# Cecile-hi/Multimodal-Learning-with-Alternating-Unimodal-Adaptation

Hardware: AMD Instinct MI355X
Metric: samples/sec per MLA alternating step, CREMA-D A+V bs=64 (higher is better)
Workload: dtype f32; 1 GPU; CREMA-D MLA step (--gs_flag, --lorb base ResNet18 audio+visual, GS projection as_intended), per-GPU batch 64: spec 1x1024x128 + frames 3x3x224x224, 6 classes; global_batch=64, parallelism=dp1

## Files before the change

### include/mla_hip.h

```cpp
#ifndef MLA_HIP_H
#define MLA_HIP_H

#include <stddef.h>
#include <stdint.h>

#ifdef __cplusplus
extern "C" {
#endif

enum mla_status {
  MLA_OK = 0,
  MLA_ERR_INVALID_ARG = -1,
  MLA_ERR_WORKSPACE = -2,
  MLA_ERR_LAUNCH = -3
};

int mla_abi_version(void);
const char* mla_last_error(void);

int mla_video_to_nhwc(const float* src, float* dst, int B, int C, int T, int H, int W, void* stream);
int mla_nchw_to_nhwc(const float* src, float* dst, int N, int C, int H, int W, void* stream);
int mla_nhwc_to_nchw(const float* src, float* dst, int N, int C, int H, int W, void* stream);

int mla_conv2d_f32_cfg(int cfg);
size_t mla_conv2d_fwd_partial_elems(int N, int H, int W, int Cin, int Cout, int KH, int KW, int stride, int pad);
int mla_conv2d_fwd(const float* x, const float* w_hwio, float* y,
                   int N, int H, int W, int Cin, int Cout, int KH, int KW, int stride, int pad,
                   float* bn_partial, int* bn_tiles, void* stream);

int mla_conv2d_dgrad(const float* dy, const float* w_hwio, float* dx,
                     int N, int H, int W, int Cin, int Cout, int KH, int KW, int stride, int pad,
                     const float* residual, const float* relu_src, float* wt_ws, void* stream);

size_t mla_conv2d_wgrad_ws_bytes(int N, int H, int W, int Cin, int Cout, int KH, int KW, int stride, int pad);
int mla_conv2d_wgrad(const float* x, const float* dy, float* dw_hwio,
                     int N, int H, int W, int Cin, int Cout, int KH, int KW, int stride, int pad,
                     void* ws, size_t ws_bytes, void* stream);

size_t mla_conv2d_wsplit_bytes(int Cin, int Cout, int KH, int KW);
int mla_conv2d_wsplit(const float* w_hwio, void* wsplit, int Cin, int Cout, int KH, int KW, int transposed, void* stream);
int mla_conv2d_wsplit_batch(const float* params, void* wsplit, const int* desc, int n, int total_blocks, void* stream);
int mla_conv2d_fwd_split(const float* x, const void* wsplit_t, float* y,
                         int N, int H, int W, int Cin, int Cout, int KH, int KW, int stride, int pad,
                         float* bn_partial, int* bn_tiles, void* stream);
int mla_conv2d_dgrad_split(const float* dy, const void* wsplit, float* dx,
                           int N, int H, int W, int Cin, int Cout, int KH, int KW, int stride, int pad,
                           const float* residual, const float* relu_src, void* stream);

typedef struct mla_bn_reduce_req {
  const float* x;
  const float* mean;
  const float* invstd;
  float* partial;
} mla_bn_reduce_req;
size_t mla_conv2d_dgrad_bn_partial_elems(int N, int H, int W, int Cin);
int mla_conv2d_dgrad_bn(const float* dy, const float* w_hwio, float* dx, int N, int H, int W, int Cin, int Cout,
                        int KH, int KW, int stride, int pad, const float* residual, const float* relu_src, float* wt_ws,
                        const mla_bn_reduce_req* reqs, int nreq, int* bn_tiles, void* stream);
int mla_conv2d_dgrad_split_bn(const float* dy, const void* wsplit, float* dx, int N, int H, int W, int Cin, int Cout,
                              int KH, int KW, int stride, int pad, const float* residual, const float* relu_src,
                              const mla_bn_reduce_req* reqs, int nreq, int* bn_tiles, void* stream);
int mla_conv2d_dgrad_classes(const float* dy, const float* w_hwio, float* dx, int N, int H, int W, int Cin, int Cout,
                             int KH, int KW, int stride, int pad, const float* residual, const float* relu_src, float* wt_ws,
                             const mla_bn_reduce_req* reqs, int nreq, int* bn_tiles, int class_mask, int residual_mask,
                             void* stream);
int mla_conv2d_dgrad_split_classes(const float* dy, const void* wsplit, float* dx, int N, int H, int W, int Cin, int Cout,
                                   int KH, int KW, int stride, int pad, const float* residual, const float* relu_src,
                                   const mla_bn_reduce_req* reqs, int nreq, int* bn_tiles, int class_mask, int residual_mask,
                                   void* stream);
size_t mla_conv2d_wgrad_split_ws_bytes(int N, int H, int W, int Cin, int Cout, int KH, int KW, int stride, int pad);
int mla_conv2d_wgrad_split(const float* x, const float* dy, float* dw_hwio,
                           int N, int H, int W, int Cin, int Cout, int KH, int KW, int stride, int pad,
                           void* ws, size_t ws_bytes, void* stream);
int mla_conv2d_wgrad_tr(int on);
int mla_conv2d_patch(int on);
int mla_conv2d_bnfold_supported(int N, int H, int W, int Cin, int Cout, int KH, int KW, int stride, int pad);
int mla_conv2d_fwd_split_bnin(const float* x, const void* wsplit_t, float* y, int N, int H, int W, int Cin, int Cout, int KH, int KW,
                              int stride, int pad, const float* in_mean, const float* in_invstd, const float* in_gamma, const float* in_beta,
                              float* bn_partial, int* bn_tiles, void* stream);
int mla_conv2d_wgrad_split_bnin(const float* x, const float* dy, float* dw_hwio, int N, int H, int W, int Cin, int Cout, int KH, int KW,
                                int stride, int pad, const float* in_mean, const float* in_invstd, const float* in_gamma,
                                const float* in_beta, void* ws, size_t ws_bytes, void* stream);
int mla_conv2d_dgrad_split_bnmask(const float* dy, const void* wsplit, float* dx, int N, int H, int W, int Cin, int Cout, int KH, int KW,
                                  int stride, int pad, const mla_bn_reduce_req* reqs, int nreq, int* bn_tiles, const float* mask_gamma,
                                  const float* mask_beta, void* stream);
int mla_conv2d_dgrad_merge(int on);
int mla_conv2d_two_phase(int on);
int mla_conv2d_split_terms(int terms);
int mla_conv2d_stem_supported(int Cin, int Cout, int KH, int KW, int stride, int pad);
int mla_conv2d_stem_waves(int waves);
size_t mla_conv2d_stem_fwd_partial_elems(void);
int mla_conv2d_stem_fwd_split(const float* x, const float* w_hwio, float* y,
                              int N, int H, int W, int Cin, int Cout, int KH, int KW, int stride, int pad,
                              float* bn_partial, int* bn_tiles, void* stream);
size_t mla_conv2d_stem_wgrad_split_ws_bytes(int Cin);
int mla_conv2d_stem_wgrad_split(const float* x, const float* dy, float* dw_hwio,
                                int N, int H, int W, int Cin, int Cout, int KH, int KW, int stride, int pad,
                                void* ws, size_t ws_bytes, void* stream);
int mla_conv2d_split_cfg(int cfg);

size_t mla_conv2d_wimage_bytes_bf16(int Cin, int Cout, int KH, int KW);
int mla_conv2d_wimage_bf16(const float* w_hwio, void* wimage, int Cin, int Cout, int KH, int KW, int transposed, void* stream);
int mla_conv2d_wimage_batch_bf16(const float* params, void* wimage, const int* desc, int n, int total_blocks, void* stream);
int mla_conv2d_tile_bf16(int M, int Cout, int k_total);
int mla_conv2d_fwd_bf16(const float* x, const void* wimage_t, float* y,
                        int N, int H, int W, int Cin, int Cout, int KH, int KW, int stride, int pad,
                        float* bn_partial, int* bn_tiles, void* stream);
int mla_conv2d_dgrad_bf16(const float* dy, const void* wimage, float* dx,
                          int N, int H, int W, int Cin, int Cout, int KH, int KW, int stride, int pad,
                          const float* residual, const float* relu_src, int class_mask, int residual_mask, void* stream);
size_t mla_conv2d_wgrad_ws_bytes_bf16(int N, int H, int W, int Cin, int Cout, int KH, int KW, int stride, int pad);
int mla_conv2d_wgrad_bf16(const float* x, const float* dy, float* dw_hwio,
                          int N, int H, int W, int Cin, int Cout, int KH, int KW, int stride, int pad,
                          void* ws, size_t ws_bytes, void* stream);

size_t mla_bn_partial_scratch_elems(int C);
size_t mla_bn_stats_partial_elems(int M, int C);
int mla_bn_stats_partial(const float* x, int M, int C, float* partial, int* tiles, void* stream);
int mla_bn_finalize(const float* partial, int tiles, int M, int C, float eps, float momentum,
                    float* mean, float* invstd, float* running_mean, float* running_var, void* stream);
int mla_bn_apply(const float* x, const float* mean, const float* invstd, const float* gamma,
                 const float* beta, const float* residual, float* out, int M, int C, int relu, void* stream);
size_t mla_bn_bwd_ws_elems(int M, int C);
int mla_bn_bwd(const float* dout, const float* relu_out, const float* x, const float* mean,
               const float* invstd, const float* gamma, float* dx, float* dgamma, float* dbeta,
               float* g_out, float* ws, int M, int C, void* stream);

int mla_bn_bwd_from_partial(const float* dout, const float* x, const float* mean, const float* invstd, const float* gamma,
                            float* dx, float* dgamma, float* dbeta, float* partial, int tiles, int M, int C, void* stream);
int mla_bn_relu_maxpool_fwd(const float* y, const float* mean, const float* invstd, const float* gamma,
                            const float* beta, float* out, uint8_t* idx, int N, int H, int W, int C, void* stream);
int mla_bn_bwd_pooled(const float* dpool, const uint8_t* idx, const float* y, const float* mean, const float* invstd,
                      const float* gamma, const float* beta, float* dy, float* dgamma, float* dbeta, float* ws,
                      int N, int H, int W, int C, void* stream);

int mla_maxpool3x3s2_fwd(const float* x, float* y, uint8_t* idx, int N, int H, int W, int C, void* stream);
int mla_maxpool3x3s2_bwd(const float* dy, const uint8_t* idx, const float* relu_src, float* dx,
                         int N, int H, int W, int C, void* stream);
int mla_avgpool_fwd(const float* x, float* y, int NB, int P, int C, void* stream);
int mla_avgpool_bwd(const float* dy, const float* relu_src, float* dx, int NB, int P, int C, void* stream);

size_t mla_head_ws_elems(int B, int C);
int mla_head_ce_fwd_bwd(const float* X, const float* W, const float* b, const int64_t* labels,
                        float* logits, float* loss, float* dW, float* db, float* dX, float* ws,
                        int B, int D, int C, float inv_batch, void* stream);

int mla_ce_fwd_bwd(const float* logits, const int64_t* labels, float* loss, float* dlogits, float* ws,
                   int B, int C, float inv_batch, void* stream);
int mla_head_bwd(const float* X, const float* W, const float* dlogits, float* dW, float* db, float* dX,
                 int B, int D, int C, float scale, void* stream);
int mla_scale_by_device_scalar(float* x, const float* scalar, size_t n, void* stream);

size_t mla_concat_head_ws_elems(int B, int C, int M);
int mla_concat_head_ce_fwd_bwd(const float* x0, const float* x1, const float* x2, const float* W, const float* b,
                               const int64_t* labels, float* out, float* out_m, float* loss, float* loss_m, float* dW,
                               float* db, float* dx0, float* dx1, float* dx2, float* ws, int M, int B, int D, int C,
                               float inv_batch, void* stream);
int mla_concat_head_fwd(const float* x0, const float* x1, const float* x2, const float* W, const float* b, float* out,
                        float* out_m, int M, int B, int D, int C, void* stream);
int mla_concat_head_bwd(const float* x0, const float* x1, const float* x2, const float* W, const float* dlogits, float* dW,
                        float* db, float* dx0, float* dx1, float* dx2, int M, int B, int D, int C, float scale, void* stream);

int mla_colsum(const float* X, float* r, int B, int D, float scale, void* stream);
size_t mla_gs_ws_elems(int D, int C);
int mla_gs_project(float* Pl, const float* r, float* G, int D, int C, float alpha, float* ws, void* stream);

int mla_ogm_coeff(const float* out0, const float* out1, const float* out2, const int64_t* labels, int M, int B, int C,
                  float alpha, float* coeff, float* info, void* stream);
int mla_ogm_chunk_elems(void);
size_t mla_ogm_ws_bytes(int total_chunks, int n_seg);
int mla_ogm_modulate(float* grad, const int64_t* seg_desc, const int* first_chunk, int n_seg, int total_chunks,
                     const float* coeff, int ge, uint64_t seed, uint64_t step, void* ws, size_t ws_bytes, void* stream);

int mla_linear_fwd(const float* x, const float* w_kn, const float* bias, const float* residual, float* y,
                   float* y_gelu, int groups, int rows, int x_group_rows, int x_off, int y_group_rows, int y_off,
                   int K, int N, void* stream);
int mla_linear_dgrad(const float* dy, const float* w_kn, float* dx, const float* residual, const float* gelu_src,
                     float* wt_ws, int groups, int rows, int dy_group_rows, int dy_off, int dx_group_rows, int dx_off,
                     int K, int N, void* stream);
size_t mla_linear_wgrad_ws_bytes(int M, int K, int N);
int mla_linear_wgrad(const float* x, const float* dy, float* dw_kn, int groups, int rows, int x_group_rows, int x_off,
                     int K, int N, void* ws, size_t ws_bytes, void* stream);
int mla_linear_fwd_split(const float* x, const void* wsplit_t, const float* bias, const float* residual, float* y,
                         float* y_gelu, int groups, int rows, int x_group_rows, int x_off, int y_group_rows, int y_off,
                         int K, int N, void* stream);
int mla_linear_dgrad_split(const float* dy, const void* wsplit, float* dx, const float* residual, const float* gelu_src,
                           int groups, int rows, int dy_group_rows, int dy_off, int dx_group_rows, int dx_off,
                           int K, int N, void* stream);
size_t mla_linear_wgrad_split_ws_bytes(int M, int K, int N);
int mla_linear_wgrad_split(const float* x, const float* dy, float* dw_kn, int groups, int rows, int x_group_rows, int x_off,
                           int K, int N, void* ws, size_t ws_bytes, void* stream);
int mla_linear_wgrad_split_bias(const float* x, const float* dy, float* dw_kn, float* dbias, int groups, int rows,
                                int x_group_rows, int x_off, int K, int N, void* ws, size_t ws_bytes, void* stream);
int mla_linear_fwd_bf16(const float* x, const void* wimage_t, const float* bias, const float* residual, float* y,
                        float* y_gelu, int groups, int rows, int x_group_rows, int x_off, int y_group_rows, int y_off,
                        int K, int N, void* stream);
int mla_linear_dgrad_bf16(const float* dy, const void* wimage, float* dx, const float* residual, const float* gelu_src,
                          int groups, int rows, int dy_group_rows, int dy_off, int dx_group_rows, int dx_off, int K, int N,
                          void* stream);
size_t mla_linear_wgrad_ws_bytes_bf16(int M, int K, int N);
int mla_linear_wgrad_bf16(const float* x, const float* dy, float* dw_kn, int groups, int rows, int x_group_rows, int x_off,
                          int K, int N, void* ws, size_t ws_bytes, void* stream);
int mla_linear_wgrad_bias_bf16(const float* x, const float* dy, float* dw_kn, float* dbias, int groups, int rows,
                               int x_group_rows, int x_off, int K, int N, void* ws, size_t ws_bytes, void* stream);
size_t mla_colreduce_ws_elems(int M, int C);
int mla_colsum_rows(const float* x, float* out, float* ws, int M, int C, void* stream);
int mla_layernorm_fwd(const float* x, const float* w, const float* b, float* y, float* mean, float* rstd,
                      int M, int D, float eps, void* stream);
int mla_layernorm_bwd(const float* dy, const float* x, const float* w, const float* mean, const float* rstd,
                      const float* add, float* dx, float* dw, float* db, float* ws, int M, int D, void* stream);
int mla_bgemm(const float* A, const float* B, float* C, int batches, int heads, int M, int N, int K,
              const long* a_strides, const long* b_strides, const long* c_strides,
              size_t a_extent, size_t b_extent, size_t c_extent, float alpha, void* stream);
int mla_softmax_fwd(float* S, const float* pad_mask, int B, int H, int n, void* stream);
int mla_softmax_bwd(const float* P, float* dP, int B, int H, int n, void* stream);

int mla_attention_fwd(const float* qkv, const float* pad_mask, float* o, float* lse, int B, int H, int n, int hd, void* stream);
int mla_attention_bwd(const float* d_o, const float* qkv, const float* o, const float* lse, const float* pad_mask,
                      float* dqkv, float* dvec, int B, int H, int n, int hd, void* stream);
int mla_tokens_assemble(float* x0, const float* table, const int64_t* ids, const float* pos, const float* type,
                        const float* cls, int B, int L, int D, int V, void* stream);
size_t mla_tokens_assemble_bwd_ws_bytes(int B, int L, int D);
int mla_tokens_assemble_bwd(const float* dx0, const float* colsum_all, const int64_t* ids, float* dcls, float* dtype,
                            float* dtable, int B, int L, int D, int V, void* ws, size_t ws_bytes, void* stream);
int mla_patchify(const float* img, float* out, int B, int C, int H, int W, int P, int transposed, void* stream);

int mla_frames_check(const int64_t* desc_host, int N, int B, int T, size_t frames_bytes, int out_h, int out_w);
int mla_frames_resample(const uint8_t* frames, size_t frames_bytes, const int64_t* desc, const int64_t* desc_host,
                        const float* lut, float* out, int N, int B, int T, int out_h, int out_w, void* stream);

int mla_head_logits(const float* X, const float* W, const float* b, float* logits, int B, int D, int C, void* stream);
int mla_eval_fuse(const float* out0, const float* out1, const float* out2, const int64_t* labels, int* counts,
                  float* weights_out, int M, int B, int C, int dynamic, float alpha0, float alpha1, float alpha2,
                  void* stream);
int mla_bn_invstd(const float* var, float* invstd, int n, float eps, void* stream);

int mla_sgd_step(float* p, const float* g, float* buf, size_t n, float lr, float momentum, float wd,
                 int first, void* stream);

#ifdef __cplusplus
}
#endif
#endif
```

### multimodal-learning-with-alternating-unimodal-adaptation_amd/csrc/bn.hip

```cpp
#include "common.h"

static size_t bn_red_scratch_floats(int C);
static int bn_tile_rows(int M) {
  long t = M > (1 << 18) ? ((long)M + 2047) / 2048 : ((long)M + 1023) / 1024;
  t = ((t + 15) / 16) * 16;
  if (t < 32) t = 32;
  if (t > 1024) t = 1024;
  return (int)t;
}

extern "C" size_t mla_bn_partial_scratch_elems(int C) { return bn_red_scratch_floats(C); }
extern "C" size_t mla_bn_stats_partial_elems(int M, int C) {
  return (size_t)cdiv(M, bn_tile_rows(M)) * 2 * C * 2 + bn_red_scratch_floats(C);
}
extern "C" size_t mla_bn_bwd_ws_elems(int M, int C) { return (size_t)cdiv(M, bn_tile_rows(M)) * 2 * C + bn_red_scratch_floats(C); }

template <int MODE>
__global__ __launch_bounds__(256) void bn_reduce_kernel(const float* __restrict__ x, const float* __restrict__ dout,
                                                         const float* __restrict__ relu_out,
                                                         const float* __restrict__ mean, const float* __restrict__ invstd,
                                                         float* __restrict__ partial, int M, int C, int tile_rows) {
  __shared__ f32x4 red[2][256];
  const int c4n = C >> 2;
  const int cg = threadIdx.x % c4n, rl = threadIdx.x / c4n, nrl = 256 / c4n;
  const int r0 = blockIdx.x * tile_rows, r1 = min(M, r0 + tile_rows);
  f32x4 s0 = {0.f, 0.f, 0.f, 0.f}, s1 = {0.f, 0.f, 0.f, 0.f};
  f32x4 mu = {0.f, 0.f, 0.f, 0.f}, is = {1.f, 1.f, 1.f, 1.f};
  if (MODE == 1) {
    mu = reinterpret_cast<const f32x4*>(mean)[cg];
    is = reinterpret_cast<const f32x4*>(invstd)[cg];
  }
  if (MODE == 0) {
    double d0[4] = {0.0, 0.0, 0.0, 0.0}, d1[4] = {0.0, 0.0, 0.0, 0.0};
    for (int r = r0 + rl; r < r1; r += nrl) {
      const f32x4 xv = reinterpret_cast<const f32x4*>(x)[(size_t)r * c4n + cg];
#pragma unroll
      for (int e = 0; e < 4; ++e) {
        const double v = (double)xv[e];
        d0[e] += v;
        d1[e] += v * v;
      }
    }
    __shared__ double redd[2][4][256];
#pragma unroll
    for (int e = 0; e < 4; ++e) {
      redd[0][e][threadIdx.x] = d0[e];
      redd[1][e][threadIdx.x] = d1[e];
    }
    __syncthreads();
    if (rl == 0) {
      double* pd = reinterpret_cast<double*>(partial);
#pragma unroll
      for (int e = 0; e < 4; ++e) {
        double a = d0[e], q = d1[e];
        for (int k = 1; k < nrl; ++k) {
          a += redd[0][e][k * c4n + cg];
          q += redd[1][e][k * c4n + cg];
        }
        pd[((size_t)blockIdx.x * 2 + 0) * C + cg * 4 + e] = a;
        pd[((size_t)blockIdx.x * 2 + 1) * C + cg * 4 + e] = q;
      }
    }
    return;
  }
  for (int r = r0 + rl; r < r1; r += nrl) {
    const size_t idx = (size_t)r * c4n + cg;
    const f32x4 xv = reinterpret_cast<const f32x4*>(x)[idx];
    if (MODE == 0) {
      s0 += xv;
      s1 += xv * xv;
    } else {
      f32x4 g = reinterpret_cast<const f32x4*>(dout)[idx];
      if (relu_out) {
        const f32x4 o = reinterpret_cast<const f32x4*>(relu_out)[idx];
#pragma unroll
        for (int e = 0; e < 4; ++e) g[e] = o[e] > 0.f ? g[e] : 0.f;
      }
      s0 += g;
      s1 += g * ((xv - mu) * is);
    }
  }
  red[0][threadIdx.x] = s0;
  red[1][threadIdx.x] = s1;
  __syncthreads();
  if (rl == 0) {
    for (int k = 1; k < nrl; ++k) {
      s0 += red[0][k * c4n + cg];
      s1 += red[1][k * c4n + cg];
    }
    reinterpret_cast<f32x4*>(partial + ((size_t)blockIdx.x * 2 + 0) * C)[cg] = s0;
    reinterpret_cast<f32x4*>(partial + ((size_t)blockIdx.x * 2 + 1) * C)[cg] = s1;
  }
}

#define BN_RED_MAXS 64
static int bn_red_chunks(int tiles) { int s = cdiv(tiles, 64); return s < 1 ? 1 : (s > BN_RED_MAXS ? BN_RED_MAXS : s); }
static size_t bn_red_scratch_floats(int C) { return (size_t)BN_RED_MAXS * 2 * C * 2 + 2; }

template <typename PT>
__global__ __launch_bounds__(256) void bn_tiles_stage1_kernel(const PT* __restrict__ partial, int tiles, int C,
                                                               double* __restrict__ scratch) {
  __shared__ double red[2][4][64];
  const int lane = threadIdx.x & 63, wave = threadIdx.x >> 6;
  const int c = blockIdx.x * 64 + lane;
  const int S = gridDim.y, per = (tiles + S - 1) / S;
  const int t0 = blockIdx.y * per, t1 = min(tiles, t0 + per);
  double s = 0.0, q = 0.0;
  if (c < C)
    for (int t = t0 + wave; t < t1; t += 4) {
      s += (double)partial[((size_t)t * 2 + 0) * C + c];
      q += (double)partial[((size_t)t * 2 + 1) * C + c];
    }
  red[0][wave][lane] = s;
  red[1][wave][lane] = q;
  __syncthreads();
  if (wave == 0 && c < C) {
    for (int w = 1; w < 4; ++w) {
      s += red[0][w][lane];
      q += red[1][w][lane];
    }
    scratch[((size_t)blockIdx.y * 2 + 0) * C + c] = s;
    scratch[((size_t)blockIdx.y * 2 + 1) * C + c] = q;
  }
}

__device__ __forceinline__ void chunk_sums(const double* __restrict__ scratch, int S, int C, double& s, double& q) {
  __shared__ double red2[2][4][64];
  const int lane = threadIdx.x & 63, kl = threadIdx.x >> 6;
  const int c = blockIdx.x * 64 + lane;
  double sv[BN_RED_MAXS / 4], qv[BN_RED_MAXS / 4];
#pragma unroll
  for (int j = 0; j < BN_RED_MAXS / 4; ++j) {
    const int k = kl + 4 * j;
    const bool ok = k < S && c < C;
    sv[j] = ok ? scratch[((size_t)k * 2 + 0) * C + c] : 0.0;
    qv[j] = ok ? scratch[((size_t)k * 2 + 1) * C + c] : 0.0;
  }
  s = 0.0;
  q = 0.0;
#pragma unroll
  for (int j = 0; j < BN_RED_MAXS / 4; ++j) {
    s += sv[j];
    q += qv[j];
  }
  red2[0][kl][lane] = s;
  red2[1][kl][lane] = q;
  __syncthreads();
  if (kl == 0)
    for (int w = 1; w < 4; ++w) {
      s += red2[0][w][lane];
      q += red2[1][w][lane];
    }
}

__global__ __launch_bounds__(256) void bn_finalize_kernel(const double* __restrict__ scratch, int S, int M, int C, float eps,
                                                           float momentum, float* __restrict__ mean, float* __restrict__ invstd,
                                                           float* running_mean, float* running_var) {
  const int c = blockIdx.x * 64 + (threadIdx.x & 63);
  double s, q;
  chunk_sums(scratch, S, C, s, q);
  if ((threadIdx.x >> 6) != 0 || c >= C) return;
  const double m = s / M;
  double var = q / M - m * m;
  if (var < 0.0) var = 0.0;
  mean[c] = (float)m;
  invstd[c] = (float)(1.0 / sqrt(var + (double)eps));
  if (running_mean) {
    const double unb = var * ((double)M / (double)(M > 1 ? M - 1 : 1));
    running_mean[c] = (float)((1.0 - momentum) * (double)running_mean[c] + momentum * m);
    running_var[c] = (float)((1.0 - momentum) * (double)running_var[c] + momentum * unb);
  }
}

__global__ __launch_bounds__(256) void bn_bwd_finalize_kernel(const double* __restrict__ scratch, int S, int C,
                                                               float* __restrict__ dgamma, float* __restrict__ dbeta) {
  const int c = blockIdx.x * 64 + (threadIdx.x & 63);
  double s, q;
  chunk_sums(scratch, S, C, s, q);
  if ((threadIdx.x >> 6) != 0 || c >= C) return;
  dbeta[c] = (float)s;
  dgamma[c] = (float)q;
}

#define BN_ONE_MAXT 1024
template <typename PT, int FWD>
__global__ __launch_bounds__(256) void bn_finalize_tiles_kernel(const PT* __restrict__ partial, int tiles, int M, int C, float eps,
                                                                 float momentum, float* __restrict__ out0, float* __restrict__ out1,
                                                                 float* running_mean, float* running_var) {
  __shared__ double red[2][16][16];
  const int cl = threadIdx.x & 15, kl = threadIdx.x >> 4;
  const int c = blockIdx.x * 16 + cl;
  double s = 0.0, q = 0.0;
  if (c < C) {
    int t = kl;
    for (; t + 48 < tiles; t += 64) {
      const double a0 = (double)partial[((size_t)t * 2 + 0) * C + c], b0 = (double)partial[((size_t)t * 2 + 1) * C + c];
      const double a1 = (double)partial[((size_t)(t + 16) * 2 + 0) * C + c], b1 = (double)partial[((size_t)(t + 16) * 2 + 1) * C + c];
      const double a2 = (double)partial[((size_t)(t + 32) * 2 + 0) * C + c], b2 = (double)partial[((size_t)(t + 32) * 2 + 1) * C + c];
      const double a3 = (double)partial[((size_t)(t + 48) * 2 + 0) * C + c], b3 = (double)partial[((size_t)(t + 48) * 2 + 1) * C + c];
      s += (a0 + a1) + (a2 + a3);
      q += (b0 + b1) + (b2 + b3);
    }
    for (; t < tiles; t += 16) {
      s += (double)partial[((size_t)t * 2 + 0) * C + c];
      q += (double)partial[((size_t)t * 2 + 1) * C + c];
    }
  }
  red[0][kl][cl] = s;
  red[1][kl][cl] = q;
  __syncthreads();
  if (kl != 0 || c >= C) return;
  for (int k = 1; k < 16; ++k) {
    s += red[0][k][cl];
    q += red[1][k][cl];
  }
  if (FWD) {
    const double m = s / M;
    double var = q / M - m * m;
    if (var < 0.0) var = 0.0;
    out0[c] = (float)m;
    out1[c] = (float)(1.0 / sqrt(var + (double)eps));
    if (running_mean) {
      const double unb = var * ((double)M / (double)(M > 1 ? M - 1 : 1));
      running_mean[c] = (float)((1.0 - momentum) * (double)running_mean[c] + momentum * m);
      running_var[c] = (float)((1.0 - momentum) * (double)running_var[c] + momentum * unb);
    }
  } else {
    out1[c] = (float)s;
    out0[c] = (float)q;
  }
}

#define BN_WIDE_MAXT 16384
template <typename PT, int FWD>
__global__ __launch_bounds__(256) void bn_finalize_tiles_wide_kernel(const PT* __restrict__ partial, int tiles, int M, int C, float eps,
                                                                      float momentum, float* __restrict__ out0, float* __restrict__ out1,
                                                                      float* running_mean, float* running_var) {
  __shared__ double red[2][64][4];
  const int cl = threadIdx.x & 3, kl = threadIdx.x >> 2;
  const int c = blockIdx.x * 4 + cl;
  double s = 0.0, q = 0.0;
  if (c < C) {
    int t = kl;
    for (; t + 192 < tiles; t += 256) {
      const double a0 = (double)partial[((size_t)t * 2 + 0) * C + c], b0 = (double)partial[((size_t)t * 2 + 1) * C + c];
      const double a1 = (double)partial[((size_t)(t + 64) * 2 + 0) * C + c], b1 = (double)partial[((size_t)(t + 64) * 2 + 1) * C + c];
      const double a2 = (double)partial[((size_t)(t + 128) * 2 + 0) * C + c], b2 = (double)partial[((size_t)(t + 128) * 2 + 1) * C + c];
      const double a3 = (double)partial[((size_t)(t + 192) * 2 + 0) * C + c], b3 = (double)partial[((size_t)(t + 192) * 2 + 1) * C + c];
      s += (a0 + a1) + (a2 + a3);
      q += (b0 + b1) + (b2 + b3);
    }
    for (; t < tiles; t += 64) {
      s += (double)partial[((size_t)t * 2 + 0) * C + c];
      q += (double)partial[((size_t)t * 2 + 1) * C + c];
    }
  }
  red[0][kl][cl] = s;
  red[1][kl][cl] = q;
  __syncthreads();
  if (kl != 0 || c >= C) return;
  for (int k = 1; k < 64; ++k) {
    s += red[0][k][cl];
    q += red[1][k][cl];
  }
  if (FWD) {
    const double m = s / M;
    double var = q / M - m * m;
    if (var < 0.0) var = 0.0;
    out0[c] = (float)m;
    out1[c] = (float)(1.0 / sqrt(var + (double)eps));
    if (running_mean) {
      const double unb = var * ((double)M / (double)(M > 1 ? M - 1 : 1));
      running_mean[c] = (float)((1.0 - momentum) * (double)running_mean[c] + momentum * m);
      running_var[c] = (float)((1.0 - momentum) * (double)running_var[c] + momentum * unb);
    }
  } else {
    out1[c] = (float)s;
    out0[c] = (float)q;
  }
}

__device__ __forceinline__ f32x4 bn_val(const f32x4 x, const f32x4 mu, const f32x4 is, const f32x4 ga, const f32x4 be) {
  f32x4 r;
#pragma unroll
  for (int e = 0; e < 4; ++e) r[e] = bn_val1(x[e], mu[e], is[e], ga[e], be[e]);
  return r;
}

__global__ __launch_bounds__(256) void bn_apply_kernel(const float* __restrict__ x, const float* __restrict__ mean,
                                                        const float* __restrict__ invstd,
                                                        const float* __restrict__ gamma, const float* __restrict__ beta,
                                                        const float* residual, float* out, size_t n4, int c4n, int relu) {
  for (size_t idx = (size_t)blockIdx.x * blockDim.x + threadIdx.x; idx < n4; idx += (size_t)gridDim.x * blockDim.x) {
    const int cg = (int)(idx % c4n);
    const f32x4 mu = reinterpret_cast<const f32x4*>(mean)[cg], is = reinterpret_cast<const f32x4*>(invstd)[cg];
    const f32x4 ga = reinterpret_cast<const f32x4*>(gamma)[cg], be = reinterpret_cast<const f32x4*>(beta)[cg];
    f32x4 v = bn_val(reinterpret_cast<const f32x4*>(x)[idx], mu, is, ga, be);
    if (residual) v += reinterpret_cast<const f32x4*>(residual)[idx];
    if (relu) {
#pragma unroll
      for (int e = 0; e < 4; ++e) v[e] = fmaxf(v[e], 0.f);
    }
    reinterpret_cast<f32x4*>(out)[idx] = v;
  }
}

__global__ __launch_bounds__(256) void bn_bwd_apply_kernel(const float* dout, const float* __restrict__ relu_out,
                                                            const float* __restrict__ x, const float* __restrict__ mean,
                                                            const float* __restrict__ invstd,
                                                            const float* __restrict__ gamma,
                                                            const float* __restrict__ dgamma,
                                                            const float* __restrict__ dbeta, float* dx, float* g_out,
                                                            size_t n4, int c4n, float invM) {
  for (size_t idx = (size_t)blockIdx.x * blockDim.x + threadIdx.x; idx < n4; idx += (size_t)gridDim.x * blockDim.x) {
    const int cg = (int)(idx % c4n);
    const f32x4 mu = reinterpret_cast<const f32x4*>(mean)[cg], is = reinterpret_cast<const f32x4*>(invstd)[cg];
    const f32x4 ga = reinterpret_cast<const f32x4*>(gamma)[cg];
    const f32x4 dg = reinterpret_cast<const f32x4*>(dgamma)[cg] * invM, db = reinterpret_cast<const f32x4*>(dbeta)[cg] * invM;
    f32x4 g = reinterpret_cast<const f32x4*>(dout)[idx];
    if (relu_out) {
      const f32x4 o = reinterpret_cast<const f32x4*>(relu_out)[idx];
#pragma unroll
      for (int e = 0; e < 4; ++e) g[e] = o[e] > 0.f ? g[e] : 0.f;
    }
    const f32x4 xhat = (reinterpret_cast<const f32x4*>(x)[idx] - mu) * is;
    if (g_out) reinterpret_cast<f32x4*>(g_out)[idx] = g;
    reinterpret_cast<f32x4*>(dx)[idx] = ga * is * (g - db - xhat * dg);
  }
}


__global__ __launch_bounds__(256) void bn_relu_maxpool_fwd_kernel(const float* __restrict__ y, const float* __restrict__ mean,
                                                                   const float* __restrict__ invstd, const float* __restrict__ gamma,
                                                                   const float* __restrict__ beta, float* __restrict__ out,
                                                                   uint8_t* __restrict__ idx, int N, int H, int W, int C, int OH, int OW) {
  const int c4n = C >> 2, QH = (OH + 1) >> 1, QW = (OW + 1) >> 1;
  const size_t total = (size_t)N * QH * QW * c4n;
  for (size_t i = (size_t)blockIdx.x * blockDim.x + threadIdx.x; i < total; i += (size_t)gridDim.x * blockDim.x) {
    const int cg = (int)(i % c4n);
    size_t p = i / c4n;
    const int oxq = (int)(p % QW); p /= QW;
    const int oyq = (int)(p % QH);
    const int n = (int)(p / QH);
    const f32x4 mu = reinterpret_cast<const f32x4*>(mean)[cg], is = reinterpret_cast<const f32x4*>(invstd)[cg];
    const f32x4 ga = reinterpret_cast<const f32x4*>(gamma)[cg], be = reinterpret_cast<const f32x4*>(beta)[cg];
    f32x4 best[2][2];
    int bi[2][2][4];
    bool first[2][2];
#pragma unroll
    for (int qy = 0; qy < 2; ++qy)
#pragma unroll
      for (int qx = 0; qx < 2; ++qx) {
        best[qy][qx] = f32x4{-INFINITY, -INFINITY, -INFINITY, -INFINITY};
        first[qy][qx] = true;
#pragma unroll
        for (int e = 0; e < 4; ++e) bi[qy][qx][e] = 0;
      }
    const int iy0 = oyq * 4 - 1, ix0 = oxq * 4 - 1;
#pragma unroll
    for (int r = 0; r < 5; ++r) {
      const int iy = iy0 + r;
      if ((unsigned)iy >= (unsigned)H) continue;
      f32x4 v[5];
      bool ok[5];
#pragma unroll
      for (int c = 0; c < 5; ++c) {
        const int ix = ix0 + c;
        ok[c] = (unsigned)ix < (unsigned)W;
        v[c] = ok[c] ? reinterpret_cast<const f32x4*>(y)[((size_t)(n * H + iy) * W + ix) * c4n + cg] : f32x4{0.f, 0.f, 0.f, 0.f};
      }
#pragma unroll
      for (int c = 0; c < 5; ++c) {
        v[c] = bn_val(v[c], mu, is, ga, be);
#pragma unroll
        for (int e = 0; e < 4; ++e) v[c][e] = v[c][e] != v[c][e] ? v[c][e] : fmaxf(v[c][e], 0.f);
      }
#pragma unroll
      for (int qy = 0; qy < 2; ++qy) {
        const int kh = r - 2 * qy;
        if (kh < 0 || kh > 2) continue;
#pragma unroll
        for (int qx = 0; qx < 2; ++qx)
#pragma unroll
          for (int kw = 0; kw < 3; ++kw) {
            const int c = 2 * qx + kw;
            if (!ok[c]) continue;
#pragma unroll
            for (int e = 0; e < 4; ++e) {
              const float ve = v[c][e];
              if (first[qy][qx] || ve > best[qy][qx][e] || ve != ve) {
                best[qy][qx][e] = ve;
                bi[qy][qx][e] = kh * 3 + kw;
              }
            }
            first[qy][qx] = false;
          }
      }
    }
#pragma unroll
    for (int qy = 0; qy < 2; ++qy)
#pragma unroll
      for (int qx = 0; qx < 2; ++qx) {
        const int oy = oyq * 2 + qy, ox = oxq * 2 + qx;
        if (oy >= OH || ox >= OW) continue;
        const size_t o = ((size_t)(n * OH + oy) * OW + ox) * c4n + cg;
        reinterpret_cast<f32x4*>(out)[o] = best[qy][qx];
        reinterpret_cast<uchar4*>(idx)[o] = make_uchar4(bi[qy][qx][0], bi[qy][qx][1], bi[qy][qx][2], bi[qy][qx][3]);
      }
  }
}

__global__ __launch_bounds__(256) void bn_bwd_pooled_reduce_kernel(const float* __restrict__ dpool, const uint8_t* __restrict__ idx,
                                                                    const float* __restrict__ y, const float* __restrict__ mean,
                                                                    const float* __restrict__ invstd, const float* __restrict__ gamma,
                                                                    const float* __restrict__ beta, float* __restrict__ out, int N, int H,
                                                                    int W, int C, int OH, int OW, int tile_rows) {
  __shared__ f32x4 red[2][256];
  const int c4n = C >> 2, MP = N * OH * OW;
  const int cg = threadIdx.x % c4n, rl = threadIdx.x / c4n, nrl = 256 / c4n;
  const int r0 = blockIdx.x * tile_rows, r1 = min(MP, r0 + tile_rows);
  const f32x4 mu = reinterpret_cast<const f32x4*>(mean)[cg], is = reinterpret_cast<const f32x4*>(invstd)[cg];
  const f32x4 ga = reinterpret_cast<const f32x4*>(gamma)[cg], be = reinterpret_cast<const f32x4*>(beta)[cg];
  f32x4 s0 = {0.f, 0.f, 0.f, 0.f}, s1 = {0.f, 0.f, 0.f, 0.f};
  for (int r = r0 + rl; r < r1; r += nrl) {
    const int ox = r % OW, t = r / OW, oy = t % OH, n = t / OH;
    const size_t o = (size_t)r * c4n + cg;
    const f32x4 g = reinterpret_cast<const f32x4*>(dpool)[o];
    const uchar4 sel = reinterpret_cast<const uchar4*>(idx)[o];
    const int code[4] = {sel.x, sel.y, sel.z, sel.w};
    f32x4 xv;
#pragma unroll
    for (int e = 0; e < 4; ++e) {
      const int kh = (code[e] * 11) >> 5, kw = code[e] - 3 * kh;
      xv[e] = y[((size_t)(n * H + oy * 2 - 1 + kh) * W + (ox * 2 - 1 + kw)) * C + cg * 4 + e];
    }
    const f32x4 a = bn_val(xv, mu, is, ga, be);
    const f32x4 xhat = (xv - mu) * is;
#pragma unroll
    for (int e = 0; e < 4; ++e) {
      const float ge = a[e] > 0.f ? g[e] : 0.f;
      s0[e] += ge;
      s1[e] += ge * xhat[e];
    }
  }
  red[0][threadIdx.x] = s0;
  red[1][threadIdx.x] = s1;
  __syncthreads();
  if (rl == 0) {
    for (int k = 1; k < nrl; ++k) {
      s0 += red[0][k * c4n + cg];
      s1 += red[1][k * c4n + cg];
    }
    reinterpret_cast<f32x4*>(out + ((size_t)blockIdx.x * 2 + 0) * C)[cg] = s0;
    reinterpret_cast<f32x4*>(out + ((size_t)blockIdx.x * 2 + 1) * C)[cg] = s1;
  }
}

__global__ __launch_bounds__(256) void bn_bwd_pooled_apply_kernel(const float* __restrict__ dpool, const uint8_t* __restrict__ idx,
                                                                   const float* __restrict__ y, const float* __restrict__ mean,
                                                                   const float* __restrict__ invstd, const float* __restrict__ gamma,
                                                                   const float* __restrict__ beta, const float* __restrict__ dgamma,
                                                                   const float* __restrict__ dbeta, float* __restrict__ out, int N, int H,
                                                                   int W, int C, int OH, int OW) {
  const int c4n = C >> 2, QH = (H + 1) >> 1, QW = (W + 1) >> 1;
  const size_t total = (size_t)N * QH * QW * c4n;
  const float invM = 1.0f / ((float)N * (float)H * (float)W);
  for (size_t i = (size_t)blockIdx.x * blockDim.x + threadIdx.x; i < total; i += (size_t)gridDim.x * blockDim.x) {
    const int cg = (int)(i % c4n);
    size_t p = i / c4n;
    const int b = (int)(p % QW); p /= QW;
    const int a = (int)(p % QH);
    const int n = (int)(p / QH);
    const f32x4 mu = reinterpret_cast<const f32x4*>(mean)[cg], is = reinterpret_cast<const f32x4*>(invstd)[cg];
    const f32x4 ga = reinterpret_cast<const f32x4*>(gamma)[cg], be = reinterpret_cast<const f32x4*>(beta)[cg];
    const f32x4 dg = reinterpret_cast<const f32x4*>(dgamma)[cg] * invM, db = reinterpret_cast<const f32x4*>(dbeta)[cg] * invM;
    f32x4 wg[2][2];
    int ws[2][2][4];
#pragma unroll
    for (int wy = 0; wy < 2; ++wy)
#pragma unroll
      for (int wx = 0; wx < 2; ++wx) {
        const int oy = a + wy, ox = b + wx;
        if (oy < OH && ox < OW) {
          const size_t o = ((size_t)(n * OH + oy) * OW + ox) * c4n + cg;
          wg[wy][wx] = reinterpret_cast<const f32x4*>(dpool)[o];
          const uchar4 s = reinterpret_cast<const uchar4*>(idx)[o];
          ws[wy][wx][0] = s.x; ws[wy][wx][1] = s.y; ws[wy][wx][2] = s.z; ws[wy][wx][3] = s.w;
        } else {
          wg[wy][wx] = f32x4{0.f, 0.f, 0.f, 0.f};
          ws[wy][wx][0] = ws[wy][wx][1] = ws[wy][wx][2] = ws[wy][wx][3] = -1;
        }
      }
#pragma unroll
    for (int py = 0; py < 2; ++py)
#pragma unroll
      for (int px = 0; px < 2; ++px) {
        const int iy = 2 * a + py, ix = 2 * b + px;
        if (iy >= H || ix >= W) continue;
        f32x4 g = {0.f, 0.f, 0.f, 0.f};
#pragma unroll
        for (int wy = 0; wy <= py; ++wy)
#pragma unroll
          for (int wx = 0; wx <= px; ++wx) {
            const int code = (py + 1 - 2 * wy) * 3 + (px + 1 - 2 * wx);
#pragma unroll
            for (int e = 0; e < 4; ++e) g[e] += ws[wy][wx][e] == code ? wg[wy][wx][e] : 0.f;
          }
        const size_t o = ((size_t)(n * H + iy) * W + ix) * c4n + cg;
        const f32x4 xv = reinterpret_cast<const f32x4*>(y)[o];
        const f32x4 av = bn_val(xv, mu, is, ga, be);
#pragma unroll
        for (int e = 0; e < 4; ++e) g[e] = av[e] > 0.f ? g[e] : 0.f;
        const f32x4 xhat = (xv - mu) * is;
        reinterpret_cast<f32x4*>(out)[o] = ga * is * (g - db - xhat * dg);
      }
  }
}

static int bn_check(const char* who, int M, int C) {
  MLA_REQUIRE(M > 0 && C > 0, "%s: non-positive dims", who);
  MLA_REQUIRE(C % 4 == 0 && C <= 1024 && 256 % (C / 4) == 0, "%s: C=%d must be 4*2^k, <= 1024", who, C);
  return MLA_OK;
}

static int ew_grid(size_t n4) {
  size_t b = (n4 + 255) / 256;
  return (int)(b < 1 ? 1 : (b > 8192 ? 8192 : b));
}

extern "C" int mla_bn_stats_partial(const float* x, int M, int C, float* partial, int* tiles, void* stream) {
  if (int rc = bn_check("mla_bn_stats_partial", M, C)) return rc;
  MLA_REQUIRE(x && partial, "mla_bn_stats_partial: null pointer");
  const int tr = bn_tile_rows(M), nt = cdiv(M, tr);
  bn_reduce_kernel<0><<<nt, 256, 0, (hipStream_t)stream>>>(x, nullptr, nullptr, nullptr, nullptr, partial, M, C, tr);
  MLA_CHECK_LAUNCH("bn_reduce_kernel<0>");
  if (tiles) *tiles = nt;
  return MLA_OK;
}

extern "C" int mla_bn_finalize(const float* partial, int tiles, int M, int C, float eps, float momentum, float* mean,
                               float* invstd, float* running_mean, float* running_var, void* stream) {
  MLA_REQUIRE(partial && mean && invstd && tiles > 0 && M > 0 && C > 0, "mla_bn_finalize: bad argument");
  MLA_REQUIRE((running_mean == nullptr) == (running_var == nullptr), "mla_bn_finalize: running stats must come in pairs");
  MLA_REQUIRE(((uintptr_t)partial % 8) == 0, "mla_bn_finalize: partial must be 8-byte aligned");
  hipStream_t st = (hipStream_t)stream;
  const double* pd = reinterpret_cast<const double*>(partial);
  if (tiles <= BN_ONE_MAXT) {
    bn_finalize_tiles_kernel<double, 1><<<cdiv(C, 16), 256, 0, st>>>(pd, tiles, M, C, eps, momentum, mean, invstd, running_mean, running_var);
    MLA_CHECK_LAUNCH("bn_finalize_tiles_kernel");
    return MLA_OK;
  }
  if (tiles <= BN_WIDE_MAXT) {
    bn_finalize_tiles_wide_kernel<double, 1><<<cdiv(C, 4), 256, 0, st>>>(pd, tiles, M, C, eps, momentum, mean, invstd, running_mean, running_var);
    MLA_CHECK_LAUNCH("bn_finalize_tiles_wide_kernel");
    return MLA_OK;
  }
  double* scratch = const_cast<double*>(pd) + (size_t)tiles * 2 * C;
  const int S = bn_red_chunks(tiles);
  bn_tiles_stage1_kernel<double><<<dim3(cdiv(C, 64), S), 256, 0, st>>>(pd, tiles, C, scratch);
  MLA_CHECK_LAUNCH("bn_tiles_stage1_kernel");
  bn_finalize_kernel<<<cdiv(C, 64), 256, 0, st>>>(scratch, S, M, C, eps, momentum, mean, invstd, running_mean, running_var);
  MLA_CHECK_LAUNCH("bn_finalize_kernel");
  return MLA_OK;
}

extern "C" int mla_bn_apply(const float* x, const float* mean, const float* invstd, const float* gamma,
                            const float* beta, const float* residual, float* out, int M, int C, int relu, void* stream) {
  if (int rc = bn_check("mla_bn_apply", M, C)) return rc;
  MLA_REQUIRE(x && mean && invstd && gamma && beta && out, "mla_bn_apply: null pointer");
  const size_t n4 = (size_t)M * C / 4;
  bn_apply_kernel<<<ew_grid(n4), 256, 0, (hipStream_t)stream>>>(x, mean, invstd, gamma, beta, residual, out, n4, C / 4, relu);
  MLA_CHECK_LAUNCH("bn_apply_kernel");
  return MLA_OK;
}

extern "C" int mla_bn_bwd(const float* dout, const float* relu_out, const float* x, const float* mean,
                          const float* invstd, const float* gamma, float* dx, float* dgamma, float* dbeta, float* g_out,
                          float* ws, int M, int C, void* stream) {
  if (int rc = bn_check("mla_bn_bwd", M, C)) return rc;
  MLA_REQUIRE(dout && x && mean && invstd && gamma && dx && dgamma && dbeta && ws, "mla_bn_bwd: null pointer");
  hipStream_t st = (hipStream_t)stream;
  const int tr = bn_tile_rows(M), nt = cdiv(M, tr);
  bn_reduce_kernel<1><<<nt, 256, 0, st>>>(x, dout, relu_out, mean, invstd, ws, M, C, tr);
  MLA_CHECK_LAUNCH("bn_reduce_kernel<1>");
  if (nt <= BN_ONE_MAXT) {
    bn_finalize_tiles_kernel<float, 0><<<cdiv(C, 16), 256, 0, st>>>(ws, nt, M, C, 0.f, 0.f, dgamma, dbeta, nullptr, nullptr);
    MLA_CHECK_LAUNCH("bn_finalize_tiles_kernel");
  } else if (nt <= BN_WIDE_MAXT) {
    bn_finalize_tiles_wide_kernel<float, 0><<<cdiv(C, 4), 256, 0, st>>>(ws, nt, M, C, 0.f, 0.f, dgamma, dbeta, nullptr, nullptr);
    MLA_CHECK_LAUNCH("bn_finalize_tiles_wide_kernel");
  } else {
    double* scratch = reinterpret_cast<double*>(ws + (size_t)nt * 2 * C);
    const int S = bn_red_chunks(nt);
    bn_tiles_stage1_kernel<float><<<dim3(cdiv(C, 64), S), 256, 0, st>>>(ws, nt, C, scratch);
    MLA_CHECK_LAUNCH("bn_tiles_stage1_kernel");
    bn_bwd_finalize_kernel<<<cdiv(C, 64), 256, 0, st>>>(scratch, S, C, dgamma, dbeta);
    MLA_CHECK_LAUNCH("bn_bwd_finalize_kernel");
  }
  const size_t n4 = (size_t)M * C / 4;
  bn_bwd_apply_kernel<<<ew_grid(n4), 256, 0, st>>>(dout, relu_out, x, mean, invstd, gamma, dgamma, dbeta, dx, g_out, n4,
                                                   C / 4, 1.0f / (float)M);
  MLA_CHECK_LAUNCH("bn_bwd_apply_kernel");
  return MLA_OK;
}

extern "C" int mla_bn_bwd_from_partial(const float* dout, const float* x, const float* mean, const float* invstd,
                                       const float* gamma, float* dx, float* dgamma, float* dbeta, float* partial, int tiles,
                                       int M, int C, void* stream) {
  if (int rc = bn_check("mla_bn_bwd_from_partial", M, C)) return rc;
  MLA_REQUIRE(dout && x && mean && invstd && gamma && dx && dgamma && dbeta && partial && tiles > 0,
              "mla_bn_bwd_from_partial: null pointer or no tiles");
  hipStream_t st = (hipStream_t)stream;
  if (tiles <= BN_ONE_MAXT) {
    bn_finalize_tiles_kernel<float, 0><<<cdiv(C, 16), 256, 0, st>>>(partial, tiles, M, C, 0.f, 0.f, dgamma, dbeta, nullptr, nullptr);
    MLA_CHECK_LAUNCH("bn_finalize_tiles_kernel");
  } else if (tiles <= BN_WIDE_MAXT) {
    bn_finalize_tiles_wide_kernel<float, 0><<<cdiv(C, 4), 256, 0, st>>>(partial, tiles, M, C, 0.f, 0.f, dgamma, dbeta, nullptr, nullptr);
    MLA_CHECK_LAUNCH("bn_finalize_tiles_wide_kernel");
  } else {
    double* scratch = reinterpret_cast<double*>(partial + (size_t)tiles * 2 * C);
    const int S = bn_red_chunks(tiles);
    bn_tiles_stage1_kernel<float><<<dim3(cdiv(C, 64), S), 256, 0, st>>>(partial, tiles, C, scratch);
    MLA_CHECK_LAUNCH("bn_tiles_stage1_kernel");
    bn_bwd_finalize_kernel<<<cdiv(C, 64), 256, 0, st>>>(scratch, S, C, dgamma, dbeta);
    MLA_CHECK_LAUNCH("bn_bwd_finalize_kernel");
  }
  const size_t n4 = (size_t)M * C / 4;
  bn_bwd_apply_kernel<<<ew_grid(n4), 256, 0, st>>>(dout, nullptr, x, mean, invstd, gamma, dgamma, dbeta, dx, nullptr, n4, C / 4,
                                                   1.0f / (float)M);
  MLA_CHECK_LAUNCH("bn_bwd_apply_kernel");
  return MLA_OK;
}

extern "C" int mla_bn_relu_maxpool_fwd(const float* y, const float* mean, const float* invstd, const float* gamma, const float* beta,
                                       float* out, uint8_t* idx, int N, int H, int W, int C, void* stream) {
  if (int rc = bn_check("mla_bn_relu_maxpool_fwd", N * H * W, C)) return rc;
  MLA_REQUIRE(y && mean && invstd && gamma && beta && out && idx && N > 0 && H > 0 && W > 0, "mla_bn_relu_maxpool_fwd: bad argument");
  const int OH = (H + 2 - 3) / 2 + 1, OW = (W + 2 - 3) / 2 + 1;
  const size_t n4 = (size_t)N * ((OH + 1) / 2) * ((OW + 1) / 2) * (C / 4);
  bn_relu_maxpool_fwd_kernel<<<ew_grid(n4), 256, 0, (hipStream_t)stream>>>(y, mean, invstd, gamma, beta, out, idx, N, H, W, C, OH, OW);
  MLA_CHECK_LAUNCH("bn_relu_maxpool_fwd_kernel");
  return MLA_OK;
}

extern "C" int mla_bn_bwd_pooled(const float* dpool, const uint8_t* idx, const float* y, const float* mean, const float* invstd,
                                 const float* gamma, const float* beta, float* dy, float* dgamma, float* dbeta, float* ws, int N,
                                 int H, int W, int C, void* stream) {
  const long Ml = (long)N * H * W;
  MLA_REQUIRE(Ml > 0 && Ml < (1L << 31), "mla_bn_bwd_pooled: bad dims");
  const int M = (int)Ml;
  if (int rc = bn_check("mla_bn_bwd_pooled", M, C)) return rc;
  MLA_REQUIRE(dpool && idx && y && mean && invstd && gamma && beta && dy && dgamma && dbeta && ws, "mla_bn_bwd_pooled: null pointer");
  hipStream_t st = (hipStream_t)stream;
  const int OH = (H + 2 - 3) / 2 + 1, OW = (W + 2 - 3) / 2 + 1;
  const int MP = N * OH * OW;
  const int trp = bn_tile_rows(MP), nt = cdiv(MP, trp);
  bn_bwd_pooled_reduce_kernel<<<nt, 256, 0, st>>>(dpool, idx, y, mean, invstd, gamma, beta, ws, N, H, W, C, OH, OW, trp);
  MLA_CHECK_LAUNCH("bn_bwd_pooled_reduce_kernel");
  if (nt <= BN_ONE_MAXT) {
    bn_finalize_tiles_kernel<float, 0><<<cdiv(C, 16), 256, 0, st>>>(ws, nt, M, C, 0.f, 0.f, dgamma, dbeta, nullptr, nullptr);
    MLA_CHECK_LAUNCH("bn_finalize_tiles_kernel");
  } else if (nt <= BN_WIDE_MAXT) {
    bn_finalize_tiles_wide_kernel<float, 0><<<cdiv(C, 4), 256, 0, st>>>(ws, nt, M, C, 0.f, 0.f, dgamma, dbeta, nullptr, nullptr);
    MLA_CHECK_LAUNCH("bn_finalize_tiles_wide_kernel");
  } else {
    double* scratch = reinterpret_cast<double*>(ws + (size_t)nt * 2 * C);
    const int S = bn_red_chunks(nt);
    bn_tiles_stage1_kernel<float><<<dim3(cdiv(C, 64), S), 256, 0, st>>>(ws, nt, C, scratch);
    MLA_CHECK_LAUNCH("bn_tiles_stage1_kernel");
    bn_bwd_finalize_kernel<<<cdiv(C, 64), 256, 0, st>>>(scratch, S, C, dgamma, dbeta);
    MLA_CHECK_LAUNCH("bn_bwd_finalize_kernel");
  }
  const size_t nq = (size_t)N * ((H + 1) / 2) * ((W + 1) / 2) * (C / 4);
  bn_bwd_pooled_apply_kernel<<<ew_grid(nq), 256, 0, st>>>(dpool, idx, y, mean, invstd, gamma, beta, dgamma, dbeta, dy, N, H, W, C, OH, OW);
  MLA_CHECK_LAUNCH("bn_bwd_pooled_apply_kernel");
  return MLA_OK;
}
```

### multimodal-learning-with-alternating-unimodal-adaptation_amd/csrc/common.h

```cpp
#pragma once
#include <hip/hip_runtime.h>
#include <limits.h>
#include <stdint.h>
#include <stdio.h>
#include <stdlib.h>
#include "../../include/mla_hip.h"

#define MLA_WAVE 64

typedef float f32x4 __attribute__((ext_vector_type(4)));
typedef float f32x16 __attribute__((ext_vector_type(16)));

void mla_set_error(const char* fmt, ...);

#define MLA_REQUIRE(cond, ...)              \
  do {                                      \
    if (!(cond)) {                          \
      mla_set_error(__VA_ARGS__);           \
      return MLA_ERR_INVALID_ARG;           \
    }                                       \
  } while (0)

#define MLA_CHECK_LAUNCH(name)                                             \
  do {                                                                     \
    hipError_t e__ = hipGetLastError();                                    \
    if (e__ != hipSuccess) {                                               \
      mla_set_error("%s: launch failed: %s", name, hipGetErrorString(e__)); \
      return MLA_ERR_LAUNCH;                                               \
    }                                                                      \
  } while (0)

static inline int cdiv(long a, long b) { return (int)((a + b - 1) / b); }

inline int mla_cu_count() {
  static const int cus = [] {
    int dev = 0, n = 0;
    if (hipGetDevice(&dev) != hipSuccess || hipDeviceGetAttribute(&n, hipDeviceAttributeMultiprocessorCount, dev) != hipSuccess || n <= 0) n = 256;
    return n;
  }();
  return cus;
}

struct EnvInt {
  const char* name;
  int lo, hi, dflt;
  bool numeric = false;
  int v = INT_MIN;
  int get() {
    if (v == INT_MIN) {
      const char* e = getenv(name);
      v = dflt;
      if (e && numeric) { const int x = atoi(e); v = x < lo ? lo : (x > hi ? hi : x); }
      else if (e && e[0] >= '0' + lo && e[0] <= '0' + hi) v = e[0] - '0';
    }
    return v;
  }
  int hook(int x) {
    if (x >= lo && x <= hi) v = x;
    return get();
  }
};

__device__ __forceinline__ float wave_sum(float v) {
#pragma unroll
  for (int o = 32; o > 0; o >>= 1) v += __shfl_xor(v, o, 64);
  return v;
}
__device__ __forceinline__ double wave_sum_d(double v) {
#pragma unroll
  for (int o = 32; o > 0; o >>= 1) v += __shfl_xor(v, o, 64);
  return v;
}
__device__ __forceinline__ float wave_max(float v) {
#pragma unroll
  for (int o = 32; o > 0; o >>= 1) v = fmaxf(v, __shfl_xor(v, o, 64));
  return v;
}

__device__ __forceinline__ float bn_val1(float x, float mu, float is, float ga, float be) { return fmaf((x - mu) * is, ga, be); }

__device__ __forceinline__ void tile_coords(int wg, int gridM, int gridN, int& tm, int& tn) {
  if (gridN <= 8) {
    tm = wg / gridN;
    tn = wg - tm * gridN;
    return;
  }
  const int per_panel = gridM * 8;
  int panel = wg / per_panel;
  const int full = gridN >> 3;
  if (panel > full) panel = full;
  const int rem = wg - panel * per_panel;
  const int pw = panel < full ? 8 : gridN - full * 8;
  tm = rem / pw;
  tn = panel * 8 + (rem - tm * pw);
}

__device__ __forceinline__ int xcd_remap(int bid, int nwg) {
  const int q = nwg >> 3, r = nwg & 7, x = bid & 7, l = bid >> 3;
  return (x < r ? x * (q + 1) : r * (q + 1) + (x - r) * q) + l;
}
```

### multimodal-learning-with-alternating-unimodal-adaptation_amd/csrc/stem_split.hip

```cpp
#include "split_common.h"
#ifndef WG_VALU
#define WG_VALU 6
#endif

namespace {

template <int CIN>
struct StemCfg {
  static_assert(CIN == 1 || CIN == 3, "stem: 1 (audio) or 3 (visual) input channels");
  static constexpr int ROWE = 7 * CIN;
  static constexpr int G = (ROWE + 7) / 8;
  static constexpr int NG = 7 * G;
  static constexpr int NCH = (NG + 1) / 2;
  static constexpr int KPAD = NCH * 16;
  static constexpr int KROW = KPAD + ((KPAD / 8) % 2 == 0 ? 8 : 0);
  static constexpr int SR = 37;
  static constexpr int SE = 37 * CIN;
  static constexpr int NPQ = (SE + 1) / 2;
  static constexpr int PD = CIN == 1 ? 24 : 56;
  static constexpr int SBUF = SR * PD + 8;
  static constexpr int NLD = (SR * NPQ + 255) / 256;
  static constexpr int WPC = CIN == 1 ? 2 : 1;
};

struct StemGeom {
  int N, H, W, OH, OW, tilesY, tilesX, ntiles;
  unsigned x_bytes, y_bytes;
};

__device__ __forceinline__ unsigned off_or_oob(int ok, unsigned off) { return off | ((unsigned)ok - 1u); }
__device__ __forceinline__ int in_range(int v, int n) { return (int)((unsigned)v < (unsigned)n); }

__device__ __forceinline__ void buf_store1(rsrc_t r, float v, unsigned voff) {
  __builtin_amdgcn_raw_buffer_store_b32(__builtin_bit_cast(unsigned, v), r, (int)voff, 0, 0);
}

template <int CIN, bool STATS, bool RAGGED, int WAVES>
__global__ __launch_bounds__(64 * WAVES, (CIN == 3 && WAVES == 4) ? 1 : 2) void stem_fwd_split_kernel(
    const float* __restrict__ X, const float* __restrict__ Wf, float* __restrict__ Y, double* __restrict__ part, const StemGeom g) {
  using C = StemCfg<CIN>;
  constexpr int G = C::G, NG = C::NG, NCH = C::NCH, KROW = C::KROW, PD = C::PD, SBUF = C::SBUF, NPQ = C::NPQ;
  constexpr int NT = 64 * WAVES, MI = 8 / WAVES;
  constexpr int NLD = (C::SR * NPQ + NT - 1) / NT;
  static_assert(WAVES == 4 || WAVES == 8, "4 or 8 waves");
  __shared__ __attribute__((aligned(16))) unsigned short Wl[3 * 64 * KROW];
  __shared__ __attribute__((aligned(16))) unsigned S[2 * 3 * SBUF];

  const int tid = threadIdx.x, lane = tid & 63, wave = tid >> 6;
  const int i = lane & 31, h = lane >> 5;

  for (int idx = tid; idx < C::KPAD * 64; idx += NT) {
    const int co = idx & 63, k = idx >> 6;
    const int gq = k >> 3, e = k & 7;
    const int kh = gq / G, pt = gq - kh * G, re = pt * 8 + e;
    const float v = (gq < NG && re < C::ROWE) ? Wf[(kh * C::ROWE + re) * 64 + co] : 0.f;
    unsigned hi, mid, lo;
    split_pair(v, 0.f, hi, mid, lo);
    Wl[co * KROW + k] = (unsigned short)hi;
    Wl[64 * KROW + co * KROW + k] = (unsigned short)mid;
    Wl[2 * 64 * KROW + co * KROW + k] = (unsigned short)lo;
  }
  for (int idx = tid; idx < 2 * 3 * SBUF; idx += NT) S[idx] = 0u;

  const rsrc_t xr = make_rsrc(X, g.x_bytes), yr = make_rsrc(Y, g.y_bytes);
  auto slot_row = [&](int u) { const int s = tid + NT * u; return s < C::SR * NPQ ? s / NPQ : -1; };
  auto slot_pair = [&](int u) { const int s = tid + NT * u; return s - (s / NPQ) * NPQ; };
  float pre0[NLD], pre1[NLD];
  auto decode = [&](int t, int& n, int& oy0, int& ox0) {
    const int per = g.tilesY * g.tilesX;
    n = t / per;
    const int rem = t - n * per;
    const int ty = rem / g.tilesX;
    oy0 = ty * 16;
    ox0 = (rem - ty * g.tilesX) * 16;
  };
  auto stage_load = [&](int t) {
    int n, oy0, ox0;
    decode(t, n, oy0, ox0);
    const int iy0 = 2 * oy0 - 3, ex0 = (2 * ox0 - 3) * CIN, rowE = g.W * CIN;
#pragma unroll
    for (int u = 0; u < NLD; ++u) {
      const int sr = slot_row(u), sp = slot_pair(u);
      const int iy = iy0 + sr, e0 = ex0 + 2 * sp;
      const int rok = (int)(sr >= 0) & in_range(iy, g.H);
      const unsigned base = ((unsigned)(n * g.H + iy) * (unsigned)rowE + (unsigned)e0) * 4u;
      const int ok0 = rok & in_range(e0, rowE) & (int)(2 * sp < C::SE);
      const int ok1 = rok & in_range(e0 + 1, rowE) & (int)(2 * sp + 1 < C::SE);
      pre0[u] = buf_load1(xr, off_or_oob(ok0, base), 0);
      pre1[u] = buf_load1(xr, off_or_oob(ok1, base + 4u), 0);
    }
  };
  constexpr int NPART = NLD < 3 ? NLD : 3, PER = (NLD + NPART - 1) / NPART;
  auto stage_store = [&](int buf, int part_) {
    unsigned* Sb = S + buf * 3 * SBUF;
#pragma unroll
    for (int u = 0; u < NLD; ++u) {
      if (part_ >= 0 && u / PER != part_) continue;
      unsigned hi, mid, lo;
      split_pair<true>(pre0[u], pre1[u], hi, mid, lo);
      const int sr = slot_row(u);
      const int d = sr >= 0 ? sr * PD + slot_pair(u) : C::SR * PD + 4;
      Sb[d] = hi;
      Sb[SBUF + d] = mid;
      Sb[2 * SBUF + d] = lo;
    }
  };

  int a_base[MI];
#pragma unroll
  for (int mi = 0; mi < MI; ++mi) {
    const int oyl = 2 * (MI * wave + mi) + (i >> 4), oxl = i & 15;
    a_base[mi] = 2 * oyl * PD + oxl * CIN;
  }
  const int b_base = i * KROW + 8 * h;

  double csum[2] = {0.0, 0.0}, csq[2] = {0.0, 0.0};
  float s1[2] = {0.f, 0.f}, s2[2] = {0.f, 0.f}, v0[2] = {0.f, 0.f}, cnt[2] = {0.f, 0.f};
  constexpr unsigned OOB_ST = 0xFFFFFF00u;
  auto epi_piece = [&](int piece, const f32x16 (&pa)[MI][2], int pn, int poy0, int pox0) {
    const int mi = piece >> 2, eq = piece & 3;
#pragma unroll
    for (int e4 = 0; e4 < 4; ++e4) {
      const int e = 4 * eq + e4;
      const int row = e4 + 8 * eq + 4 * h;
      const int oy = poy0 + 2 * (MI * wave + mi) + (row >> 4), ox = pox0 + (row & 15);
      int ok;
      if constexpr (RAGGED) ok = (int)(oy < g.OH) & (int)(ox < g.OW);
      else ok = (int)(poy0 < (1 << 27));
      const unsigned off = (((unsigned)((pn * g.OH + oy) * g.OW + ox) * 64u + (unsigned)i) * 4u) | (((unsigned)ok - 1u) & OOB_ST);
#pragma unroll
      for (int ni = 0; ni < 2; ++ni) {
        const float v = pa[mi][ni][e];
        buf_store1(yr, v, off + ni * 128u);
        if constexpr (STATS) {
          if (piece == 0 && e4 == 0) {
            v0[ni] = RAGGED ? (ok ? v : 0.f) : v;
            if constexpr (RAGGED) cnt[ni] = 0.f;
          }
          const float d = v - v0[ni];
          if constexpr (RAGGED) {
            const float dz = ok ? d : 0.f;
            s1[ni] += dz;
            s2[ni] = fmaf(dz, dz, s2[ni]);
            cnt[ni] += ok ? 1.f : 0.f;
          } else {
            s1[ni] += d;
            s2[ni] = fmaf(d, d, s2[ni]);
          }
        }
      }
    }
  };
  auto fold_stats = [&](bool valid) {
    if constexpr (STATS) {
#pragma unroll
      for (int ni = 0; ni < 2; ++ni) {
        const double n_ = RAGGED ? (double)cnt[ni] : (valid ? 16.0 * MI : 0.0);
        const double a = (double)v0[ni], b = (double)s1[ni], c = (double)s2[ni];
        csum[ni] += n_ * a + b;
        csq[ni] += n_ * a * a + 2.0 * a * b + c;
        s1[ni] = 0.f;
        s2[ni] = 0.f;
      }
    }
  };

  int cur = 0;
  int t = blockIdx.x;
  if (t < g.ntiles) {
    stage_load(t);
    __syncthreads();
    stage_store(0, -1);
  }
  __syncthreads();
  f32x16 prev[MI][2];
  zero_acc(prev);
  int pn = 0, poy0 = 1 << 28, pox0 = 0;
  constexpr int NPC = 4 * MI;
  constexpr int NEB = NCH >= NPC + NPART ? NCH - NPART : (NCH < NPC ? NCH : NPC);
  constexpr int EPB = (NPC + NEB - 1) / NEB;
  for (; t < g.ntiles; t += gridDim.x) {
    const int tn = t + gridDim.x;
    const bool has_next = tn < g.ntiles;
    if (has_next) stage_load(tn);
    f32x16 acc[MI][2];
    const unsigned* Sc = S + cur * 3 * SBUF;
    struct Frags { u32x4 a[3][MI]; bf16x8_t b[3][2]; };
    auto load_frags = [&](int kk, Frags& f) {
      const int g0 = 2 * kk, g1 = 2 * kk + 1;
      const int off0 = g0 < NG ? (g0 / G) * PD + (g0 % G) * 4 : 0, off1 = g1 < NG ? (g1 / G) * PD + (g1 % G) * 4 : 0;
      const int loff = h ? off1 : off0;
#pragma unroll
      for (int pl = 0; pl < 3; ++pl) {
#pragma unroll
        for (int mi = 0; mi < MI; ++mi) {
          const unsigned* p = Sc + pl * SBUF + a_base[mi] + loff;
          f.a[pl][mi] = u32x4{p[0], p[1], p[2], p[3]};
        }
#pragma unroll
        for (int ni = 0; ni < 2; ++ni)
          f.b[pl][ni] = __builtin_bit_cast(bf16x8_t, *reinterpret_cast<const u32x4*>(Wl + pl * 64 * KROW + ni * 32 * KROW + b_base + kk * 16));
      }
    };
    auto mask_frags = [&](int kk, Frags& f) {
#pragma unroll
      for (int d = 0; d < 4; ++d) {
        unsigned m[2];
#pragma unroll
        for (int hh = 0; hh < 2; ++hh) {
          const int gq = 2 * kk + hh;
          const int pt = gq % G;
          const int nreal = gq < NG ? (C::ROWE - pt * 8 < 8 ? C::ROWE - pt * 8 : 8) : 0;
          m[hh] = nreal >= 2 * d + 2 ? 0xFFFFFFFFu : (nreal == 2 * d + 1 ? 0x0000FFFFu : 0u);
        }
        if (m[0] == 0xFFFFFFFFu && m[1] == 0xFFFFFFFFu) continue;
        const unsigned lm = h ? m[1] : m[0];
#pragma unroll
        for (int pl = 0; pl < 3; ++pl)
#pragma unroll
          for (int mi = 0; mi < MI; ++mi) f.a[pl][mi][d] &= lm;
      }
    };
    auto mma_frags = [&](const Frags& f, bool first) {
#pragma unroll
      for (int term = 0; term < 6; ++term)
#pragma unroll
        for (int mi = 0; mi < MI; ++mi)
#pragma unroll
          for (int ni = 0; ni < 2; ++ni) {
            f32x16 c = acc[mi][ni];
            if (first && term == 0) {
#pragma unroll
              for (int e = 0; e < 16; ++e) c[e] = 0.f;
            }
            acc[mi][ni] = __builtin_amdgcn_mfma_f32_32x32x16_bf16(__builtin_bit_cast(bf16x8_t, f.a[TERM_A[term]][mi]), f.b[TERM_B[term]][ni], c, 0, 0, 0);
          }
    };
    constexpr bool DBUF = !(CIN == 1 && WAVES == 4);
    Frags fr0, fr1;
    if constexpr (DBUF) load_frags(0, fr0);
#pragma unroll
    for (int kk = 0; kk < NCH; ++kk) {
      Frags& fc = (DBUF && (kk & 1)) ? fr1 : fr0;
      Frags& fn = (kk & 1) ? fr0 : fr1;
      if constexpr (DBUF) {
        if (kk + 1 < NCH) load_frags(kk + 1, fn);
      } else {
        load_frags(kk, fr0);
      }
      mask_frags(kk, fc);
      mma_frags(fc, kk == 0);
      if (kk < NEB) {
#pragma unroll
        for (int q = 0; q < EPB; ++q)
          if (kk * EPB + q < NPC) epi_piece(kk * EPB + q, prev, pn, poy0, pox0);
      }
      if (kk >= NCH - NPART) stage_store(cur ^ 1, kk - (NCH - NPART));
      __builtin_amdgcn_sched_group_barrier(0x100, 32, 0);
      __builtin_amdgcn_sched_group_barrier(0x002, 12 * MI, 0);
#pragma unroll
      for (int m = 0; m < 12 * MI; ++m) {
        __builtin_amdgcn_sched_group_barrier(0x008, 1, 0);
        __builtin_amdgcn_sched_group_barrier(0x002, 6, 0);
        __builtin_amdgcn_sched_group_barrier(0x040, 1, 0);
      }
      __builtin_amdgcn_sched_barrier(0);
    }
    fold_stats(poy0 < (1 << 27));
#pragma unroll
    for (int mi = 0; mi < MI; ++mi)
#pragma unroll
      for (int ni = 0; ni < 2; ++ni) prev[mi][ni] = acc[mi][ni];
    decode(t, pn, poy0, pox0);
    __syncthreads();
    cur ^= 1;
  }
#pragma unroll
  for (int piece = 0; piece < NPC; ++piece) epi_piece(piece, prev, pn, poy0, pox0);
  fold_stats(poy0 < (1 << 27));
  if constexpr (STATS) {
    double* red = reinterpret_cast<double*>(S);
    __syncthreads();
#pragma unroll
    for (int ni = 0; ni < 2; ++ni) {
      csum[ni] += __shfl_xor(csum[ni], 32, 64);
      csq[ni] += __shfl_xor(csq[ni], 32, 64);
      if (h == 0) {
        red[(wave * 2 + 0) * 64 + ni * 32 + i] = csum[ni];
        red[(wave * 2 + 1) * 64 + ni * 32 + i] = csq[ni];
      }
    }
    __syncthreads();
    if (tid < 64) {
      double s = 0.0, q = 0.0;
#pragma unroll
      for (int w = 0; w < WAVES; ++w) {
        s += red[(w * 2 + 0) * 64 + tid];
        q += red[(w * 2 + 1) * 64 + tid];
      }
      part[((size_t)blockIdx.x * 2 + 0) * 64 + tid] = s;
      part[((size_t)blockIdx.x * 2 + 1) * 64 + tid] = q;
    }
  }
}

template <int CIN>
struct StemWCfg {
  static constexpr int K = 49 * CIN;
  static constexpr int KB = (K + 31) / 32;
  static constexpr int SR = 37;
  static constexpr int XQ = 10;
  static constexpr int XPD = CIN == 1 ? 13 : 10;
  static constexpr int ARR = SR * XPD;
  static constexpr int HALF = CIN * ARR + (CIN == 1 ? 9 : 0);
  static constexpr int ZROW = 2 * HALF;
  static constexpr int PLANE = ZROW + 16;
  static constexpr int COPY = 3 * PLANE + (CIN == 1 ? 20 : 0);
  static constexpr int SBUF = 2 * COPY;
  static constexpr int NSL = 2 * CIN * SR * XQ;
  static constexpr int RACC = KB * 32 * 64;
  static constexpr int LDSF = 2 * SBUF > RACC ? 2 * SBUF : RACC;
};

template <int CIN>
__global__ __launch_bounds__(512, 2) void stem_wgrad_split_kernel(const float* __restrict__ X, const float* __restrict__ dY,
                                                                   float* __restrict__ slabs, const StemGeom g, unsigned dy_bytes) {
  using C = StemWCfg<CIN>;
  constexpr int KB = C::KB, XPD = C::XPD, ARR = C::ARR, HALF = C::HALF, PLANE = C::PLANE, COPY = C::COPY, SBUF = C::SBUF;
  constexpr int NT = 512, NLD = (C::NSL + NT - 1) / NT;
  __shared__ __attribute__((aligned(16))) unsigned S[C::LDSF];

  const int tid = threadIdx.x, lane = tid & 63, wave = tid >> 6;
  const int i = lane & 31, h = lane >> 5;
  const int ni = wave >> 2, wq = wave & 3;
  for (int idx = tid; idx < C::LDSF; idx += NT) S[idx] = 0u;

  const rsrc_t xr = make_rsrc(X, g.x_bytes), yr = make_rsrc(dY, dy_bytes);
  float pre0[NLD], pre1[NLD], pre2[NLD];
  auto decode = [&](int t, int& n, int& oy0, int& ox0) {
    const int per = g.tilesY * g.tilesX;
    n = t / per;
    const int rem = t - n * per;
    const int ty = rem / g.tilesX;
    oy0 = ty * 16;
    ox0 = (rem - ty * g.tilesX) * 16;
  };
  auto stage_load = [&](int t) {
    int n, oy0, ox0;
    decode(t, n, oy0, ox0);
    const int iy0 = 2 * oy0 - 3, ix0 = 2 * ox0 - 3;
#pragma unroll
    for (int u = 0; u < NLD; ++u) {
      const int sl = tid + NT * u;
      const int a = sl / (C::SR * C::XQ), rq = sl - a * (C::SR * C::XQ);
      const int r = rq / C::XQ, q = rq - r * C::XQ;
      const int par = a / CIN, ci = a - par * CIN;
      const int iy = iy0 + r;
      const int rok = (int)(sl < C::NSL) & in_range(iy, g.H);
      auto ld = [&](int j) {
        const int sc = 2 * (2 * q + j) + par;
        const int ix = ix0 + sc;
        const int ok = rok & (int)(sc <= 36) & in_range(ix, g.W);
        return buf_load1(xr, off_or_oob(ok, (((unsigned)(n * g.H + iy) * (unsigned)g.W + (unsigned)ix) * CIN + ci) * 4u), 0);
      };
      pre0[u] = ld(0);
      pre1[u] = ld(1);
      pre2[u] = ld(2);
    }
  };
  auto stage_store = [&](int buf, int u) {
    unsigned* Sb = S + buf * SBUF;
    const int sl = tid + NT * u;
    const int a = sl / (C::SR * C::XQ), rq = sl - a * (C::SR * C::XQ);
    const int r = rq / C::XQ, q = rq - r * C::XQ;
    const int par = a / CIN, ci = a - par * CIN;
    const int d = sl < C::NSL ? par * HALF + ci * ARR + r * XPD + q : C::ZROW + 8;
    unsigned h0, m0, l0, h1, m1, l1;
    split_pair<true>(pre0[u], pre1[u], h0, m0, l0);
    split_pair<true>(pre1[u], pre2[u], h1, m1, l1);
    Sb[d] = h0; Sb[PLANE + d] = m0; Sb[2 * PLANE + d] = l0;
    Sb[COPY + d] = h1; Sb[COPY + PLANE + d] = m1; Sb[COPY + 2 * PLANE + d] = l1;
  };

  int a_base[KB], a_rstep[KB];
#pragma unroll
  for (int kb = 0; kb < KB; ++kb) {
    const int k = kb * 32 + i;
    if (k < C::K) {
      const int kh = k / (7 * CIN), rem = k - kh * 7 * CIN;
      const int kw = rem / CIN, ci = rem - kw * CIN;
      const int sft = kw >> 1;
      a_base[kb] = (sft & 1) * COPY + (kw & 1) * HALF + ci * ARR + (kh + 8 * wq) * XPD + 4 * h + (sft >> 1);
      a_rstep[kb] = 2 * XPD;
    } else {
      a_base[kb] = C::ZROW + 4 * h;
      a_rstep[kb] = 0;
    }
  }

  f32x16 acc[KB];
  zero_acc(acc);

  constexpr int U = 4 * KB;
  float dyv[2][8];
  auto load_dy = [&](int t, int s, float (&dst)[8]) {
    int n, oy0, ox0;
    decode(t, n, oy0, ox0);
    const int oy = oy0 + 4 * wq + s;
#pragma unroll
    for (int e = 0; e < 8; ++e) {
      const int ox = ox0 + 8 * h + e;
      const int ok = (int)(t < g.ntiles) & (int)(oy < g.OH) & (int)(ox < g.OW);
      dst[e] = buf_load1(yr, off_or_oob(ok, ((unsigned)((n * g.OH + oy) * g.OW + ox) * 64u + (unsigned)(ni * 32 + i)) * 4u), 0);
    }
  };
  auto load_dy_step = [&](int t, int tn, int s, float (&dst)[8]) {
    if (s < 4) load_dy(t, s, dst);
    else load_dy(tn, s - 4, dst);
  };
  struct BFr { u32x4 p[3]; };
  auto split_dy_half = [&](int j, const float (&src)[8], BFr& b) {
#pragma unroll
    for (int qq = 0; qq < 2; ++qq) {
      const int q = 2 * j + qq;
      unsigned hi, mid, lo;
      split_pair<true>(src[2 * q], src[2 * q + 1], hi, mid, lo);
      b.p[0][q] = hi; b.p[1][q] = mid; b.p[2][q] = lo;
    }
  };
  struct AFr { u32x4 p[3]; };
  auto read_a = [&](const unsigned* Sc, int u, AFr& a) {
    const int s_ = u / KB, kb = u - s_ * KB;
    const unsigned* ap = Sc + a_base[kb] + s_ * a_rstep[kb];
#pragma unroll
    for (int pl = 0; pl < 3; ++pl) a.p[pl] = u32x4{ap[pl * PLANE], ap[pl * PLANE + 1], ap[pl * PLANE + 2], ap[pl * PLANE + 3]};
  };

  int cur = 0;
  int t = blockIdx.x;
  BFr bf0, bf1;
  if (t < g.ntiles) stage_load(t);
  __syncthreads();
  if (t < g.ntiles) {
#pragma unroll
    for (int u = 0; u < NLD; ++u) stage_store(0, u);
    load_dy(t, 0, dyv[0]);
    split_dy_half(0, dyv[0], bf0);
    split_dy_half(1, dyv[0], bf0);
    load_dy(t, 1, dyv[1]);
    load_dy(t, 2, dyv[0]);
  }
  __syncthreads();
  constexpr int ST0 = U - NLD < 0 ? 0 : U - NLD;
  for (; t < g.ntiles; t += gridDim.x) {
    const int tn = t + gridDim.x;
    const bool has_next = tn < g.ntiles;
    if (has_next) stage_load(tn);
    const unsigned* Sc = S + cur * SBUF;
    AFr a0, a1;
    read_a(Sc, 0, a0);
    __builtin_amdgcn_sched_barrier(0);
#pragma unroll
    for (int u = 0; u < U; ++u) {
      const int s_ = u / KB, kb = u - s_ * KB;
      AFr& acur = (u & 1) ? a1 : a0;
      AFr& anext = (u & 1) ? a0 : a1;
      BFr& bcur = (s_ & 1) ? bf1 : bf0;
      BFr& bnext = (s_ & 1) ? bf0 : bf1;
      if (u + 1 < U) read_a(Sc, u + 1, anext);
      if (kb < 2) split_dy_half(kb, dyv[(s_ + 1) & 1], bnext);
      if (u >= ST0) stage_store(cur ^ 1, u - ST0);
      split_mma<6>(acur.p, bcur.p, acc[kb]);
      if (kb == 1) load_dy_step(t, tn, s_ + 3, dyv[(s_ + 1) & 1]);
      __builtin_amdgcn_sched_group_barrier(0x100, 16, 0);
#pragma unroll
      for (int m = 0; m < 6; ++m) {
        __builtin_amdgcn_sched_group_barrier(0x008, 1, 0);
        __builtin_amdgcn_sched_group_barrier(0x002, WG_VALU, 0);
      }
      __builtin_amdgcn_sched_barrier(0);
    }
    __syncthreads();
    cur ^= 1;
  }
  float* R = reinterpret_cast<float*>(S);
  for (int w = 0; w < 4; ++w) {
    if (wq == w) {
#pragma unroll
      for (int kb = 0; kb < KB; ++kb) {
#pragma unroll
        for (int e = 0; e < 16; ++e) {
          const int row = kb * 32 + acc_row(e) + 4 * h;
          const int o = row * 64 + ni * 32 + i;
          const float v = w == 0 ? acc[kb][e] : R[o] + acc[kb][e];
          if (w == 3) {
            if (row < C::K) slabs[(size_t)blockIdx.x * C::K * 64 + o] = v;
          } else {
            R[o] = v;
          }
        }
      }
    }
    __syncthreads();
  }
}

int stem_check(const char* who, int N, int H, int W, int Cin, int Cout, int KH, int KW, int stride, int pad) {
  MLA_REQUIRE(KH == 7 && KW == 7 && stride == 2 && pad == 3 && Cout == 64 && (Cin == 1 || Cin == 3),
              "%s: the stem kernels are 7x7 / stride 2 / pad 3, 1 or 3 -> 64 channels (got %dx%d s%d p%d, %d -> %d)", who, KH, KW, stride, pad, Cin, Cout);
  MLA_REQUIRE(N > 0 && H > 0 && W > 0 && H < 32768 && W < 32768, "%s: bad dims", who);
  const long oh = (H + 6 - 7) / 2 + 1, ow = (W + 6 - 7) / 2 + 1;
  MLA_REQUIRE(oh > 0 && ow > 0 && (long)N * H * W * Cin * 4 < 0xFFFFFFF0L && (long)N * oh * ow * 64 * 4 < 0xFFFFFFF0L,
              "%s: input and output tensors must each be < 4 GiB (32-bit buffer offsets)", who);
  return MLA_OK;
}

}

static int g_stem_waves = 0;
extern "C" int mla_conv2d_stem_waves(int waves) {
  if (waves == 4 || waves == 8 || waves == 0) g_stem_waves = waves;
  return g_stem_waves;
}

extern "C" int mla_conv2d_stem_supported(int Cin, int Cout, int KH, int KW, int stride, int pad) {
  return KH == 7 && KW == 7 && stride == 2 && pad == 3 && Cout == 64 && (Cin == 1 || Cin == 3);
}

extern "C" size_t mla_conv2d_stem_fwd_partial_elems(void) { return (size_t)mla_cu_count() * 2 * 2 * 64 * 2; }

extern "C" int mla_conv2d_stem_fwd_split(const float* x, const float* w, float* y, int N, int H, int W, int Cin, int Cout, int KH,
                                         int KW, int stride, int pad, float* bn_partial, int* bn_tiles, void* stream) {
  if (int rc = stem_check("mla_conv2d_stem_fwd_split", N, H, W, Cin, Cout, KH, KW, stride, pad)) return rc;
  MLA_REQUIRE(x && w && y, "mla_conv2d_stem_fwd_split: null pointer");
  MLA_REQUIRE(!bn_partial || ((uintptr_t)bn_partial % 8) == 0, "mla_conv2d_stem_fwd_split: bn_partial must be 8-byte aligned");
  StemGeom g;
  g.N = N; g.H = H; g.W = W;
  g.OH = conv_out(H, 7, 2, 3); g.OW = conv_out(W, 7, 2, 3);
  g.tilesY = cdiv(g.OH, 16); g.tilesX = cdiv(g.OW, 16);
  g.ntiles = N * g.tilesY * g.tilesX;
  g.x_bytes = (unsigned)((size_t)N * H * W * Cin * 4);
  g.y_bytes = (unsigned)((size_t)N * g.OH * g.OW * 64 * 4);
  hipStream_t st = (hipStream_t)stream;
  const int waves = g_stem_waves ? g_stem_waves : (Cin == 1 ? 4 : 8);
  const int slots = mla_cu_count() * ((Cin == 1 && waves == 4) ? 2 : 1);
  const int grid = g.ntiles < slots ? g.ntiles : slots;
  double* pd = reinterpret_cast<double*>(bn_partial);
  const bool ragged = (g.OH % 16) != 0 || (g.OW % 16) != 0;
#define STEM_LAUNCH(CIN_, ST_, RG_, WV_) stem_fwd_split_kernel<CIN_, ST_, RG_, WV_><<<grid, 64 * WV_, 0, st>>>(x, w, y, pd, g)
#define STEM_PICK(CIN_, WV_)                                                            \
  do {                                                                                  \
    if (pd && ragged) STEM_LAUNCH(CIN_, true, true, WV_);                               \
    else if (pd) STEM_LAUNCH(CIN_, true, false, WV_);                                   \
    else if (ragged) STEM_LAUNCH(CIN_, false, true, WV_);                               \
    else STEM_LAUNCH(CIN_, false, false, WV_);                                          \
  } while (0)
  if (Cin == 1 && waves == 8) STEM_PICK(1, 8);
  else if (Cin == 1) STEM_PICK(1, 4);
  else if (waves == 8) STEM_PICK(3, 8);
  else STEM_PICK(3, 4);
#undef STEM_PICK
#undef STEM_LAUNCH
  MLA_CHECK_LAUNCH("stem_fwd_split_kernel");
  if (bn_tiles) *bn_tiles = grid;
  return MLA_OK;
}

int mla_wgrad_reduce(const float* part, float* dw, size_t n4, int splits, hipStream_t st);

extern "C" size_t mla_conv2d_stem_wgrad_split_ws_bytes(int Cin) { return (size_t)mla_cu_count() * 49 * Cin * 64 * sizeof(float); }

extern "C" int mla_conv2d_stem_wgrad_split(const float* x, const float* dy, float* dw, int N, int H, int W, int Cin, int Cout,
                                           int KH, int KW, int stride, int pad, void* ws, size_t ws_bytes, void* stream) {
  if (int rc = stem_check("mla_conv2d_stem_wgrad_split", N, H, W, Cin, Cout, KH, KW, stride, pad)) return rc;
  MLA_REQUIRE(x && dy && dw && ws, "mla_conv2d_stem_wgrad_split: null pointer");
  StemGeom g;
  g.N = N; g.H = H; g.W = W;
  g.OH = conv_out(H, 7, 2, 3); g.OW = conv_out(W, 7, 2, 3);
  g.tilesY = cdiv(g.OH, 16); g.tilesX = cdiv(g.OW, 16);
  g.ntiles = N * g.tilesY * g.tilesX;
  g.x_bytes = (unsigned)((size_t)N * H * W * Cin * 4);
  const size_t dyb = (size_t)N * g.OH * g.OW * 64 * 4;
  MLA_REQUIRE(dyb < 0xFFFFFFF0UL, "mla_conv2d_stem_wgrad_split: dy must be < 4 GiB (32-bit buffer offsets)");
  const int grid = g.ntiles < mla_cu_count() ? g.ntiles : mla_cu_count();
  const size_t need = (size_t)grid * 49 * Cin * 64 * sizeof(float);
  if (ws_bytes < need) {
    mla_set_error("mla_conv2d_stem_wgrad_split: workspace %zu < %zu bytes", ws_bytes, need);
    return MLA_ERR_WORKSPACE;
  }
  hipStream_t st = (hipStream_t)stream;
  if (Cin == 1) stem_wgrad_split_kernel<1><<<grid, 512, 0, st>>>(x, dy, (float*)ws, g, (unsigned)dyb);
  else stem_wgrad_split_kernel<3><<<grid, 512, 0, st>>>(x, dy, (float*)ws, g, (unsigned)dyb);
  MLA_CHECK_LAUNCH("stem_wgrad_split_kernel");
  return mla_wgrad_reduce((const float*)ws, dw, (size_t)49 * Cin * 64 / 4, grid, st);
}
```

### multimodal-learning-with-alternating-unimodal-adaptation_amd/mla_hip/_lib.py

```python
from __future__ import annotations

import ctypes
import os
from ctypes import c_char_p, c_float, c_int, c_size_t, c_void_p

_HERE = os.path.dirname(os.path.abspath(__file__))
LIB_PATH = os.path.join(_HERE, "libmla_hip.so")
LIB_PATH = os.environ.get("MLA_HIP_LIB", LIB_PATH)


class MLAHipError(RuntimeError):
    pass


_P, _I, _F, _Z = c_void_p, c_int, c_float, c_size_t

PROTOTYPES = {
    "mla_abi_version": (_I, []),
    "mla_last_error": (c_char_p, []),
    "mla_video_to_nhwc": (_I, [_P, _P, _I, _I, _I, _I, _I, _P]),
    "mla_nchw_to_nhwc": (_I, [_P, _P, _I, _I, _I, _I, _P]),
    "mla_nhwc_to_nchw": (_I, [_P, _P, _I, _I, _I, _I, _P]),
    "mla_conv2d_f32_cfg": (_I, [_I]),
    "mla_conv2d_fwd_partial_elems": (_Z, [_I] * 9),
    "mla_conv2d_fwd": (_I, [_P, _P, _P] + [_I] * 9 + [_P, _P, _P]),
    "mla_conv2d_dgrad": (_I, [_P, _P, _P] + [_I] * 9 + [_P, _P, _P, _P]),
    "mla_conv2d_wgrad_ws_bytes": (_Z, [_I] * 9),
    "mla_conv2d_wgrad": (_I, [_P, _P, _P] + [_I] * 9 + [_P, _Z, _P]),
    "mla_conv2d_wsplit_bytes": (_Z, [_I] * 4),
    "mla_conv2d_wsplit": (_I, [_P, _P, _I, _I, _I, _I, _I, _P]),
    "mla_conv2d_wsplit_batch": (_I, [_P, _P, _P, _I, _I, _P]),
    "mla_conv2d_fwd_split": (_I, [_P, _P, _P] + [_I] * 9 + [_P, _P, _P]),
    "mla_conv2d_dgrad_split": (_I, [_P, _P, _P] + [_I] * 9 + [_P, _P, _P]),
    "mla_conv2d_dgrad_bn_partial_elems": (_Z, [_I, _I, _I, _I]),
    "mla_conv2d_dgrad_bn": (_I, [_P, _P, _P] + [_I] * 9 + [_P, _P, _P, _P, _I, _P, _P]),
    "mla_conv2d_dgrad_split_bn": (_I, [_P, _P, _P] + [_I] * 9 + [_P, _P, _P, _I, _P, _P]),
    "mla_conv2d_dgrad_classes": (_I, [_P, _P, _P] + [_I] * 9 + [_P, _P, _P, _P, _I, _P, _I, _I, _P]),
    "mla_conv2d_dgrad_split_classes": (_I, [_P, _P, _P] + [_I] * 9 + [_P, _P, _P, _I, _P, _I, _I, _P]),
    "mla_conv2d_wgrad_split_ws_bytes": (_Z, [_I] * 9),
    "mla_conv2d_wgrad_split": (_I, [_P, _P, _P] + [_I] * 9 + [_P, _Z, _P]),
    "mla_conv2d_wgrad_tr": (_I, [_I]),
    "mla_conv2d_patch": (_I, [_I]),
    "mla_conv2d_dgrad_merge": (_I, [_I]),
    "mla_conv2d_two_phase": (_I, [_I]),
    "mla_conv2d_bnfold_supported": (_I, [_I] * 9),
    "mla_conv2d_fwd_split_bnin": (_I, [_P, _P, _P] + [_I] * 9 + [_P, _P, _P, _P, _P, _P, _P]),
    "mla_conv2d_wgrad_split_bnin": (_I, [_P, _P, _P] + [_I] * 9 + [_P, _P, _P, _P, _P, _Z, _P]),
    "mla_conv2d_dgrad_split_bnmask": (_I, [_P, _P, _P] + [_I] * 9 + [_P, _I, _P, _P, _P, _P]),
    "mla_conv2d_split_terms": (_I, [_I]),
    "mla_conv2d_stem_supported": (_I, [_I] * 6),
    "mla_conv2d_stem_waves": (_I, [_I]),
    "mla_conv2d_stem_fwd_partial_elems": (_Z, []),
    "mla_conv2d_stem_fwd_split": (_I, [_P, _P, _P] + [_I] * 9 + [_P, _P, _P]),
    "mla_conv2d_stem_wgrad_split_ws_bytes": (_Z, [_I]),
    "mla_conv2d_stem_wgrad_split": (_I, [_P, _P, _P] + [_I] * 9 + [_P, _Z, _P]),
    "mla_conv2d_split_cfg": (_I, [_I]),
    "mla_conv2d_wimage_bytes_bf16": (_Z, [_I] * 4),
    "mla_conv2d_wimage_bf16": (_I, [_P, _P, _I, _I, _I, _I, _I, _P]),
    "mla_conv2d_wimage_batch_bf16": (_I, [_P, _P, _P, _I, _I, _P]),
    "mla_conv2d_tile_bf16": (_I, [_I, _I, _I]),
    "mla_conv2d_fwd_bf16": (_I, [_P, _P, _P] + [_I] * 9 + [_P, _P, _P]),
    "mla_conv2d_dgrad_bf16": (_I, [_P, _P, _P] + [_I] * 9 + [_P, _P, _I, _I, _P]),
    "mla_conv2d_wgrad_ws_bytes_bf16": (_Z, [_I] * 9),
    "mla_conv2d_wgrad_bf16": (_I, [_P, _P, _P] + [_I] * 9 + [_P, _Z, _P]),
    "mla_bn_partial_scratch_elems": (_Z, [_I]),
    "mla_bn_stats_partial_elems": (_Z, [_I, _I]),
    "mla_bn_stats_partial": (_I, [_P, _I, _I, _P, _P, _P]),
    "mla_bn_finalize": (_I, [_P, _I, _I, _I, _F, _F, _P, _P, _P, _P, _P]),
    "mla_bn_apply": (_I, [_P, _P, _P, _P, _P, _P, _P, _I, _I, _I, _P]),
    "mla_bn_bwd_ws_elems": (_Z, [_I, _I]),
    "mla_bn_bwd": (_I, [_P] * 11 + [_I, _I, _P]),
    "mla_bn_bwd_from_partial": (_I, [_P] * 9 + [_I, _I, _I, _P]),
    "mla_bn_relu_maxpool_fwd": (_I, [_P] * 7 + [_I, _I, _I, _I, _P]),
    "mla_bn_bwd_pooled": (_I, [_P] * 11 + [_I, _I, _I, _I, _P]),
    "mla_maxpool3x3s2_fwd": (_I, [_P, _P, _P, _I, _I, _I, _I, _P]),
    "mla_maxpool3x3s2_bwd": (_I, [_P, _P, _P, _P, _I, _I, _I, _I, _P]),
    "mla_avgpool_fwd": (_I, [_P, _P, _I, _I, _I, _P]),
    "mla_avgpool_bwd": (_I, [_P, _P, _P, _I, _I, _I, _P]),
    "mla_head_ws_elems": (_Z, [_I, _I]),
    "mla_head_ce_fwd_bwd": (_I, [_P] * 10 + [_I, _I, _I, _F, _P]),
    "mla_ce_fwd_bwd": (_I, [_P, _P, _P, _P, _P, _I, _I, _F, _P]),
    "mla_head_bwd": (_I, [_P] * 6 + [_I, _I, _I, _F, _P]),
    "mla_scale_by_device_scalar": (_I, [_P, _P, _Z, _P]),
    "mla_concat_head_ws_elems": (_Z, [_I, _I, _I]),
    "mla_concat_head_ce_fwd_bwd": (_I, [_P] * 16 + [_I, _I, _I, _I, _F, _P]),
    "mla_concat_head_fwd": (_I, [_P] * 7 + [_I, _I, _I, _I, _P]),
    "mla_concat_head_bwd": (_I, [_P] * 10 + [_I, _I, _I, _I, _F, _P]),
    "mla_ogm_coeff": (_I, [_P, _P, _P, _P, _I, _I, _I, _F, _P, _P, _P]),
    "mla_ogm_chunk_elems": (_I, []),
    "mla_ogm_ws_bytes": (_Z, [_I, _I]),
    "mla_ogm_modulate": (_I, [_P, _P, _P, _I, _I, _P, _I, ctypes.c_uint64, ctypes.c_uint64, _P, _Z, _P]),
    "mla_colsum": (_I, [_P, _P, _I, _I, _F, _P]),
    "mla_gs_ws_elems": (_Z, [_I, _I]),
    "mla_gs_project": (_I, [_P, _P, _P, _I, _I, _F, _P, _P]),
    "mla_sgd_step": (_I, [_P, _P, _P, _Z, _F, _F, _F, _I, _P]),
    "mla_head_logits": (_I, [_P, _P, _P, _P, _I, _I, _I, _P]),
    "mla_eval_fuse": (_I, [_P, _P, _P, _P, _P, _P, _I, _I, _I, _I, _F, _F, _F, _P]),
    "mla_bn_invstd": (_I, [_P, _P, _I, _F, _P]),
    "mla_linear_fwd": (_I, [_P] * 6 + [_I] * 8 + [_P]),
    "mla_linear_dgrad": (_I, [_P] * 6 + [_I] * 8 + [_P]),
    "mla_linear_wgrad_ws_bytes": (_Z, [_I, _I, _I]),
    "mla_linear_wgrad": (_I, [_P, _P, _P] + [_I] * 6 + [_P, _Z, _P]),
    "mla_linear_fwd_split": (_I, [_P] * 6 + [_I] * 8 + [_P]),
    "mla_linear_dgrad_split": (_I, [_P] * 5 + [_I] * 8 + [_P]),
    "mla_linear_wgrad_split_ws_bytes": (_Z, [_I, _I, _I]),
    "mla_linear_wgrad_split": (_I, [_P, _P, _P] + [_I] * 6 + [_P, _Z, _P]),
    "mla_linear_wgrad_split_bias": (_I, [_P, _P, _P, _P, _I, _I, _I, _I, _I, _I, _P, _Z, _P]),
    "mla_linear_fwd_bf16": (_I, [_P] * 6 + [_I] * 8 + [_P]),
    "mla_linear_dgrad_bf16": (_I, [_P] * 5 + [_I] * 8 + [_P]),
    "mla_linear_wgrad_ws_bytes_bf16": (_Z, [_I, _I, _I]),
    "mla_linear_wgrad_bf16": (_I, [_P, _P, _P] + [_I] * 6 + [_P, _Z, _P]),
    "mla_linear_wgrad_bias_bf16": (_I, [_P, _P, _P, _P, _I, _I, _I, _I, _I, _I, _P, _Z, _P]),
    "mla_colreduce_ws_elems": (_Z, [_I, _I]),
    "mla_colsum_rows": (_I, [_P, _P, _P, _I, _I, _P]),
    "mla_layernorm_fwd": (_I, [_P] * 6 + [_I, _I, _F, _P]),
    "mla_layernorm_bwd": (_I, [_P] * 10 + [_I, _I, _P]),
    "mla_bgemm": (_I, [_P, _P, _P, _I, _I, _I, _I, _I, _P, _P, _P, _Z, _Z, _Z, _F, _P]),
    "mla_softmax_fwd": (_I, [_P, _P, _I, _I, _I, _P]),
    "mla_softmax_bwd": (_I, [_P, _P, _I, _I, _I, _P]),
    "mla_attention_fwd": (_I, [_P, _P, _P, _P, _I, _I, _I, _I, _P]),
    "mla_attention_bwd": (_I, [_P] * 7 + [_I, _I, _I, _I, _P]),
    "mla_tokens_assemble": (_I, [_P] * 6 + [_I, _I, _I, _I, _P]),
    "mla_tokens_assemble_bwd_ws_bytes": (_Z, [_I, _I, _I]),
    "mla_tokens_assemble_bwd": (_I, [_P] * 6 + [_I, _I, _I, _I, _P, _Z, _P]),
    "mla_patchify": (_I, [_P, _P, _I, _I, _I, _I, _I, _I, _P]),
    "mla_frames_check": (_I, [_P, _I, _I, _I, _Z, _I, _I]),
    "mla_frames_resample": (_I, [_P, _Z, _P, _P, _P, _P, _I, _I, _I, _I, _I, _P]),
}

_lib = None


def load() -> ctypes.CDLL:
    global _lib
    if _lib is not None:
        return _lib
    if not os.path.exists(LIB_PATH):
        raise MLAHipError(
            f"{LIB_PATH} not found: build it with `python -c 'import __graft_entry__ as g; g.build()'` "
            "(or `make -C multimodal-learning-with-alternating-unimodal-adaptation_amd/csrc`). "
            "mla_hip has no CPU/eager fallback.")
    lib = ctypes.CDLL(LIB_PATH)
    for name, (res, args) in PROTOTYPES.items():
        try:
            fn = getattr(lib, name)
        except AttributeError as e:
            raise MLAHipError(f"libmla_hip.so does not export {name}") from e
        fn.restype = res
        fn.argtypes = args
    _lib = lib
    return lib


def check(rc: int, who: str) -> None:
    if rc != 0:
        msg = load().mla_last_error()
        raise MLAHipError(f"{who} failed (status {rc}): {msg.decode() if msg else '?'}")
```

### multimodal-learning-with-alternating-unimodal-adaptation_amd/mla_hip/encoder.py

```python
from __future__ import annotations

import math
import os
from typing import Dict, List, Optional, Tuple

import torch

from . import ops
from ._lib import MLAHipError
from .module import BatchNorm2dHolder, Conv2dHolder, FlatEncoder

FUSE_BN_REDUCE = os.environ.get("MLA_FUSE_BN_REDUCE", "1") != "0"
DS_DGRAD_FOLD = os.environ.get("MLA_DS_DGRAD_FOLD", "1") != "0"
BN_FOLD = os.environ.get("MLA_BN_FOLD", "1") != "0"


def conv_specs(modality: str) -> List[Tuple[str, int, int, int, int, int]]:
    if modality not in ("audio", "visual"):
        raise NotImplementedError("Incorrect modality, should be audio or visual but got {}".format(modality))
    specs = [("conv1", 1 if modality == "audio" else 3, 64, 7, 2, 3)]
    inpl = 64
    for li, planes in enumerate([64, 128, 256, 512], start=1):
        for bi in range(2):
            stride = 2 if (li > 1 and bi == 0) else 1
            specs.append((f"layer{li}.{bi}.conv1", inpl, planes, 3, stride, 1))
            specs.append((f"layer{li}.{bi}.conv2", planes, planes, 3, 1, 1))
            if bi == 0 and (stride != 1 or inpl != planes):
                specs.append((f"layer{li}.{bi}.downsample.0", inpl, planes, 1, stride, 0))
            inpl = planes
    return specs


def bn_name_for_conv(conv_name: str) -> str:
    if conv_name == "conv1":
        return "bn1"
    if conv_name.endswith("downsample.0"):
        return conv_name[:-1] + "1"
    return conv_name.replace("conv", "bn")


class ResNet18Encoder(FlatEncoder):

    side_wgrad = True

    def __init__(self, modality: str, device="cuda", seed: Optional[int] = None, conv_math: Optional[str] = None):
        super().__init__(device, conv_math)
        self.modality = modality
        self.specs = conv_specs(modality)
        self.stem_split = (self.conv_math in ("split", "bf16") and os.environ.get("MLA_STEM_SPLIT", "1") != "0"
                           and ops.conv2d_stem_supported(self.specs[0][1], self.specs[0][2], self.specs[0][3], self.specs[0][3], self.specs[0][4], self.specs[0][5]))
        self._alloc_flat([(name + ".weight", (k, k, cin, cout)) for name, cin, cout, k, _s, _p in self.specs] +
                         [(bn_name_for_conv(name) + leaf, (cout,)) for name, _cin, cout, _k, _s, _p in self.specs
                          for leaf in (".weight", ".bias")])
        self.bn_names = [bn_name_for_conv(n) for n, *_ in self.specs]
        self.bn_ch = {bn_name_for_conv(n): cout for n, _ci, cout, *_ in self.specs}
        tot = sum(self.bn_ch.values())
        self.running = torch.zeros(2 * tot, device=self.device, dtype=torch.float32)
        self.rm, self.rv = {}, {}
        o = 0
        for bn in self.bn_names:
            c = self.bn_ch[bn]
            self.rm[bn] = self.running[o:o + c]
            self.rv[bn] = self.running[tot + o:tot + o + c]
            o += c
        self.running[tot:].fill_(1.0)
        self.num_batches_tracked = {bn: 0 for bn in self.bn_names}
        self._rinv_flat = torch.zeros(tot, device=self.device, dtype=torch.float32)
        self._tot_bn = tot
        self.rinv = {}
        o = 0
        for bn in self.bn_names:
            c = self.bn_ch[bn]
            self.rinv[bn] = self._rinv_flat[o:o + c]
            o += c
        self.grad_ready = False
        self._fwd_training = False
        self._plan_key = None
        self._ws: dict = {}
        self.fuse_bn_reduce = FUSE_BN_REDUCE and not self.bf16
        self._build_wsplit([(name, name + ".weight", k * k, cin, cout) for name, cin, cout, k, _s, _p in self.specs if cin % 64 == 0])
        self.wgrad_stream: Optional[torch.cuda.Stream] = None
        for name, _cin, _cout, _k, s_, p_ in self.specs:
            w = self._param_view(self.p[name + ".weight"], self.g[name + ".weight"], lambda t: t.permute(3, 2, 0, 1), name + ".weight")
            parent, leaf = self._descend(self, name)
            parent.add_module(leaf, Conv2dHolder(w, s_, p_))
            bn = bn_name_for_conv(name)
            bw = self._param_view(self.p[bn + ".weight"], self.g[bn + ".weight"], lambda t: t, bn + ".weight")
            bb = self._param_view(self.p[bn + ".bias"], self.g[bn + ".bias"], lambda t: t, bn + ".bias")
            parent, leaf = self._descend(self, bn)
            parent.add_module(leaf, BatchNorm2dHolder(bw, bb, self.rm[bn], self.rv[bn]))
        self.register_state_dict_pre_hook(ResNet18Encoder._before_state_dict)
        self.register_load_state_dict_post_hook(ResNet18Encoder._after_load_state_dict)
        self.reset_parameters(seed)

    @torch.no_grad()
    def reset_parameters(self, seed: Optional[int] = None) -> None:
        gen = torch.Generator(device="cpu")
        if seed is not None:
            gen.manual_seed(seed)
        else:
            gen.seed()
        for name, cin, cout, k, _s, _p in self.specs:
            std = math.sqrt(2.0 / (cout * k * k))
            w = torch.randn((k, k, cin, cout), generator=gen) * std
            self.p[name + ".weight"].copy_(w)
            bn = bn_name_for_conv(name)
            self.p[bn + ".weight"].fill_(1.0)
            self.p[bn + ".bias"].zero_()

    def _bn_module(self, bn: str):
        m = self
        for part in bn.split("."):
            m = m._modules[part]
        return m

    @staticmethod
    def _before_state_dict(self, prefix, keep_vars) -> None:
        for bn in self.bn_names:
            self._bn_module(bn).num_batches_tracked.fill_(self.num_batches_tracked[bn])

    @staticmethod
    def _after_load_state_dict(self, incompatible_keys) -> None:
        for bn in self.bn_names:
            self.num_batches_tracked[bn] = int(self._bn_module(bn).num_batches_tracked)

    def grads_as_reference(self) -> Dict[str, torch.Tensor]:
        self._await_tail()
        out = {}
        for k in self.layout:
            t = self.g[k]
            out[k] = t.permute(3, 2, 0, 1).contiguous() if t.dim() == 4 else t.clone()
        return out

    def _plan(self, N: int, H: int, W: int) -> dict:
        key = (N, H, W)
        if self._plan_key == key:
            return self._ws
        dev = self.device
        ws: dict = {"shapes": {}}
        f32 = dict(device=dev, dtype=torch.float32)
        cin0 = self.specs[0][1]
        h1, w1 = ops.conv_out(H, 7, 2, 3), ops.conv_out(W, 7, 2, 3)
        hp, wp = ops.conv_out(h1, 3, 2, 1), ops.conv_out(w1, 3, 2, 1)
        ws["x0_shape"] = (N, H, W, cin0)
        ws["y_stem"] = torch.empty((N, h1, w1, 64), **f32)
        ws["p0"] = torch.empty((N, hp, wp, 64), **f32)
        ws["pool_idx"] = torch.empty((N, hp, wp, 64), device=dev, dtype=torch.uint8)
        max_act = N * hp * wp * 64
        max_partial = max(ops.conv2d_fwd_partial_elems(N, H, W, cin0, 64, 7, 7, 2, 3), ops.conv2d_stem_fwd_partial_elems())
        max_wgrad = max(ops.conv2d_wgrad_ws_bytes(N, H, W, cin0, 64, 7, 7, 2, 3), ops.conv2d_stem_wgrad_split_ws_bytes(cin0))
        max_bnws = ops.bn_bwd_ws_elems(N * h1 * w1, 64)
        max_w = 0
        ch, cw, inpl = hp, wp, 64
        blocks = []
        for li, planes in enumerate([64, 128, 256, 512], start=1):
            for bi in range(2):
                pre = f"layer{li}.{bi}"
                stride = 2 if (li > 1 and bi == 0) else 1
                oh, ow = ops.conv_out(ch, 3, stride, 1), ops.conv_out(cw, 3, stride, 1)
                has_ds = bi == 0 and (stride != 1 or inpl != planes)
                blk = {"pre": pre, "stride": stride, "cin": inpl, "cout": planes, "in_hw": (ch, cw), "out_hw": (oh, ow),
                       "ds": has_ds, "fold": False}
                for nm in ("y1", "y2", "out"):
                    blk[nm] = torch.empty((N, oh, ow, planes), **f32)
                if has_ds:
                    blk["yd"] = torch.empty((N, oh, ow, planes), **f32)
                blocks.append(blk)
                max_act = max(max_act, N * oh * ow * planes, N * ch * cw * inpl)
                for (ci, co, k, s, p, hh, ww) in ((inpl, planes, 3, stride, 1, ch, cw), (planes, planes, 3, 1, 1, oh, ow)) + \
                        (((inpl, planes, 1, stride, 0, ch, cw),) if has_ds else ()):
                    max_partial = max(max_partial, ops.conv2d_fwd_partial_elems(N, hh, ww, ci, co, k, k, s, p))
                    max_wgrad = max(max_wgrad, ops.conv2d_wgrad_ws_bytes(N, hh, ww, ci, co, k, k, s, p))
                    if self.conv_math == "split":
                        max_wgrad = max(max_wgrad, ops.conv2d_wgrad_split_ws_bytes(N, hh, ww, ci, co, k, k, s, p))
                    elif self.bf16:
                        max_wgrad = max(max_wgrad, ops.conv2d_wgrad_ws_bytes_bf16(N, hh, ww, ci, co, k, k, s, p))
                    max_w = max(max_w, ci * co * k * k)
                max_bnws = max(max_bnws, ops.bn_bwd_ws_elems(N * oh * ow, planes))
                ch, cw, inpl = oh, ow, planes
        ws["blocks"] = blocks
        ws["feat_hw"] = (ch, cw)
        ws["idn"] = torch.empty(max_act, **f32)
        ws["partial"] = torch.empty(max(max_partial, 1), **f32)
        ws["stats"] = {bn: (torch.empty(self.bn_ch[bn], **f32), torch.empty(self.bn_ch[bn], **f32)) for bn in self.bn_names}
        ws["bwd_sizes"] = (max_act, max_wgrad, max_w, max_bnws)
        self._ws, self._plan_key = ws, key
        return ws

    def _bwd_ws(self, ws: dict) -> None:
        if "G" in ws:
            return
        max_act, max_wgrad, max_w, max_bnws = ws["bwd_sizes"]
        f32 = dict(device=self.device, dtype=torch.float32)
        ws["G"] = [torch.empty(max_act, **f32) for _ in range(4)]
        ws["DY"] = {"conv1": torch.empty_like(ws["y_stem"])}
        for blk in ws["blocks"]:
            ws["DY"][blk["pre"] + ".conv1"] = torch.empty_like(blk["y1"])
            ws["DY"][blk["pre"] + ".conv2"] = torch.empty_like(blk["y2"])
            if blk["ds"]:
                ws["DY"][blk["pre"] + ".downsample.0"] = torch.empty_like(blk["yd"])
        ws["wgrad_ws"] = torch.empty((max_wgrad + 3) // 4, **f32)
        ws["wt_ws"] = torch.empty(max_w, **f32)
        ws["bn_ws"] = torch.empty(max_bnws, **f32)
        n_bnp = max(ops.conv2d_dgrad_bn_partial_elems(b["out"].shape[0], b["out"].shape[1], b["out"].shape[2], b["cout"])
                    for b in ws["blocks"])
        ws["bnp"] = [torch.empty(n_bnp, **f32) for _ in range(3)]

    def train(self, mode: bool = True):
        super().train(mode)
        self._await_tail()
        if not self.training:
            ops.bn_invstd(self.running[self._tot_bn:], self._rinv_flat)
        return self

    def _bn_in(self, ws, bn):
        mean, invstd = ws["stats"][bn]
        return (mean, invstd, self.p[bn + ".weight"], self.p[bn + ".bias"])

    def _conv_fwd(self, ws, st, x, name, stride, pad, y, partial=None, bn_in=None) -> int:
        w = self.p[name + ".weight"]
        wsp = self.wsp.get(name)
        if name == "conv1" and self.stem_split:
            return ops.conv2d_stem_fwd_split(x, w, y=y, bn_partial=partial, stream=st)[1]
        if bn_in is not None:
            return ops.conv2d_fwd_split_bnin(x, wsp[0], w.shape, stride, pad, bn_in, y=y, bn_partial=partial, stream=st)[1]
        if wsp is not None:
            fwd = ops.conv2d_fwd_bf16 if self.bf16 else ops.conv2d_fwd_split
            return fwd(x, wsp[0], w.shape, stride, pad, y=y, bn_partial=partial, stream=st)[1]
        return ops.conv2d_fwd(x, w, stride, pad, y=y, bn_partial=partial, stream=st)[1]

    def _conv_bn(self, ws, st, x, conv_name, stride, pad, y, out, relu, residual=None, bn_in=None):
        bn = bn_name_for_conv(conv_name)
        C = y.shape[3]
        M = y.numel() // C
        if not self.training:
            self._conv_fwd(ws, st, x, conv_name, stride, pad, y)
            ops.bn_apply(y, self.rm[bn], self.rinv[bn], self.p[bn + ".weight"], self.p[bn + ".bias"], out, M, C, relu, residual=residual, stream=st)
            return
        tiles = self._conv_fwd(ws, st, x, conv_name, stride, pad, y, ws["partial"], bn_in)
        mean, invstd = ws["stats"][bn]
        ops.bn_finalize(ws["partial"], tiles, M, C, mean, invstd, self.rm[bn], self.rv[bn], stream=st)
        self.num_batches_tracked[bn] += 1
        if out is None:
            return
        ops.bn_apply(y, mean, invstd, self.p[bn + ".weight"], self.p[bn + ".bias"], out, M, C, relu, residual=residual, stream=st)

    def _stem(self, ws, st) -> None:
        x, y = ws["x0"], ws["y_stem"]
        ga, be = self.p["bn1.weight"], self.p["bn1.bias"]
        if not self.training:
            self._conv_fwd(ws, st, x, "conv1", 2, 3, y)
            ops.bn_relu_maxpool_fwd(y, self.rm["bn1"], self.rinv["bn1"], ga, be, ws["p0"], ws["pool_idx"], stream=st)
            return
        tiles = self._conv_fwd(ws, st, x, "conv1", 2, 3, y, ws["partial"])
        mean, invstd = ws["stats"]["bn1"]
        ops.bn_finalize(ws["partial"], tiles, y.numel() // 64, 64, mean, invstd, self.rm["bn1"], self.rv["bn1"], stream=st)
        self.num_batches_tracked["bn1"] += 1
        ops.bn_relu_maxpool_fwd(y, mean, invstd, ga, be, ws["p0"], ws["pool_idx"], stream=st)

    def stem_relu(self, gamma: Optional[torch.Tensor] = None, beta: Optional[torch.Tensor] = None) -> torch.Tensor:
        ws = self._ws
        y = ws["y_stem"]
        mean, invstd = ws["stats"]["bn1"] if self._fwd_training else (self.rm["bn1"], self.rinv["bn1"])
        ga = self.p["bn1.weight"] if gamma is None else gamma.to(y.device, torch.float32).contiguous()
        be = self.p["bn1.bias"] if beta is None else beta.to(y.device, torch.float32).contiguous()
        out = torch.empty_like(y)
        ops.bn_apply(y, mean, invstd, ga, be, out, y.numel() // 64, 64, True)
        return out

    def block_a1(self, blk: dict, gamma: Optional[torch.Tensor] = None, beta: Optional[torch.Tensor] = None) -> torch.Tensor:
        if not blk["fold"]:
            return blk["a1"]
        bn = blk["pre"] + ".bn1"
        y = blk["y1"]
        C = y.shape[3]
        mean, invstd = self._ws["stats"][bn]
        ga = self.p[bn + ".weight"] if gamma is None else gamma.to(y.device, torch.float32).contiguous()
        be = self.p[bn + ".bias"] if beta is None else beta.to(y.device, torch.float32).contiguous()
        out = torch.empty_like(y)
        ops.bn_apply(y, mean, invstd, ga, be, out, y.numel() // C, C, True)
        return out

    def forward(self, x: torch.Tensor) -> torch.Tensor:
        self._await_tail()
        st = ops.cur_stream()
        if self.modality == "visual":
            if x.dim() != 5:
                raise MLAHipError("visual encoder expects (B,C,T,H,W)")
            B, C, T, H, W = x.shape
            N = B * T
        else:
            if x.dim() != 4 or x.shape[1] != 1:
                raise MLAHipError("audio encoder expects (B,1,H,W)")
            N, C, H, W = x.shape
        if C != self.specs[0][1]:
            raise MLAHipError(f"{self.modality} encoder expects {self.specs[0][1]} input channels, got {C}")
        ws = self._plan(N, H, W)
        if self.wsp and (self.training or self._wsplit_dirty):
            self._refresh_wsplit(st)
        x = x.contiguous()
        if self.modality == "visual":
            if "x0" not in ws:
                ws["x0"] = torch.empty((N, H, W, C), device=self.device, dtype=torch.float32)
            ops.video_to_nhwc(x, ws["x0"], stream=st)
        else:
            if "x0" not in ws:
                ws["x0"] = torch.empty((N, H, W, 1), device=self.device, dtype=torch.float32)
            ws["x0"].copy_(x.view(N, H, W, 1))
        self._fwd_training = False
        self._stem(ws, st)
        cur = ws["p0"]
        for blk in ws["blocks"]:
            pre = blk["pre"]
            fold = blk["fold"] = bool(BN_FOLD and self.training and self.fuse_bn_reduce and self.conv_math == "split"
                                      and ops.conv2d_bnfold_supported(*blk["y1"].shape, blk["cout"], 3, 3, 1, 1))
            if not fold and "a1" not in blk:
                blk["a1"] = torch.empty_like(blk["y1"])
            self._conv_bn(ws, st, cur, pre + ".conv1", blk["stride"], 1, blk["y1"], None if fold else blk["a1"], relu=True)
            if blk["ds"]:
                idn = ws["idn"][:blk["yd"].numel()].view(blk["yd"].shape)
                self._conv_bn(ws, st, cur, pre + ".downsample.0", blk["stride"], 0, blk["yd"], idn, relu=False)
            else:
                idn = cur
            self._conv_bn(ws, st, blk["y1"] if fold else blk["a1"], pre + ".conv2", 1, 1, blk["y2"], blk["out"], relu=True, residual=idn,
                          bn_in=self._bn_in(ws, pre + ".bn1") if fold else None)
            blk["xin"] = cur
            cur = blk["out"]
        self._fwd_training, self.grad_ready = self.training, False
        return cur

    def _bn_bwd(self, ws, st, bn, dout, x, dx, reduced=None):
        C = self.bn_ch[bn]
        M = x.numel() // C
        mean, invstd = ws["stats"][bn]
        if reduced is not None:
            ops.bn_bwd_from_partial(dout, x, mean, invstd, self.p[bn + ".weight"], dx, self.g[bn + ".weight"],
                                    self.g[bn + ".bias"], reduced[0], reduced[1], M, C, stream=st)
            return
        ops.bn_bwd(dout, x, mean, invstd, self.p[bn + ".weight"], dx, self.g[bn + ".weight"], self.g[bn + ".bias"],
                   ws["bn_ws"], M, C, stream=st)

    def backward_from_pooled(self, dfeat: torch.Tensor, P: int) -> None:
        if not self._fwd_training:
            raise MLAHipError(f"{self.modality} encoder: backward_from_pooled needs a training-mode forward, but the most recent forward "
                              "ran in eval mode (or none has run)")
        ws = self._ws
        st = ops.cur_stream()
        self._bwd_ws(ws)
        G = ws["G"]
        last = ws["blocks"][-1]
        out = last["out"]
        NB = dfeat.shape[0]
        d = G[0][:out.numel()].view(out.shape)
        ops.avgpool_bwd(dfeat.contiguous(), d, NB, P, out.shape[3], relu_src=out, stream=st)
        self._backward_trunk(ws, st)

    def _wgrad(self, ws, x, dy, name, stride, pad, bn_in=None) -> None:
        if bn_in is not None:
            wgrad = ops.conv2d_wgrad_split_bnin
        elif name == "conv1" and self.stem_split:
            wgrad = ops.conv2d_stem_wgrad_split
        elif self.bf16 and name in self.wsp:
            wgrad = ops.conv2d_wgrad_bf16
        else:
            wgrad = ops.conv2d_wgrad_split if name in self.wsp else ops.conv2d_wgrad
        args = (x, dy, self.g[name + ".weight"], stride, pad, ws["wgrad_ws"]) + (() if bn_in is None else (bn_in,))
        side = self.wgrad_stream
        if side is None:
            wgrad(*args)
            return
        ev = torch.cuda.Event()
        ev.record()
        side.wait_event(ev)
        with torch.cuda.stream(side):
            wgrad(*args)

    def _dgrad(self, ws, st, dy, name, x_shape, stride, pad, dx, residual=None, relu_src=None, bn_next=(), class_mask=0xF,
               residual_mask=0xF, mask_gb=None):
        wsp = self.wsp.get(name)
        w = self.p[name + ".weight"]
        if not self.fuse_bn_reduce:
            bn_next = ()
        reqs = [(y,) + tuple(ws["stats"][bn]) + (part,) for bn, y, part in bn_next]
        if mask_gb is not None:
            r = ops.conv2d_dgrad_split_bnmask(dy, wsp[1], w.shape, x_shape, stride, pad, dx, reqs[0], mask_gb[0], mask_gb[1], stream=st)
        elif wsp is not None and self.bf16:
            r = ops.conv2d_dgrad_bf16(dy, wsp[1], w.shape, x_shape, stride, pad, dx=dx, residual=residual, relu_src=relu_src, stream=st,
                                      class_mask=class_mask, residual_mask=residual_mask)
        elif wsp is not None:
            r = ops.conv2d_dgrad_split(dy, wsp[1], w.shape, x_shape, stride, pad, dx=dx, residual=residual, relu_src=relu_src,
                                       stream=st, bn_reqs=reqs, class_mask=class_mask, residual_mask=residual_mask)
        else:
            r = ops.conv2d_dgrad(dy, w, x_shape, stride, pad, ws["wt_ws"], dx=dx, residual=residual, relu_src=relu_src, stream=st,
                                 bn_reqs=reqs, class_mask=class_mask, residual_mask=residual_mask)
        return {bn: (part, r[1]) for bn, _, part in bn_next} if bn_next else {}

    def _backward_trunk(self, ws, st) -> None:
        G, DY = ws["G"], ws["DY"]
        if self.wgrad_stream is not None:
            self.wgrad_stream.wait_stream(torch.cuda.current_stream())
        blocks = ws["blocks"]
        bnp = ws["bnp"]
        have: dict = {}
        for bi_, blk in reversed(list(enumerate(blocks))):
            pre = blk["pre"]
            oshape = blk["out"].shape
            n_out = blk["out"].numel()
            xin = blk["xin"]
            d = G[0][:n_out].view(oshape)
            dy2 = DY[pre + ".conv2"]
            self._bn_bwd(ws, st, pre + ".bn2", d, blk["y2"], dy2, have.pop(pre + ".bn2", None))
            da1 = G[2][:n_out].view(oshape)
            bn_in = self._bn_in(ws, pre + ".bn1") if blk["fold"] else None
            a1 = blk["y1"] if blk["fold"] else blk["a1"]
            self._wgrad(ws, a1, dy2, pre + ".conv2", 1, 1, bn_in=bn_in)
            got = self._dgrad(ws, st, dy2, pre + ".conv2", oshape, 1, 1, da1, relu_src=a1 if bn_in is None else None,
                              bn_next=[(pre + ".bn1", blk["y1"], bnp[2])], mask_gb=None if bn_in is None else bn_in[2:])
            dy1 = DY[pre + ".conv1"]
            self._bn_bwd(ws, st, pre + ".bn1", da1, blk["y1"], dy1, got.get(pre + ".bn1"))
            self._wgrad(ws, xin, dy1, pre + ".conv1", blk["stride"], 1)
            dx = G[3][:xin.numel()].view(xin.shape)
            mask = xin if bi_ > 0 else None
            nxt = []
            if bi_ > 0:
                prev = blocks[bi_ - 1]
                nxt.append((prev["pre"] + ".bn2", prev["y2"], bnp[0]))
                if prev["ds"]:
                    nxt.append((prev["pre"] + ".downsample.1", prev["yd"], bnp[1]))
            if blk["ds"]:
                dyd = DY[pre + ".downsample.0"]
                self._bn_bwd(ws, st, pre + ".downsample.1", d, blk["yd"], dyd, have.pop(pre + ".downsample.1", None))
                self._wgrad(ws, xin, dyd, pre + ".downsample.0", blk["stride"], 0)
                if blk["stride"] == 2 and DS_DGRAD_FOLD:
                    self._dgrad(ws, st, dyd, pre + ".downsample.0", xin.shape, 2, 0, dx, class_mask=0x1)
                    have = self._dgrad(ws, st, dy1, pre + ".conv1", xin.shape, 2, 1, dx, residual=dx, relu_src=mask, bn_next=nxt,
                                       residual_mask=0x1)
                else:
                    self._dgrad(ws, st, dy1, pre + ".conv1", xin.shape, blk["stride"], 1, dx)
                    have = self._dgrad(ws, st, dyd, pre + ".downsample.0", xin.shape, blk["stride"], 0, dx, residual=dx, relu_src=mask,
                                       bn_next=nxt)
            else:
                have = self._dgrad(ws, st, dy1, pre + ".conv1", xin.shape, blk["stride"], 1, dx, residual=d, relu_src=mask,
                                   bn_next=nxt)
            G[0], G[3] = G[3], G[0]
        dpool = G[0][:ws["p0"].numel()].view(ws["p0"].shape)
        mean, invstd = ws["stats"]["bn1"]
        ops.bn_bwd_pooled(dpool, ws["pool_idx"], ws["y_stem"], mean, invstd, self.p["bn1.weight"], self.p["bn1.bias"],
                          DY["conv1"], self.g["bn1.weight"], self.g["bn1.bias"], ws["bn_ws"], stream=st)
        self._wgrad(ws, ws["x0"], DY["conv1"], "conv1", 2, 3)
        if self.wgrad_stream is not None:
            torch.cuda.current_stream().wait_stream(self.wgrad_stream)
        self.grad_ready = True
```

### multimodal-learning-with-alternating-unimodal-adaptation_amd/mla_hip/ops.py

```python
from __future__ import annotations

import ctypes
from typing import Optional, Tuple

import torch

from . import _lib
from ._lib import MLAHipError, check

BN_EPS = 1e-5
BN_MOMENTUM = 0.1


class KernelTimer:

    def __init__(self):
        self.records = []

    def begin(self):
        e = torch.cuda.Event(enable_timing=True)
        e.record()
        return e

    def end(self, kind: str, work: float, start, moved: float = 0.0) -> None:
        e = torch.cuda.Event(enable_timing=True)
        e.record()
        self.records.append((kind, work, start, e, moved))

    def summary(self) -> dict:
        groups: dict = {}
        for kind, work, s, e, moved in self.records:
            groups.setdefault((kind, work), []).append(s.elapsed_time(e))
        med = {k: sorted(v)[len(v) // 2] for k, v in groups.items()}
        out: dict = {}
        for kind, work, s, e, moved in self.records:
            d = out.setdefault(kind, {"launches": 0, "ms": 0.0, "ms_raw": 0.0, "work": 0.0, "moved": 0.0, "stalls": 0})
            t, m = s.elapsed_time(e), med[(kind, work)]
            d["ms_raw"] += t
            if len(groups[(kind, work)]) >= 3 and t > 4.0 * m and t > m + 1.0:
                t = m
                d["stalls"] += 1
            d["launches"] += 1
            d["ms"] += t
            d["work"] += work
            d["moved"] += moved
        return out


TIMER: Optional[KernelTimer] = None


def cur_stream() -> int:
    return torch.cuda.current_stream().cuda_stream


def _p(t: Optional[torch.Tensor], dtype=torch.float32) -> Optional[int]:
    if t is None:
        return None
    if not (t.is_cuda and t.dtype == dtype and t.is_contiguous()):
        raise MLAHipError(f"expected a contiguous {dtype} device tensor, got {t.dtype} {t.device} "
                          f"contiguous={t.is_contiguous()}")
    return t.data_ptr()


def _call(name: str, *args) -> None:
    check(getattr(_lib.load(), name)(*args), name)


def _begin():
    return None if TIMER is None else TIMER.begin()


def _end(t0, kind: str, work: float, moved: float = 0.0) -> None:
    if t0 is not None:
        TIMER.end(kind, work, t0, moved)


def conv_out(n: int, k: int, s: int, p: int) -> int:
    return (n + 2 * p - k) // s + 1


def video_to_nhwc(src: torch.Tensor, dst: Optional[torch.Tensor] = None, stream: Optional[int] = None) -> torch.Tensor:
    B, C, T, H, W = src.shape
    if dst is None:
        dst = torch.empty((B * T, H, W, C), device=src.device, dtype=torch.float32)
    _call("mla_video_to_nhwc", _p(src), _p(dst), B, C, T, H, W, stream or cur_stream())
    return dst


def nchw_to_nhwc(src: torch.Tensor, stream: Optional[int] = None) -> torch.Tensor:
    N, C, H, W = src.shape
    dst = torch.empty((N, H, W, C), device=src.device, dtype=torch.float32)
    _call("mla_nchw_to_nhwc", _p(src), _p(dst), N, C, H, W, stream or cur_stream())
    return dst


def nhwc_to_nchw(src: torch.Tensor, stream: Optional[int] = None) -> torch.Tensor:
    N, H, W, C = src.shape
    dst = torch.empty((N, C, H, W), device=src.device, dtype=torch.float32)
    _call("mla_nhwc_to_nchw", _p(src), _p(dst), N, C, H, W, stream or cur_stream())
    return dst


def conv2d_f32_cfg(cfg: int = -1) -> int:
    return int(_lib.load().mla_conv2d_f32_cfg(int(cfg)))


def conv2d_fwd_partial_elems(N, H, W, Cin, Cout, KH, KW, stride, pad) -> int:
    return int(_lib.load().mla_conv2d_fwd_partial_elems(N, H, W, Cin, Cout, KH, KW, stride, pad))


def _conv_fwd(who: str, entry: str, kind: str, x, w, w_dtype, w_shape, stride: int, pad: int, y, bn_partial, stream, bn_in=(),
              min_partial: int = 0) -> Tuple[torch.Tensor, int]:
    N, H, W, Cin = x.shape
    KH, KW, Cin2, Cout = w_shape
    if Cin2 != Cin:
        raise MLAHipError(f"{who}: x has {Cin} channels, weight expects {Cin2}")
    if y is None:
        y = torch.empty((N, conv_out(H, KH, stride, pad), conv_out(W, KW, stride, pad), Cout), device=x.device, dtype=torch.float32)
    if bn_partial is not None and bn_partial.numel() < min_partial:
        raise MLAHipError(f"{who}: bn_partial too small")
    tiles = ctypes.c_int(0)
    t0 = _begin()
    _call(entry, _p(x), _p(w, w_dtype), _p(y), N, H, W, Cin, Cout, KH, KW, stride, pad, *[_p(t) for t in bn_in[:4]], _p(bn_partial),
          ctypes.addressof(tiles), stream or cur_stream())
    _end(t0, kind, 2.0 * y.numel() * KH * KW * Cin)
    return y, tiles.value


def conv2d_fwd(x: torch.Tensor, w_hwio: torch.Tensor, stride: int, pad: int, y: Optional[torch.Tensor] = None,
               bn_partial: Optional[torch.Tensor] = None, stream: Optional[int] = None) -> Tuple[torch.Tensor, int]:
    return _conv_fwd("conv2d_fwd", "mla_conv2d_fwd", "conv_fwd", x, w_hwio, torch.float32, w_hwio.shape, stride, pad, y, bn_partial, stream)


class _BnReduceReq(ctypes.Structure):
    _fields_ = [("x", ctypes.c_void_p), ("mean", ctypes.c_void_p), ("invstd", ctypes.c_void_p), ("partial", ctypes.c_void_p)]


def conv2d_dgrad_bn_partial_elems(N: int, H: int, W: int, Cin: int) -> int:
    return int(_lib.load().mla_conv2d_dgrad_bn_partial_elems(N, H, W, Cin))


def _bn_reqs(bn_reqs, x_shape):
    if not bn_reqs:
        return None, 0
    if len(bn_reqs) > 2:
        raise MLAHipError("conv2d_dgrad: at most two BatchNorm reduction requests")
    N, H, W, Cin = x_shape
    need = conv2d_dgrad_bn_partial_elems(N, H, W, Cin)
    arr = (_BnReduceReq * len(bn_reqs))()
    for q, (x, mean, invstd, partial) in enumerate(bn_reqs):
        if tuple(x.shape) != tuple(x_shape) or mean.numel() != Cin or invstd.numel() != Cin or partial.numel() < need:
            raise MLAHipError(f"conv2d_dgrad: BatchNorm request {q} does not match dx {tuple(x_shape)} (partial >= {need} floats)")
        arr[q].x, arr[q].mean, arr[q].invstd, arr[q].partial = _p(x), _p(mean), _p(invstd), _p(partial)
    return arr, len(bn_reqs)


def _conv_dgrad(entry: str, dy, w, w_dtype, w_shape, x_shape, stride: int, pad: int, dx, bn_reqs, stream, before=(), after=()):
    N, H, W, Cin = x_shape
    KH, KW, _, Cout = w_shape
    if dx is None:
        dx = torch.empty((N, H, W, Cin), device=dy.device, dtype=torch.float32)
    arr, nreq = _bn_reqs(bn_reqs, x_shape)
    tiles = ctypes.c_int(0)
    t0 = _begin()
    _call(entry, _p(dy), _p(w, w_dtype), _p(dx), N, H, W, Cin, Cout, KH, KW, stride, pad, *[_p(t) for t in before],
          ctypes.addressof(arr) if nreq else None, nreq, ctypes.addressof(tiles), *[a if isinstance(a, int) else _p(a) for a in after],
          stream or cur_stream())
    _end(t0, "conv_dgrad", 2.0 * dy.numel() * KH * KW * Cin)
    return (dx, tiles.value) if nreq else dx


def conv2d_dgrad(dy: torch.Tensor, w_hwio: torch.Tensor, x_shape, stride: int, pad: int, wt_ws: torch.Tensor,
                 dx: Optional[torch.Tensor] = None, residual: Optional[torch.Tensor] = None,
                 relu_src: Optional[torch.Tensor] = None, stream: Optional[int] = None, bn_reqs=None,
                 class_mask: int = 0xF, residual_mask: int = 0xF):
    if wt_ws.numel() < w_hwio.numel():
        raise MLAHipError("conv2d_dgrad: wt_ws too small")
    return _conv_dgrad("mla_conv2d_dgrad_classes", dy, w_hwio, torch.float32, w_hwio.shape, x_shape, stride, pad, dx, bn_reqs, stream,
                       before=(residual, relu_src, wt_ws), after=(class_mask, residual_mask))


def conv2d_wsplit(w_hwio: torch.Tensor, transposed: bool, out: Optional[torch.Tensor] = None,
                  stream: Optional[int] = None) -> torch.Tensor:
    KH, KW, Cin, Cout = w_hwio.shape
    n = int(_lib.load().mla_conv2d_wsplit_bytes(Cin, Cout, KH, KW)) // 2
    if out is None:
        out = torch.empty(n, device=w_hwio.device, dtype=torch.int16)
    if out.numel() < n or out.dtype != torch.int16:
        raise MLAHipError("conv2d_wsplit: out must hold 3*KH*KW*Cin*Cout int16")
    _call("mla_conv2d_wsplit", _p(w_hwio), _p(out, torch.int16), Cin, Cout, KH, KW, int(transposed), stream or cur_stream())
    return out


def conv2d_wsplit_batch(params: torch.Tensor, wsplit: torch.Tensor, desc: torch.Tensor, total_blocks: int,
                        stream: Optional[int] = None) -> None:
    _call("mla_conv2d_wsplit_batch", _p(params), _p(wsplit, torch.int16), _p(desc, torch.int32), desc.shape[0], int(total_blocks),
          stream or cur_stream())


def conv2d_fwd_split(x: torch.Tensor, wsplit_t: torch.Tensor, w_shape, stride: int, pad: int,
                     y: Optional[torch.Tensor] = None, bn_partial: Optional[torch.Tensor] = None,
                     stream: Optional[int] = None) -> Tuple[torch.Tensor, int]:
    return _conv_fwd("conv2d_fwd_split", "mla_conv2d_fwd_split", "conv_fwd", x, wsplit_t, torch.int16, w_shape, stride, pad, y, bn_partial,
                     stream)


def conv2d_dgrad_split(dy: torch.Tensor, wsplit: torch.Tensor, w_shape, x_shape, stride: int, pad: int,
                       dx: Optional[torch.Tensor] = None, residual: Optional[torch.Tensor] = None,
                       relu_src: Optional[torch.Tensor] = None, stream: Optional[int] = None, bn_reqs=None,
                       class_mask: int = 0xF, residual_mask: int = 0xF):
    return _conv_dgrad("mla_conv2d_dgrad_split_classes", dy, wsplit, torch.int16, w_shape, x_shape, stride, pad, dx, bn_reqs, stream,
                       before=(residual, relu_src), after=(class_mask, residual_mask))


def conv2d_wimage_bf16(w_hwio: torch.Tensor, transposed: bool, out: Optional[torch.Tensor] = None,
                       stream: Optional[int] = None) -> torch.Tensor:
    KH, KW, Cin, Cout = w_hwio.shape
    n = int(_lib.load().mla_conv2d_wimage_bytes_bf16(Cin, Cout, KH, KW)) // 2
    if out is None:
        out = torch.empty(n, device=w_hwio.device, dtype=torch.int16)
    if out.numel() < n or out.dtype != torch.int16:
        raise MLAHipError("conv2d_wimage_bf16: out must hold KH*KW*Cin*Cout int16")
    _call("mla_conv2d_wimage_bf16", _p(w_hwio), _p(out, torch.int16), Cin, Cout, KH, KW, int(transposed), stream or cur_stream())
    return out


def conv2d_wimage_batch_bf16(params: torch.Tensor, wimage: torch.Tensor, desc: torch.Tensor, total_blocks: int,
                             stream: Optional[int] = None) -> None:
    _call("mla_conv2d_wimage_batch_bf16", _p(params), _p(wimage, torch.int16), _p(desc, torch.int32), desc.shape[0], int(total_blocks),
          stream or cur_stream())


def conv2d_tile_bf16(M: int, Cout: int, k_total: int) -> int:
    return int(_lib.load().mla_conv2d_tile_bf16(int(M), int(Cout), int(k_total)))


def conv2d_fwd_bf16(x: torch.Tensor, wimage_t: torch.Tensor, w_shape, stride: int, pad: int, y: Optional[torch.Tensor] = None,
                    bn_partial: Optional[torch.Tensor] = None, stream: Optional[int] = None) -> Tuple[torch.Tensor, int]:
    return _conv_fwd("conv2d_fwd_bf16", "mla_conv2d_fwd_bf16", "conv_fwd", x, wimage_t, torch.int16, w_shape, stride, pad, y, bn_partial,
                     stream)


def conv2d_dgrad_bf16(dy: torch.Tensor, wimage: torch.Tensor, w_shape, x_shape, stride: int, pad: int,
                      dx: Optional[torch.Tensor] = None, residual: Optional[torch.Tensor] = None,
                      relu_src: Optional[torch.Tensor] = None, stream: Optional[int] = None, class_mask: int = 0xF,
                      residual_mask: int = 0xF) -> torch.Tensor:
    N, H, W, Cin = x_shape
    KH, KW, _, Cout = w_shape
    if dx is None:
        dx = torch.empty((N, H, W, Cin), device=dy.device, dtype=torch.float32)
    t0 = _begin()
    _call("mla_conv2d_dgrad_bf16", _p(dy), _p(wimage, torch.int16), _p(dx), N, H, W, Cin, Cout, KH, KW, stride, pad, _p(residual), _p(relu_src),
          class_mask, residual_mask, stream or cur_stream())
    _end(t0, "conv_dgrad", 2.0 * dy.numel() * KH * KW * Cin)
    return dx


def conv2d_wgrad_ws_bytes_bf16(N, H, W, Cin, Cout, KH, KW, stride, pad) -> int:
    return int(_lib.load().mla_conv2d_wgrad_ws_bytes_bf16(N, H, W, Cin, Cout, KH, KW, stride, pad))


def conv2d_wgrad_bf16(x: torch.Tensor, dy: torch.Tensor, dw_hwio: torch.Tensor, stride: int, pad: int, ws: torch.Tensor,
                      stream: Optional[int] = None) -> torch.Tensor:
    return _conv_wgrad("mla_conv2d_wgrad_bf16", "conv_wgrad", x, dy, dw_hwio, stride, pad, ws, stream)


def conv2d_bnfold_supported(N: int, H: int, W: int, Cin: int, Cout: int, KH: int, KW: int, stride: int, pad: int) -> bool:
    return bool(_lib.load().mla_conv2d_bnfold_supported(N, H, W, Cin, Cout, KH, KW, stride, pad))


def conv2d_fwd_split_bnin(x: torch.Tensor, wsplit_t: torch.Tensor, w_shape, stride: int, pad: int, bn_in, y: Optional[torch.Tensor] = None,
                          bn_partial: Optional[torch.Tensor] = None, stream: Optional[int] = None) -> Tuple[torch.Tensor, int]:
    return _conv_fwd("conv2d_fwd_split_bnin", "mla_conv2d_fwd_split_bnin", "conv_fwd", x, wsplit_t, torch.int16, w_shape, stride, pad, y,
                     bn_partial, stream, bn_in=bn_in)


def conv2d_wgrad_split_bnin(x: torch.Tensor, dy: torch.Tensor, dw_hwio: torch.Tensor, stride: int, pad: int, ws: torch.Tensor, bn_in,
                            stream: Optional[int] = None) -> torch.Tensor:
    return _conv_wgrad("mla_conv2d_wgrad_split_bnin", "conv_wgrad", x, dy, dw_hwio, stride, pad, ws, stream, bn_in=bn_in)


def conv2d_dgrad_split_bnmask(dy: torch.Tensor, wsplit: torch.Tensor, w_shape, x_shape, stride: int, pad: int, dx: torch.Tensor, bn_req,
                              mask_gamma: torch.Tensor, mask_beta: torch.Tensor, stream: Optional[int] = None):
    return _conv_dgrad("mla_conv2d_dgrad_split_bnmask", dy, wsplit, torch.int16, w_shape, x_shape, stride, pad, dx, [bn_req], stream,
                       after=(mask_gamma, mask_beta))


def conv2d_stem_supported(Cin: int, Cout: int, KH: int, KW: int, stride: int, pad: int) -> bool:
    return bool(_lib.load().mla_conv2d_stem_supported(Cin, Cout, KH, KW, stride, pad))


def conv2d_stem_waves(waves: int = -1) -> int:
    return int(_lib.load().mla_conv2d_stem_waves(int(waves)))


def conv2d_stem_fwd_partial_elems() -> int:
    return int(_lib.load().mla_conv2d_stem_fwd_partial_elems())


def conv2d_stem_fwd_split(x: torch.Tensor, w_hwio: torch.Tensor, y: Optional[torch.Tensor] = None,
                          bn_partial: Optional[torch.Tensor] = None, stream: Optional[int] = None) -> Tuple[torch.Tensor, int]:
    return _conv_fwd("conv2d_stem_fwd_split", "mla_conv2d_stem_fwd_split", "stem_fwd", x, w_hwio, torch.float32, w_hwio.shape, 2, 3, y,
                     bn_partial, stream, min_partial=conv2d_stem_fwd_partial_elems() if bn_partial is not None else 0)


def conv2d_stem_wgrad_split_ws_bytes(Cin: int) -> int:
    return int(_lib.load().mla_conv2d_stem_wgrad_split_ws_bytes(Cin))


def _conv_wgrad(entry: str, kind: str, x, dy, dw_hwio, stride: int, pad: int, ws, stream, bn_in=()) -> torch.Tensor:
    N, H, W, Cin = x.shape
    KH, KW, _, Cout = dw_hwio.shape
    t0 = _begin()
    _call(entry, _p(x), _p(dy), _p(dw_hwio), N, H, W, Cin, Cout, KH, KW, stride, pad, *[_p(t) for t in bn_in[:4]], _p(ws),
          ws.numel() * ws.element_size(), stream or cur_stream())
    _end(t0, kind, 2.0 * dy.numel() * KH * KW * Cin)
    return dw_hwio


def conv2d_stem_wgrad_split(x: torch.Tensor, dy: torch.Tensor, dw_hwio: torch.Tensor, stride: int, pad: int, ws: torch.Tensor,
                            stream: Optional[int] = None) -> torch.Tensor:
    return _conv_wgrad("mla_conv2d_stem_wgrad_split", "stem_wgrad", x, dy, dw_hwio, stride, pad, ws, stream)


def conv2d_wgrad_tr(on: int = -1) -> int:
    return int(_lib.load().mla_conv2d_wgrad_tr(int(on)))


def conv2d_patch(on: int = -1) -> int:
    return int(_lib.load().mla_conv2d_patch(int(on)))


def conv2d_dgrad_merge(on: int = -1) -> int:
    return int(_lib.load().mla_conv2d_dgrad_merge(int(on)))


def conv2d_two_phase(on: int = -1) -> int:
    return int(_lib.load().mla_conv2d_two_phase(int(on)))


def conv2d_split_terms(terms: int = 0) -> int:
    return int(_lib.load().mla_conv2d_split_terms(int(terms)))


def conv2d_split_cfg(cfg: int = -1) -> int:
    return int(_lib.load().mla_conv2d_split_cfg(int(cfg)))


def conv2d_wgrad_ws_bytes(N, H, W, Cin, Cout, KH, KW, stride, pad) -> int:
    return int(_lib.load().mla_conv2d_wgrad_ws_bytes(N, H, W, Cin, Cout, KH, KW, stride, pad))


def conv2d_wgrad(x: torch.Tensor, dy: torch.Tensor, dw_hwio: torch.Tensor, stride: int, pad: int, ws: torch.Tensor,
                 stream: Optional[int] = None) -> torch.Tensor:
    return _conv_wgrad("mla_conv2d_wgrad", "conv_wgrad", x, dy, dw_hwio, stride, pad, ws, stream)


def conv2d_wgrad_split_ws_bytes(N, H, W, Cin, Cout, KH, KW, stride, pad) -> int:
    return int(_lib.load().mla_conv2d_wgrad_split_ws_bytes(N, H, W, Cin, Cout, KH, KW, stride, pad))


def conv2d_wgrad_split(x: torch.Tensor, dy: torch.Tensor, dw_hwio: torch.Tensor, stride: int, pad: int, ws: torch.Tensor,
                       stream: Optional[int] = None) -> torch.Tensor:
    return _conv_wgrad("mla_conv2d_wgrad_split", "conv_wgrad", x, dy, dw_hwio, stride, pad, ws, stream)


def bn_stats_partial_elems(M: int, C: int) -> int:
    return int(_lib.load().mla_bn_stats_partial_elems(M, C))


def bn_stats_partial(x2d: torch.Tensor, M: int, C: int, partial: torch.Tensor, stream: Optional[int] = None) -> int:
    tiles = ctypes.c_int(0)
    _call("mla_bn_stats_partial", _p(x2d), M, C, _p(partial), ctypes.addressof(tiles), stream or cur_stream())
    return tiles.value


def bn_finalize(partial: torch.Tensor, tiles: int, M: int, C: int, mean: torch.Tensor, invstd: torch.Tensor,
                running_mean: Optional[torch.Tensor], running_var: Optional[torch.Tensor],
                eps: float = BN_EPS, momentum: float = BN_MOMENTUM, stream: Optional[int] = None) -> None:
    t0 = _begin()
    _call("mla_bn_finalize", _p(partial), tiles, M, C, eps, momentum, _p(mean), _p(invstd), _p(running_mean), _p(running_var), stream or cur_stream())
    _end(t0, "bn_fwd", 0.0)


def bn_apply(x: torch.Tensor, mean, invstd, gamma, beta, out: torch.Tensor, M: int, C: int, relu: bool,
             residual: Optional[torch.Tensor] = None, stream: Optional[int] = None) -> torch.Tensor:
    t0 = _begin()
    _call("mla_bn_apply", _p(x), _p(mean), _p(invstd), _p(gamma), _p(beta), _p(residual), _p(out), M, C, int(relu), stream or cur_stream())
    _end(t0, "bn_fwd", 12.0 * M * C, (12.0 if residual is not None else 8.0) * M * C)
    return out


def bn_bwd_ws_elems(M: int, C: int) -> int:
    return int(_lib.load().mla_bn_bwd_ws_elems(M, C))


def bn_bwd(dout, x, mean, invstd, gamma, dx, dgamma, dbeta, ws, M: int, C: int, relu_out=None, g_out=None,
           stream: Optional[int] = None) -> None:
    t0 = _begin()
    _call("mla_bn_bwd", _p(dout), _p(relu_out), _p(x), _p(mean), _p(invstd), _p(gamma), _p(dx), _p(dgamma), _p(dbeta), _p(g_out), _p(ws), M, C,
          stream or cur_stream())
    _end(t0, "bn_bwd", 20.0 * M * C, 20.0 * M * C)


def bn_relu_maxpool_fwd(y, mean, invstd, gamma, beta, out, idx, stream: Optional[int] = None) -> None:
    N, H, W, C = y.shape
    t0 = _begin()
    _call("mla_bn_relu_maxpool_fwd", _p(y), _p(mean), _p(invstd), _p(gamma), _p(beta), _p(out), _p(idx, torch.uint8), N, H, W, C,
          stream or cur_stream())
    by = 4.0 * N * H * W * C + 5.0 * out.numel()
    _end(t0, "bn_fwd", by, by)


def bn_bwd_pooled(dpool, idx, y, mean, invstd, gamma, beta, dy, dgamma, dbeta, ws, stream: Optional[int] = None) -> None:
    N, H, W, C = y.shape
    t0 = _begin()
    _call("mla_bn_bwd_pooled", _p(dpool), _p(idx, torch.uint8), _p(y), _p(mean), _p(invstd), _p(gamma), _p(beta), _p(dy), _p(dgamma), _p(dbeta),
          _p(ws), N, H, W, C, stream or cur_stream())
    by = 12.0 * N * H * W * C + 10.0 * dpool.numel()
    _end(t0, "bn_bwd", by, by)


def bn_bwd_from_partial(dout, x, mean, invstd, gamma, dx, dgamma, dbeta, partial, tiles: int, M: int, C: int,
                        stream: Optional[int] = None) -> None:
    t0 = _begin()
    _call("mla_bn_bwd_from_partial", _p(dout), _p(x), _p(mean), _p(invstd), _p(gamma), _p(dx), _p(dgamma), _p(dbeta), _p(partial), tiles, M, C,
          stream or cur_stream())
    _end(t0, "bn_bwd", 12.0 * M * C, 12.0 * M * C)


def maxpool_fwd(x: torch.Tensor, y: torch.Tensor, idx: torch.Tensor, stream: Optional[int] = None) -> None:
    N, H, W, C = x.shape
    _call("mla_maxpool3x3s2_fwd", _p(x), _p(y), _p(idx, torch.uint8), N, H, W, C, stream or cur_stream())


def maxpool_bwd(dy, idx, dx, x_shape, relu_src=None, stream: Optional[int] = None) -> None:
    N, H, W, C = x_shape
    _call("mla_maxpool3x3s2_bwd", _p(dy), _p(idx, torch.uint8), _p(relu_src), _p(dx), N, H, W, C, stream or cur_stream())


def avgpool_fwd(x, y, NB: int, P: int, C: int, stream: Optional[int] = None) -> None:
    _call("mla_avgpool_fwd", _p(x), _p(y), NB, P, C, stream or cur_stream())


def avgpool_bwd(dy, dx, NB: int, P: int, C: int, relu_src=None, stream: Optional[int] = None) -> None:
    _call("mla_avgpool_bwd", _p(dy), _p(relu_src), _p(dx), NB, P, C, stream or cur_stream())


def head_ws_elems(B: int, C: int) -> int:
    return int(_lib.load().mla_head_ws_elems(B, C))


def head_ce_fwd_bwd(X, W, b, labels, logits, loss, dW, db, dX, ws, inv_batch: float, stream: Optional[int] = None) -> None:
    B, D = X.shape
    C = W.shape[0]
    _call("mla_head_ce_fwd_bwd", _p(X), _p(W), _p(b), _p(labels, torch.int64), _p(logits), _p(loss), _p(dW), _p(db), _p(dX), _p(ws), B, D, C,
          inv_batch, stream or cur_stream())


def ce_fwd_bwd(logits, labels, loss, dlogits, ws, inv_batch: float, stream: Optional[int] = None) -> None:
    B, C = logits.shape
    _call("mla_ce_fwd_bwd", _p(logits), _p(labels, torch.int64), _p(loss), _p(dlogits), _p(ws), B, C, inv_batch, stream or cur_stream())


def head_bwd(X, W, dlogits, dW, db, dX, scale: float = 1.0, stream: Optional[int] = None) -> None:
    B, D = X.shape
    C = W.shape[0]
    if tuple(dlogits.shape) != (B, C):
        raise MLAHipError(f"head_bwd: dlogits {tuple(dlogits.shape)} does not match ({B}, {C})")
    _call("mla_head_bwd", _p(X), _p(W), _p(dlogits), _p(dW), _p(db), _p(dX), B, D, C, scale, stream or cur_stream())


def _concat_ptrs(xs, who: str):
    M = len(xs)
    if M not in (2, 3):
        raise MLAHipError(f"{who}: needs 2 or 3 feature tensors, got {M}")
    B, D = xs[0].shape
    for x in xs[1:]:
        if tuple(x.shape) != (B, D):
            raise MLAHipError(f"{who}: every modality must have the same (B, D); got {[tuple(t.shape) for t in xs]}")
    return [_p(x) for x in xs] + [None] * (3 - M), M, B, D


def concat_head_ws_elems(B: int, C: int, M: int) -> int:
    return int(_lib.load().mla_concat_head_ws_elems(B, C, M))


def concat_head_ce_fwd_bwd(xs, W, b, labels, out, out_m, loss, loss_m, dW, db, dxs, ws, inv_batch: float,
                           stream: Optional[int] = None) -> None:
    x, M, B, D = _concat_ptrs(xs, "concat_head_ce_fwd_bwd")
    C = W.shape[0]
    if tuple(W.shape) != (C, M * D) or len(dxs) != M:
        raise MLAHipError(f"concat_head_ce_fwd_bwd: W {tuple(W.shape)} does not match {M} x (B, {D})")
    dx = [_p(t) for t in dxs] + [None] * (3 - M)
    _call("mla_concat_head_ce_fwd_bwd", x[0], x[1], x[2], _p(W), _p(b), _p(labels, torch.int64), _p(out), _p(out_m), _p(loss), _p(loss_m), _p(dW),
          _p(db), dx[0], dx[1], dx[2], _p(ws), M, B, D, C, inv_batch, stream or cur_stream())


def concat_head_fwd(xs, W, b, out, out_m, stream: Optional[int] = None) -> None:
    x, M, B, D = _concat_ptrs(xs, "concat_head_fwd")
    C = W.shape[0]
    if tuple(W.shape) != (C, M * D):
        raise MLAHipError(f"concat_head_fwd: W {tuple(W.shape)} does not match {M} x (B, {D})")
    _call("mla_concat_head_fwd", x[0], x[1], x[2], _p(W), _p(b), _p(out), _p(out_m), M, B, D, C, stream or cur_stream())


def concat_head_bwd(xs, W, dlogits, dW, db, dxs, scale: float = 1.0, stream: Optional[int] = None) -> None:
    x, M, B, D = _concat_ptrs(xs, "concat_head_bwd")
    C = W.shape[0]
    if tuple(W.shape) != (C, M * D) or tuple(dlogits.shape) != (B, C) or len(dxs) != M:
        raise MLAHipError(f"concat_head_bwd: W {tuple(W.shape)} / dlogits {tuple(dlogits.shape)} do not match {M} x ({B}, {D})")
    dx = [_p(t) for t in dxs] + [None] * (3 - M)
    _call("mla_concat_head_bwd", x[0], x[1], x[2], _p(W), _p(dlogits), _p(dW), _p(db), dx[0], dx[1], dx[2], M, B, D, C, scale, stream or cur_stream())


def scale_by_device_scalar(x, scalar, stream: Optional[int] = None) -> None:
    _call("mla_scale_by_device_scalar", _p(x), _p(scalar), x.numel(), stream or cur_stream())


def colsum(X, r, scale: float, stream: Optional[int] = None) -> None:
    B, D = X.shape
    _call("mla_colsum", _p(X), _p(r), B, D, scale, stream or cur_stream())


def gs_ws_elems(D: int, C: int) -> int:
    return int(_lib.load().mla_gs_ws_elems(D, C))


def gs_project(Pl, r, G, alpha: float, ws, stream: Optional[int] = None) -> None:
    D = Pl.shape[0]
    C = G.shape[0]
    _call("mla_gs_project", _p(Pl), _p(r), _p(G), D, C, alpha, _p(ws), stream or cur_stream())


def sgd_step(p, g, buf, lr: float, momentum: float, wd: float, first: bool, stream: Optional[int] = None) -> None:
    _call("mla_sgd_step", _p(p), _p(g), _p(buf), p.numel(), lr, momentum, wd, int(first), stream or cur_stream())


LN_EPS = 1e-5


def linear_fwd(x, w_kn, bias, y, groups: int, rows: int, K: int, N: int, x_group_rows: Optional[int] = None, x_off: int = 0,
               y_group_rows: Optional[int] = None, y_off: int = 0, residual=None, y_gelu=None, stream: Optional[int] = None,
               wsplit=None, bf16: bool = False):
    if bf16 and wsplit is None:
        raise MLAHipError("linear_fwd: bf16 needs the weight image (conv2d_wimage_bf16)")
    if wsplit is not None:
        _call("mla_linear_fwd_bf16" if bf16 else "mla_linear_fwd_split", _p(x), _p(wsplit, torch.int16), _p(bias), _p(residual), _p(y), _p(y_gelu), groups, rows, x_group_rows or rows,
              x_off, y_group_rows or rows, y_off, K, N, stream or cur_stream())
        return
    _call("mla_linear_fwd", _p(x), _p(w_kn), _p(bias), _p(residual), _p(y), _p(y_gelu), groups, rows, x_group_rows or rows, x_off,
          y_group_rows or rows, y_off, K, N, stream or cur_stream())


def linear_dgrad(dy, w_kn, dx, wt_ws, groups: int, rows: int, K: int, N: int, residual=None, gelu_src=None,
                 stream: Optional[int] = None, wsplit=None, bf16: bool = False):
    if bf16 and wsplit is None:
        raise MLAHipError("linear_dgrad: bf16 needs the weight image (conv2d_wimage_bf16)")
    if wsplit is not None:
        _call("mla_linear_dgrad_bf16" if bf16 else "mla_linear_dgrad_split", _p(dy), _p(wsplit, torch.int16), _p(dx), _p(residual), _p(gelu_src), groups, rows, rows, 0, rows, 0, K, N,
              stream or cur_stream())
        return
    _call("mla_linear_dgrad", _p(dy), _p(w_kn), _p(dx), _p(residual), _p(gelu_src), _p(wt_ws), groups, rows, rows, 0, rows, 0, K, N,
          stream or cur_stream())


def linear_wgrad_ws_bytes(M: int, K: int, N: int, split: bool = False, bf16: bool = False) -> int:
    if bf16:
        return int(_lib.load().mla_linear_wgrad_ws_bytes_bf16(M, K, N))
    if split:
        return int(_lib.load().mla_linear_wgrad_split_ws_bytes(M, K, N))
    return int(_lib.load().mla_linear_wgrad_ws_bytes(M, K, N))


def linear_wgrad(x, dy, dw_kn, ws, groups: int, rows: int, K: int, N: int, x_group_rows: Optional[int] = None, x_off: int = 0,
                 stream: Optional[int] = None, split: bool = False, dbias: Optional[torch.Tensor] = None, bf16: bool = False):
    if split or bf16:
        _call("mla_linear_wgrad_bias_bf16" if bf16 else "mla_linear_wgrad_split_bias", _p(x), _p(dy), _p(dw_kn), _p(dbias), groups, rows, x_group_rows or rows, x_off, K, N, _p(ws),
              ws.numel() * ws.element_size(), stream or cur_stream())
        return
    if dbias is not None:
        raise MLAHipError("linear_wgrad: the fused bias gradient exists on the split arithmetic only (use colsum_rows)")
    _call("mla_linear_wgrad", _p(x), _p(dy), _p(dw_kn), groups, rows, x_group_rows or rows, x_off, K, N, _p(ws), ws.numel() * ws.element_size(),
          stream or cur_stream())


def colreduce_ws_elems(M: int, C: int) -> int:
    return int(_lib.load().mla_colreduce_ws_elems(M, C))


def colsum_rows(x, out, ws, M: int, C: int, stream: Optional[int] = None):
    _call("mla_colsum_rows", _p(x), _p(out), _p(ws), M, C, stream or cur_stream())


def layernorm_fwd(x, w, b, y, mean, rstd, M: int, D: int, eps: float = LN_EPS, stream: Optional[int] = None):
    _call("mla_layernorm_fwd", _p(x), _p(w), _p(b), _p(y), _p(mean), _p(rstd), M, D, eps, stream or cur_stream())


def layernorm_bwd(dy, x, w, mean, rstd, dx, dw, db, ws, M: int, D: int, add=None, stream: Optional[int] = None):
    _call("mla_layernorm_bwd", _p(dy), _p(x), _p(w), _p(mean), _p(rstd), _p(add), _p(dx), _p(dw), _p(db), _p(ws), M, D, stream or cur_stream())


def bgemm(A, B, C, batches: int, heads: int, M: int, N: int, K: int, a_strides, b_strides, c_strides, alpha: float = 1.0,
          a_off: int = 0, b_off: int = 0, c_off: int = 0, stream: Optional[int] = None):
    L4 = ctypes.c_long * 4
    sa, sb, sc = L4(*a_strides), L4(*b_strides), L4(*c_strides)
    pa, pb, pc = _p(A) + 4 * a_off, _p(B) + 4 * b_off, _p(C) + 4 * c_off
    if min(a_off, b_off, c_off) < 0 or a_off >= A.numel() or b_off >= B.numel() or c_off >= C.numel():
        raise MLAHipError("bgemm: element offset outside its buffer")
    _call("mla_bgemm", pa, pb, pc, batches, heads, M, N, K, ctypes.addressof(sa), ctypes.addressof(sb), ctypes.addressof(sc), A.numel() - a_off,
          B.numel() - b_off, C.numel() - c_off, alpha, stream or cur_stream())


def softmax_fwd(S, pad_mask, B: int, H: int, n: int, stream: Optional[int] = None):
    _call("mla_softmax_fwd", _p(S), _p(pad_mask), B, H, n, stream or cur_stream())


def softmax_bwd(P, dP, B: int, H: int, n: int, stream: Optional[int] = None):
    _call("mla_softmax_bwd", _p(P), _p(dP), B, H, n, stream or cur_stream())


def attention_fwd(qkv, pad_mask, o, lse, B: int, H: int, n: int, hd: int, stream: Optional[int] = None):
    _call("mla_attention_fwd", _p(qkv), _p(pad_mask), _p(o), _p(lse), B, H, n, hd, stream or cur_stream())


def attention_bwd(do, qkv, o, lse, pad_mask, dqkv, dvec, B: int, H: int, n: int, hd: int, stream: Optional[int] = None):
    _call("mla_attention_bwd", _p(do), _p(qkv), _p(o), _p(lse), _p(pad_mask), _p(dqkv), _p(dvec), B, H, n, hd, stream or cur_stream())


def tokens_assemble(x0, table, ids, pos, type_emb, cls, B: int, L: int, D: int, stream: Optional[int] = None):
    V = table.shape[0] if table is not None else 0
    _call("mla_tokens_assemble", _p(x0), _p(table), _p(ids, torch.int64), _p(pos), _p(type_emb), _p(cls), B, L, D, V, stream or cur_stream())


def tokens_assemble_bwd_ws_bytes(B: int, L: int, D: int) -> int:
    return int(_lib.load().mla_tokens_assemble_bwd_ws_bytes(B, L, D))


def tokens_assemble_bwd(dx0, colsum_all, ids, dcls, dtype, dtable, B: int, L: int, D: int, stream: Optional[int] = None,
                        ws: Optional[torch.Tensor] = None):
    V = dtable.shape[0] if dtable is not None else 0
    if dtable is not None and ws is None:
        ws = torch.empty(tokens_assemble_bwd_ws_bytes(B, L, D), device=dx0.device, dtype=torch.uint8)
    _call("mla_tokens_assemble_bwd", _p(dx0), _p(colsum_all), _p(ids, torch.int64), _p(dcls), _p(dtype), _p(dtable), B, L, D, V,
          _p(ws, torch.uint8) if ws is not None else None, ws.numel() if ws is not None else 0, stream or cur_stream())


def patchify(img, out, P: int = 16, transposed_hw: Optional[tuple] = None, stream: Optional[int] = None):
    if transposed_hw is None:
        B, C, H, W = img.shape
        tr = 0
    else:
        B, C = img.shape[0], 1
        H, W = transposed_hw
        tr = 1
    _call("mla_patchify", _p(img), _p(out), B, C, H, W, P, tr, stream or cur_stream())


def head_logits(X, W, b, logits, stream: Optional[int] = None):
    B, D = X.shape
    _call("mla_head_logits", _p(X), _p(W), _p(b), _p(logits), B, D, W.shape[0], stream or cur_stream())


def eval_fuse(outs, labels, counts, weights_out, dynamic: bool, alphas, stream: Optional[int] = None):
    M = len(outs)
    B, C = outs[0].shape
    o = [_p(t) for t in outs] + [None] * (3 - M)
    al = list(alphas) + [0.0] * (3 - len(alphas))
    _call("mla_eval_fuse", o[0], o[1], o[2], _p(labels, torch.int64), _p(counts, torch.int32), _p(weights_out), M, B, C, int(dynamic), al[0], al[1],
          al[2], stream or cur_stream())


def bn_invstd(var, invstd, eps: float = BN_EPS, stream: Optional[int] = None):
    _call("mla_bn_invstd", _p(var), _p(invstd), var.numel(), eps, stream or cur_stream())


def ogm_coeff(outs, labels, alpha: float, coeff, info=None, stream: Optional[int] = None):
    M = len(outs)
    B, C = outs[0].shape
    ptrs = [_p(t) for t in outs] + [None] * (3 - M)
    _call("mla_ogm_coeff", ptrs[0], ptrs[1], ptrs[2], _p(labels, torch.int64), M, B, C, alpha, _p(coeff), _p(info), stream or cur_stream())


def ogm_chunk_elems() -> int:
    return int(_lib.load().mla_ogm_chunk_elems())


def ogm_ws_bytes(total_chunks: int, n_seg: int) -> int:
    return int(_lib.load().mla_ogm_ws_bytes(total_chunks, n_seg))


def ogm_modulate(grad, seg_desc, first_chunk, n_seg: int, total_chunks: int, coeff, ge: bool, seed: int, step: int, ws,
                 stream: Optional[int] = None):
    _call("mla_ogm_modulate", _p(grad), _p(seg_desc, torch.int64), _p(first_chunk, torch.int32), n_seg, total_chunks, _p(coeff), int(ge), seed, step,
          _p(ws, torch.uint8) if ws is not None else None, ws.numel() if ws is not None else 0, stream or cur_stream())


def _desc_host(desc_host: torch.Tensor) -> torch.Tensor:
    if desc_host.is_cuda or desc_host.dtype != torch.int64 or desc_host.dim() != 2 or desc_host.shape[1] != 8 \
            or not desc_host.is_contiguous():
        raise MLAHipError(f"frame descriptors: expected a contiguous host int64 (N, 8) tensor, got {desc_host.dtype} "
                          f"{tuple(desc_host.shape)} on {desc_host.device}")
    return desc_host


def frames_check(desc_host: torch.Tensor, B: int, T: int, frames_bytes: int, out_h: int = 224, out_w: int = 224) -> None:
    d = _desc_host(desc_host)
    _call("mla_frames_check", d.data_ptr(), d.shape[0], B, T, frames_bytes, out_h, out_w)


def frames_resample(frames: torch.Tensor, desc: torch.Tensor, desc_host: torch.Tensor, lut: torch.Tensor, out: torch.Tensor,
                    T: int, stream: Optional[int] = None) -> torch.Tensor:
    d = _desc_host(desc_host)
    if tuple(desc.shape) != tuple(d.shape):
        raise MLAHipError(f"frame descriptors: device table {tuple(desc.shape)} and host table {tuple(d.shape)} differ")
    if tuple(lut.shape) != (3, 256) or out.dim() != 5 or out.shape[1] != 3 or out.shape[2] != T:
        raise MLAHipError(f"frames_resample: lut {tuple(lut.shape)} / out {tuple(out.shape)} do not match (3, 256) / (B, 3, {T}, H, W)")
    B, _, _, OH, OW = out.shape
    _call("mla_frames_resample", _p(frames, torch.uint8), frames.numel(), _p(desc, torch.int64), d.data_ptr(), _p(lut), _p(out), d.shape[0], B, T, OH,
          OW, stream or cur_stream())
    return out
```

Baseline: 2795 samples/s.

## Fuse stem BN+maxpool backward into stem weight-gradient kernel, skip dy materialization

The stem backward no longer writes the full-resolution conv1 dy tensor. The BN-pooled backward now only computes dgamma/dbeta. The stem wgrad kernel recomputes dy on the fly from the pooled gradient, pool indices, the pre-BN output and the BN stats while it loads its operands, with ragged-edge variants. This removes a large write plus re-read of the stem activation gradient, at the cost of more VALU work and extra loads inside the wgrad MMA loop. The fused kernel also runs on the side wgrad stream.

```diff
diff --git a/include/mla_hip.h b/include/mla_hip.h
--- a/include/mla_hip.h
+++ b/include/mla_hip.h
@@ -97,6 +97,11 @@
 int mla_conv2d_stem_wgrad_split(const float* x, const float* dy, float* dw_hwio,
                                 int N, int H, int W, int Cin, int Cout, int KH, int KW, int stride, int pad,
                                 void* ws, size_t ws_bytes, void* stream);
+int mla_conv2d_stem_wgrad_split_bnpool(const float* x, const float* dpool, const uint8_t* idx, const float* y,
+                                       const float* mean, const float* invstd, const float* gamma, const float* beta,
+                                       const float* dgamma, const float* dbeta, float* dw_hwio,
+                                       int N, int H, int W, int Cin, int Cout, int KH, int KW, int stride, int pad,
+                                       void* ws, size_t ws_bytes, void* stream);
 int mla_conv2d_split_cfg(int cfg);
 
 size_t mla_conv2d_wimage_bytes_bf16(int Cin, int Cout, int KH, int KW);
diff --git a/multimodal-learning-with-alternating-unimodal-adaptation_amd/csrc/bn.hip b/multimodal-learning-with-alternating-unimodal-adaptation_amd/csrc/bn.hip
--- a/multimodal-learning-with-alternating-unimodal-adaptation_amd/csrc/bn.hip
+++ b/multimodal-learning-with-alternating-unimodal-adaptation_amd/csrc/bn.hip
@@ -464,7 +464,7 @@
                                                                    int W, int C, int OH, int OW) {
   const int c4n = C >> 2, QH = (H + 1) >> 1, QW = (W + 1) >> 1;
   const size_t total = (size_t)N * QH * QW * c4n;
-  const float invM = 1.0f / ((float)N * (float)H * (float)W);
+  const float invM = bn_inv_count(N, H, W);
   for (size_t i = (size_t)blockIdx.x * blockDim.x + threadIdx.x; i < total; i += (size_t)gridDim.x * blockDim.x) {
     const int cg = (int)(i % c4n);
     size_t p = i / c4n;
@@ -473,7 +473,10 @@
     const int n = (int)(p / QH);
     const f32x4 mu = reinterpret_cast<const f32x4*>(mean)[cg], is = reinterpret_cast<const f32x4*>(invstd)[cg];
     const f32x4 ga = reinterpret_cast<const f32x4*>(gamma)[cg], be = reinterpret_cast<const f32x4*>(beta)[cg];
-    const f32x4 dg = reinterpret_cast<const f32x4*>(dgamma)[cg] * invM, db = reinterpret_cast<const f32x4*>(dbeta)[cg] * invM;
+    const f32x4 dgs = reinterpret_cast<const f32x4*>(dgamma)[cg], dbs = reinterpret_cast<const f32x4*>(dbeta)[cg];
+    f32x4 dg, db;
+#pragma unroll
+    for (int e = 0; e < 4; ++e) { dg[e] = bn_bwd_scale(dgs[e], invM); db[e] = bn_bwd_scale(dbs[e], invM); }
     f32x4 wg[2][2];
     int ws[2][2][4];
 #pragma unroll
@@ -504,15 +507,14 @@
           for (int wx = 0; wx <= px; ++wx) {
             const int code = (py + 1 - 2 * wy) * 3 + (px + 1 - 2 * wx);
 #pragma unroll
-            for (int e = 0; e < 4; ++e) g[e] += ws[wy][wx][e] == code ? wg[wy][wx][e] : 0.f;
+            for (int e = 0; e < 4; ++e) g[e] = pool_pick(g[e], ws[wy][wx][e], code, wg[wy][wx][e]);
           }
         const size_t o = ((size_t)(n * H + iy) * W + ix) * c4n + cg;
         const f32x4 xv = reinterpret_cast<const f32x4*>(y)[o];
-        const f32x4 av = bn_val(xv, mu, is, ga, be);
-#pragma unroll
-        for (int e = 0; e < 4; ++e) g[e] = av[e] > 0.f ? g[e] : 0.f;
-        const f32x4 xhat = (xv - mu) * is;
-        reinterpret_cast<f32x4*>(out)[o] = ga * is * (g - db - xhat * dg);
+        f32x4 r;
+#pragma unroll
+        for (int e = 0; e < 4; ++e) r[e] = bn_bwd_pooled_dy1(xv[e], g[e], mu[e], is[e], ga[e], be[e], dg[e], db[e]);
+        reinterpret_cast<f32x4*>(out)[o] = r;
       }
   }
 }
@@ -650,7 +652,7 @@
   MLA_REQUIRE(Ml > 0 && Ml < (1L << 31), "mla_bn_bwd_pooled: bad dims");
   const int M = (int)Ml;
   if (int rc = bn_check("mla_bn_bwd_pooled", M, C)) return rc;
-  MLA_REQUIRE(dpool && idx && y && mean && invstd && gamma && beta && dy && dgamma && dbeta && ws, "mla_bn_bwd_pooled: null pointer");
+  MLA_REQUIRE(dpool && idx && y && mean && invstd && gamma && beta && dgamma && dbeta && ws, "mla_bn_bwd_pooled: null pointer");
   hipStream_t st = (hipStream_t)stream;
   const int OH = (H + 2 - 3) / 2 + 1, OW = (W + 2 - 3) / 2 + 1;
   const int MP = N * OH * OW;
@@ -671,6 +673,7 @@
     bn_bwd_finalize_kernel<<<cdiv(C, 64), 256, 0, st>>>(scratch, S, C, dgamma, dbeta);
     MLA_CHECK_LAUNCH("bn_bwd_finalize_kernel");
   }
+  if (!dy) return MLA_OK;
   const size_t nq = (size_t)N * ((H + 1) / 2) * ((W + 1) / 2) * (C / 4);
   bn_bwd_pooled_apply_kernel<<<ew_grid(nq), 256, 0, st>>>(dpool, idx, y, mean, invstd, gamma, beta, dgamma, dbeta, dy, N, H, W, C, OH, OW);
   MLA_CHECK_LAUNCH("bn_bwd_pooled_apply_kernel");
diff --git a/multimodal-learning-with-alternating-unimodal-adaptation_amd/csrc/common.h b/multimodal-learning-with-alternating-unimodal-adaptation_amd/csrc/common.h
--- a/multimodal-learning-with-alternating-unimodal-adaptation_amd/csrc/common.h
+++ b/multimodal-learning-with-alternating-unimodal-adaptation_amd/csrc/common.h
@@ -79,6 +79,15 @@
 
 __device__ __forceinline__ float bn_val1(float x, float mu, float is, float ga, float be) { return fmaf((x - mu) * is, ga, be); }
 
+__device__ __forceinline__ float pool_pick(float g, int sel, int code, float w) { return g + (sel == code ? w : 0.f); }
+__device__ __forceinline__ float bn_bwd_pooled_dy1(float y, float g, float mu, float is, float ga, float be, float dg, float db) {
+  const float gm = bn_val1(y, mu, is, ga, be) > 0.f ? g : 0.f;
+  const float xhat = (y - mu) * is;
+  return (ga * is) * fmaf(-xhat, dg, gm - db);
+}
+__device__ __forceinline__ float bn_inv_count(int N, int H, int W) { return 1.0f / ((float)N * (float)H * (float)W); }
+__device__ __forceinline__ float bn_bwd_scale(float sum, float invM) { return __fmul_rn(sum, invM); }
+
 __device__ __forceinline__ void tile_coords(int wg, int gridM, int gridN, int& tm, int& tn) {
   if (gridN <= 8) {
     tm = wg / gridN;
diff --git a/multimodal-learning-with-alternating-unimodal-adaptation_amd/csrc/stem_split.hip b/multimodal-learning-with-alternating-unimodal-adaptation_amd/csrc/stem_split.hip
--- a/multimodal-learning-with-alternating-unimodal-adaptation_amd/csrc/stem_split.hip
+++ b/multimodal-learning-with-alternating-unimodal-adaptation_amd/csrc/stem_split.hip
@@ -1,6 +1,9 @@
 #include "split_common.h"
 #ifndef WG_VALU
 #define WG_VALU 6
+#endif
+#ifndef WG_VALU_FUSED
+#define WG_VALU_FUSED 16
 #endif
 
 namespace {
@@ -28,8 +31,18 @@
   unsigned x_bytes, y_bytes;
 };
 
+struct StemBnPool {
+  const float* dpool;
+  const uint8_t* idx;
+  const float *mean, *invstd, *gamma, *beta, *dgamma, *dbeta;
+  int PH, PW;
+  unsigned dp_bytes;
+};
+
 __device__ __forceinline__ unsigned off_or_oob(int ok, unsigned off) { return off | ((unsigned)ok - 1u); }
 __device__ __forceinline__ int in_range(int v, int n) { return (int)((unsigned)v < (unsigned)n); }
+
+__device__ __forceinline__ int buf_load_u8(rsrc_t r, unsigned voff) { return (int)__builtin_amdgcn_raw_buffer_load_b8(r, (int)voff, 0, 0); }
 
 __device__ __forceinline__ void buf_store1(rsrc_t r, float v, unsigned voff) {
   __builtin_amdgcn_raw_buffer_store_b32(__builtin_bit_cast(unsigned, v), r, (int)voff, 0, 0);
@@ -322,9 +335,11 @@
   static constexpr int LDSF = 2 * SBUF > RACC ? 2 * SBUF : RACC;
 };
 
-template <int CIN>
+template <int CIN, bool FUSED, bool RAGGED>
 __global__ __launch_bounds__(512, 2) void stem_wgrad_split_kernel(const float* __restrict__ X, const float* __restrict__ dY,
-                                                                   float* __restrict__ slabs, const StemGeom g, unsigned dy_bytes) {
+                                                                   float* __restrict__ slabs, const StemGeom g, unsigned dy_bytes,
+                                                                   const StemBnPool bp) {
+  static_assert(FUSED || !RAGGED, "the plain kernel needs no ragged form: its out-of-range dy loads are zeros");
   using C = StemWCfg<CIN>;
   constexpr int KB = C::KB, XPD = C::XPD, ARR = C::ARR, HALF = C::HALF, PLANE = C::PLANE, COPY = C::COPY, SBUF = C::SBUF;
   constexpr int NT = 512, NLD = (C::NSL + NT - 1) / NT;
@@ -402,29 +417,94 @@
   zero_acc(acc);
 
   constexpr int U = 4 * KB;
+  constexpr bool WDEEP = CIN == 1;
+  constexpr int NWS = WDEEP ? 2 : 1;
   float dyv[2][8];
-  auto load_dy = [&](int t, int s, float (&dst)[8]) {
+  float wp[NWS][2][5];
+  int wc[NWS][2][5], nv[2], nw[NWS];
+  float mu = 0.f, is = 0.f, ga = 0.f, be = 0.f, dg = 0.f, db = 0.f;
+  rsrc_t dpr = yr, ixr = yr;
+  if constexpr (FUSED) {
+    const int ch = ni * 32 + i;
+    const float invM = bn_inv_count(g.N, g.OH, g.OW);
+    mu = bp.mean[ch]; is = bp.invstd[ch]; ga = bp.gamma[ch]; be = bp.beta[ch];
+    dg = bn_bwd_scale(bp.dgamma[ch], invM); db = bn_bwd_scale(bp.dbeta[ch], invM);
+    dpr = make_rsrc(bp.dpool, bp.dp_bytes);
+    ixr = make_rsrc(bp.idx, bp.dp_bytes >> 2);
+  }
+  constexpr unsigned OOB_ROW = 0xFFFFF000u;
+  auto load_dy = [&](int t, int s, int slot) {
     int n, oy0, ox0;
     decode(t, n, oy0, ox0);
     const int oy = oy0 + 4 * wq + s;
-#pragma unroll
-    for (int e = 0; e < 8; ++e) {
-      const int ox = ox0 + 8 * h + e;
-      const int ok = (int)(t < g.ntiles) & (int)(oy < g.OH) & (int)(ox < g.OW);
-      dst[e] = buf_load1(yr, off_or_oob(ok, ((unsigned)((n * g.OH + oy) * g.OW + ox) * 64u + (unsigned)(ni * 32 + i)) * 4u), 0);
-    }
-  };
-  auto load_dy_step = [&](int t, int tn, int s, float (&dst)[8]) {
-    if (s < 4) load_dy(t, s, dst);
-    else load_dy(tn, s - 4, dst);
+    const int tok = (int)(t < g.ntiles);
+    if constexpr (!FUSED) {
+#pragma unroll
+      for (int e = 0; e < 8; ++e) {
+        const int ox = ox0 + 8 * h + e;
+        const int ok = tok & (int)(oy < g.OH) & (int)(ox < g.OW);
+        dyv[slot][e] = buf_load1(yr, off_or_oob(ok, ((unsigned)((n * g.OH + oy) * g.OW + ox) * 64u + (unsigned)(ni * 32 + i)) * 4u), 0);
+      }
+    } else {
+      const int ox = ox0 + 8 * h;
+      const int rok = tok & (int)(oy < g.OH) & (int)(ox < g.OW);
+      const unsigned yo = rok ? ((unsigned)((n * g.OH + oy) * g.OW + ox) * 64u + (unsigned)(ni * 32 + i)) * 4u : OOB_ROW;
+#pragma unroll
+      for (int e = 0; e < 8; ++e) dyv[slot][e] = buf_load1(yr, yo + 256u * e, 0);
+      if constexpr (RAGGED) nv[slot] = rok ? g.OW - ox : 0;
+    }
+  };
+  auto load_win = [&](int t, int s, int slot) {
+    int n, oy0, ox0;
+    decode(t, n, oy0, ox0);
+    const int a = (oy0 + 4 * wq + s) >> 1, b0 = (ox0 >> 1) + 4 * h;
+    const int tok = (int)(t < g.ntiles);
+#pragma unroll
+    for (int wy = 0; wy < 2; ++wy) {
+      if (wy > (s & 1)) continue;
+      const int wok = tok & (int)(a + wy < bp.PH) & (int)(b0 < bp.PW);
+      const unsigned o = (unsigned)((n * bp.PH + a + wy) * bp.PW + b0) * 64u + (unsigned)(ni * 32 + i);
+      const unsigned po = wok ? o * 4u : OOB_ROW, co = wok ? o : OOB_ROW;
+#pragma unroll
+      for (int c = 0; c < 5; ++c) {
+        const unsigned pc = (!RAGGED && c == 4) ? ((wok & (int)(b0 + 4 < bp.PW)) ? po : OOB_ROW) : po;
+        wp[slot][wy][c] = buf_load1(dpr, pc + 256u * c, 0);
+        wc[slot][wy][c] = buf_load_u8(ixr, co + 64u * c);
+      }
+    }
+    if constexpr (RAGGED) nw[slot] = bp.PW - b0;
+  };
+  auto at_step = [&](auto&& ld, int t, int tn, int s, int slot) {
+    if (s < 4) ld(t, s, slot);
+    else ld(tn, s - 4, slot);
+  };
+  auto dy_val = [&](int py, int e) -> float {
+    if constexpr (FUSED) {
+      const int c = e >> 1, px = e & 1, wsl = WDEEP ? py : 0;
+      float gs = 0.f;
+#pragma unroll
+      for (int wy = 0; wy < 2; ++wy)
+#pragma unroll
+        for (int wx = 0; wx < 2; ++wx)
+          if (wy <= py && wx <= px) {
+            float w = wp[wsl][wy][c + wx];
+            if (RAGGED && wx == 1) w = c + wx < nw[wsl] ? w : 0.f;
+            gs = pool_pick(gs, wc[wsl][wy][c + wx], (py + 1 - 2 * wy) * 3 + (px + 1 - 2 * wx), w);
+          }
+      const float d = bn_bwd_pooled_dy1(dyv[py][e], gs, mu, is, ga, be, dg, db);
+      if constexpr (RAGGED) return e < nv[py] ? d : 0.f;
+      else return d;
+    } else {
+      return dyv[py][e];
+    }
   };
   struct BFr { u32x4 p[3]; };
-  auto split_dy_half = [&](int j, const float (&src)[8], BFr& b) {
+  auto split_dy_half = [&](int j, int slot, BFr& b) {
 #pragma unroll
     for (int qq = 0; qq < 2; ++qq) {
       const int q = 2 * j + qq;
       unsigned hi, mid, lo;
-      split_pair<true>(src[2 * q], src[2 * q + 1], hi, mid, lo);
+      split_pair<true>(dy_val(slot, 2 * q), dy_val(slot, 2 * q + 1), hi, mid, lo);
       b.p[0][q] = hi; b.p[1][q] = mid; b.p[2][q] = lo;
     }
   };
@@ -444,11 +524,14 @@
   if (t < g.ntiles) {
 #pragma unroll
     for (int u = 0; u < NLD; ++u) stage_store(0, u);
-    load_dy(t, 0, dyv[0]);
-    split_dy_half(0, dyv[0], bf0);
-    split_dy_half(1, dyv[0], bf0);
-    load_dy(t, 1, dyv[1]);
-    load_dy(t, 2, dyv[0]);
+    load_dy(t, 0, 0);
+    if constexpr (FUSED) load_win(t, 0, 0);
+    split_dy_half(0, 0, bf0);
+    split_dy_half(1, 0, bf0);
+    load_dy(t, 1, 1);
+    if constexpr (FUSED) load_win(t, 1, WDEEP ? 1 : 0);
+    load_dy(t, 2, 0);
+    if constexpr (FUSED && WDEEP) load_win(t, 2, 0);
   }
   __syncthreads();
   constexpr int ST0 = U - NLD < 0 ? 0 : U - NLD;
@@ -457,26 +540,31 @@
     const bool has_next = tn < g.ntiles;
     if (has_next) stage_load(tn);
     const unsigned* Sc = S + cur * SBUF;
+    constexpr bool APRE = !(FUSED && RAGGED && CIN == 3);
     AFr a0, a1;
-    read_a(Sc, 0, a0);
+    if constexpr (APRE) read_a(Sc, 0, a0);
     __builtin_amdgcn_sched_barrier(0);
 #pragma unroll
     for (int u = 0; u < U; ++u) {
       const int s_ = u / KB, kb = u - s_ * KB;
-      AFr& acur = (u & 1) ? a1 : a0;
+      AFr& acur = (APRE && (u & 1)) ? a1 : a0;
       AFr& anext = (u & 1) ? a0 : a1;
       BFr& bcur = (s_ & 1) ? bf1 : bf0;
       BFr& bnext = (s_ & 1) ? bf0 : bf1;
-      if (u + 1 < U) read_a(Sc, u + 1, anext);
-      if (kb < 2) split_dy_half(kb, dyv[(s_ + 1) & 1], bnext);
+      if constexpr (!APRE) read_a(Sc, u, a0);
+      else if (u + 1 < U) read_a(Sc, u + 1, anext);
+      if (kb < 2) split_dy_half(kb, (s_ + 1) & 1, bnext);
       if (u >= ST0) stage_store(cur ^ 1, u - ST0);
       split_mma<6>(acur.p, bcur.p, acc[kb]);
-      if (kb == 1) load_dy_step(t, tn, s_ + 3, dyv[(s_ + 1) & 1]);
+      if (kb == 1) {
+        at_step(load_dy, t, tn, s_ + 3, (s_ + 1) & 1);
+        if constexpr (FUSED) at_step(load_win, t, tn, WDEEP ? s_ + 3 : s_ + 2, WDEEP ? (s_ + 1) & 1 : 0);
+      }
       __builtin_amdgcn_sched_group_barrier(0x100, 16, 0);
 #pragma unroll
       for (int m = 0; m < 6; ++m) {
         __builtin_amdgcn_sched_group_barrier(0x008, 1, 0);
-        __builtin_amdgcn_sched_group_barrier(0x002, WG_VALU, 0);
+        __builtin_amdgcn_sched_group_barrier(0x002, (FUSED && CIN == 1) ? WG_VALU_FUSED : WG_VALU, 0);
       }
       __builtin_amdgcn_sched_barrier(0);
     }
@@ -570,10 +658,11 @@
 
 extern "C" size_t mla_conv2d_stem_wgrad_split_ws_bytes(int Cin) { return (size_t)mla_cu_count() * 49 * Cin * 64 * sizeof(float); }
 
-extern "C" int mla_conv2d_stem_wgrad_split(const float* x, const float* dy, float* dw, int N, int H, int W, int Cin, int Cout,
-                                           int KH, int KW, int stride, int pad, void* ws, size_t ws_bytes, void* stream) {
-  if (int rc = stem_check("mla_conv2d_stem_wgrad_split", N, H, W, Cin, Cout, KH, KW, stride, pad)) return rc;
-  MLA_REQUIRE(x && dy && dw && ws, "mla_conv2d_stem_wgrad_split: null pointer");
+static int stem_wgrad_launch(const char* who, const float* x, const float* dy, const StemBnPool* bp, float* dw, int N, int H, int W,
+                             int Cin, int Cout, int KH, int KW, int stride, int pad, void* ws, size_t ws_bytes, void* stream) {
+  if (int rc = stem_check(who, N, H, W, Cin, Cout, KH, KW, stride, pad)) return rc;
+  MLA_REQUIRE(x && dy && dw && ws, "%s: null pointer", who);
+  MLA_REQUIRE(!bp || (bp->dpool && bp->idx && bp->mean && bp->invstd && bp->gamma && bp->beta && bp->dgamma && bp->dbeta), "%s: null pointer", who);
   StemGeom g;
   g.N = N; g.H = H; g.W = W;
   g.OH = conv_out(H, 7, 2, 3); g.OW = conv_out(W, 7, 2, 3);
@@ -581,16 +670,46 @@
   g.ntiles = N * g.tilesY * g.tilesX;
   g.x_bytes = (unsigned)((size_t)N * H * W * Cin * 4);
   const size_t dyb = (size_t)N * g.OH * g.OW * 64 * 4;
-  MLA_REQUIRE(dyb < 0xFFFFFFF0UL, "mla_conv2d_stem_wgrad_split: dy must be < 4 GiB (32-bit buffer offsets)");
+  MLA_REQUIRE(dyb < 0xFFFFFFF0UL, "%s: dy must be < 4 GiB (32-bit buffer offsets)", who);
   const int grid = g.ntiles < mla_cu_count() ? g.ntiles : mla_cu_count();
   const size_t need = (size_t)grid * 49 * Cin * 64 * sizeof(float);
   if (ws_bytes < need) {
-    mla_set_error("mla_conv2d_stem_wgrad_split: workspace %zu < %zu bytes", ws_bytes, need);
+    mla_set_error("%s: workspace %zu < %zu bytes", who, ws_bytes, need);
     return MLA_ERR_WORKSPACE;
   }
   hipStream_t st = (hipStream_t)stream;
-  if (Cin == 1) stem_wgrad_split_kernel<1><<<grid, 512, 0, st>>>(x, dy, (float*)ws, g, (unsigned)dyb);
-  else stem_wgrad_split_kernel<3><<<grid, 512, 0, st>>>(x, dy, (float*)ws, g, (unsigned)dyb);
+  StemBnPool b = {};
+  if (bp) {
+    b = *bp;
+    b.PH = conv_out(g.OH, 3, 2, 1); b.PW = conv_out(g.OW, 3, 2, 1);
+    b.dp_bytes = (unsigned)((size_t)N * b.PH * b.PW * 64 * 4);
+  }
+  const bool ragged = (g.OH % 16) != 0 || (g.OW % 16) != 0;
+#define STEM_WG(CIN_, FU_, RG_) stem_wgrad_split_kernel<CIN_, FU_, RG_><<<grid, 512, 0, st>>>(x, dy, (float*)ws, g, (unsigned)dyb, b)
+  if (!bp) {
+    if (Cin == 1) STEM_WG(1, false, false);
+    else STEM_WG(3, false, false);
+  } else if (Cin == 1) {
+    if (ragged) STEM_WG(1, true, true);
+    else STEM_WG(1, true, false);
+  } else {
+    if (ragged) STEM_WG(3, true, true);
+    else STEM_WG(3, true, false);
+  }
+#undef STEM_WG
   MLA_CHECK_LAUNCH("stem_wgrad_split_kernel");
   return mla_wgrad_reduce((const float*)ws, dw, (size_t)49 * Cin * 64 / 4, grid, st);
 }
+
+extern "C" int mla_conv2d_stem_wgrad_split(const float* x, const float* dy, float* dw, int N, int H, int W, int Cin, int Cout,
+                                           int KH, int KW, int stride, int pad, void* ws, size_t ws_bytes, void* stream) {
+  return stem_wgrad_launch("mla_conv2d_stem_wgrad_split", x, dy, nullptr, dw, N, H, W, Cin, Cout, KH, KW, stride, pad, ws, ws_bytes, stream);
+}
+
+extern "C" int mla_conv2d_stem_wgrad_split_bnpool(const float* x, const float* dpool, const uint8_t* idx, const float* y, const float* mean,
+                                                  const float* invstd, const float* gamma, const float* beta, const float* dgamma,
+                                                  const float* dbeta, float* dw, int N, int H, int W, int Cin, int Cout, int KH, int KW,
+                                                  int stride, int pad, void* ws, size_t ws_bytes, void* stream) {
+  StemBnPool bp = {dpool, idx, mean, invstd, gamma, beta, dgamma, dbeta, 0, 0, 0u};
+  return stem_wgrad_launch("mla_conv2d_stem_wgrad_split_bnpool", x, y, &bp, dw, N, H, W, Cin, Cout, KH, KW, stride, pad, ws, ws_bytes, stream);
+}
diff --git a/multimodal-learning-with-alternating-unimodal-adaptation_amd/mla_hip/_lib.py b/multimodal-learning-with-alternating-unimodal-adaptation_amd/mla_hip/_lib.py
--- a/multimodal-learning-with-alternating-unimodal-adaptation_amd/mla_hip/_lib.py
+++ b/multimodal-learning-with-alternating-unimodal-adaptation_amd/mla_hip/_lib.py
@@ -54,6 +54,7 @@
     "mla_conv2d_stem_fwd_split": (_I, [_P, _P, _P] + [_I] * 9 + [_P, _P, _P]),
     "mla_conv2d_stem_wgrad_split_ws_bytes": (_Z, [_I]),
     "mla_conv2d_stem_wgrad_split": (_I, [_P, _P, _P] + [_I] * 9 + [_P, _Z, _P]),
+    "mla_conv2d_stem_wgrad_split_bnpool": (_I, [_P] * 11 + [_I] * 9 + [_P, _Z, _P]),
     "mla_conv2d_split_cfg": (_I, [_I]),
     "mla_conv2d_wimage_bytes_bf16": (_Z, [_I] * 4),
     "mla_conv2d_wimage_bf16": (_I, [_P, _P, _I, _I, _I, _I, _I, _P]),
diff --git a/multimodal-learning-with-alternating-unimodal-adaptation_amd/mla_hip/encoder.py b/multimodal-learning-with-alternating-unimodal-adaptation_amd/mla_hip/encoder.py
--- a/multimodal-learning-with-alternating-unimodal-adaptation_amd/mla_hip/encoder.py
+++ b/multimodal-learning-with-alternating-unimodal-adaptation_amd/mla_hip/encoder.py
@@ -13,6 +13,7 @@
 FUSE_BN_REDUCE = os.environ.get("MLA_FUSE_BN_REDUCE", "1") != "0"
 DS_DGRAD_FOLD = os.environ.get("MLA_DS_DGRAD_FOLD", "1") != "0"
 BN_FOLD = os.environ.get("MLA_BN_FOLD", "1") != "0"
+STEM_BWD_FUSE = os.environ.get("MLA_STEM_BWD_FUSE", "1") != "0"
 
 
 def conv_specs(modality: str) -> List[Tuple[str, int, int, int, int, int]]:
@@ -78,6 +79,7 @@
         self._plan_key = None
         self._ws: dict = {}
         self.fuse_bn_reduce = FUSE_BN_REDUCE and not self.bf16
+        self.stem_bwd_fuse = STEM_BWD_FUSE and self.stem_split and self.conv_math == "split"
         self._build_wsplit([(name, name + ".weight", k * k, cin, cout) for name, cin, cout, k, _s, _p in self.specs if cin % 64 == 0])
         self.wgrad_stream: Optional[torch.cuda.Stream] = None
         for name, _cin, _cout, _k, s_, p_ in self.specs:
@@ -193,7 +195,7 @@
         max_act, max_wgrad, max_w, max_bnws = ws["bwd_sizes"]
         f32 = dict(device=self.device, dtype=torch.float32)
         ws["G"] = [torch.empty(max_act, **f32) for _ in range(4)]
-        ws["DY"] = {"conv1": torch.empty_like(ws["y_stem"])}
+        ws["DY"] = {}
         for blk in ws["blocks"]:
             ws["DY"][blk["pre"] + ".conv1"] = torch.empty_like(blk["y1"])
             ws["DY"][blk["pre"] + ".conv2"] = torch.empty_like(blk["y2"])
@@ -364,16 +366,18 @@
             wgrad = ops.conv2d_wgrad_bf16
         else:
             wgrad = ops.conv2d_wgrad_split if name in self.wsp else ops.conv2d_wgrad
-        args = (x, dy, self.g[name + ".weight"], stride, pad, ws["wgrad_ws"]) + (() if bn_in is None else (bn_in,))
+        self._side(wgrad, x, dy, self.g[name + ".weight"], stride, pad, ws["wgrad_ws"], *(() if bn_in is None else (bn_in,)))
+
+    def _side(self, fn, *args) -> None:
         side = self.wgrad_stream
         if side is None:
-            wgrad(*args)
+            fn(*args)
             return
         ev = torch.cuda.Event()
         ev.record()
         side.wait_event(ev)
         with torch.cuda.stream(side):
-            wgrad(*args)
+            fn(*args)
 
     def _dgrad(self, ws, st, dy, name, x_shape, stride, pad, dx, residual=None, relu_src=None, bn_next=(), class_mask=0xF,
                residual_mask=0xF, mask_gb=None):
@@ -445,9 +449,16 @@
             G[0], G[3] = G[3], G[0]
         dpool = G[0][:ws["p0"].numel()].view(ws["p0"].shape)
         mean, invstd = ws["stats"]["bn1"]
-        ops.bn_bwd_pooled(dpool, ws["pool_idx"], ws["y_stem"], mean, invstd, self.p["bn1.weight"], self.p["bn1.bias"],
-                          DY["conv1"], self.g["bn1.weight"], self.g["bn1.bias"], ws["bn_ws"], stream=st)
-        self._wgrad(ws, ws["x0"], DY["conv1"], "conv1", 2, 3)
+        ga, be, dga, dbe = self.p["bn1.weight"], self.p["bn1.bias"], self.g["bn1.weight"], self.g["bn1.bias"]
+        if self.stem_bwd_fuse:
+            ops.bn_bwd_pooled(dpool, ws["pool_idx"], ws["y_stem"], mean, invstd, ga, be, None, dga, dbe, ws["bn_ws"], stream=st)
+            self._side(ops.conv2d_stem_wgrad_split_bnpool, ws["x0"], dpool, ws["pool_idx"], ws["y_stem"], mean, invstd, ga, be, dga, dbe,
+                       self.g["conv1.weight"], ws["wgrad_ws"])
+        else:
+            if "conv1" not in DY:
+                DY["conv1"] = torch.empty_like(ws["y_stem"])
+            ops.bn_bwd_pooled(dpool, ws["pool_idx"], ws["y_stem"], mean, invstd, ga, be, DY["conv1"], dga, dbe, ws["bn_ws"], stream=st)
+            self._wgrad(ws, ws["x0"], DY["conv1"], "conv1", 2, 3)
         if self.wgrad_stream is not None:
             torch.cuda.current_stream().wait_stream(self.wgrad_stream)
         self.grad_ready = True
diff --git a/multimodal-learning-with-alternating-unimodal-adaptation_amd/mla_hip/ops.py b/multimodal-learning-with-alternating-unimodal-adaptation_amd/mla_hip/ops.py
--- a/multimodal-learning-with-alternating-unimodal-adaptation_amd/mla_hip/ops.py
+++ b/multimodal-learning-with-alternating-unimodal-adaptation_amd/mla_hip/ops.py
@@ -324,6 +324,17 @@
     return _conv_wgrad("mla_conv2d_stem_wgrad_split", "stem_wgrad", x, dy, dw_hwio, stride, pad, ws, stream)
 
 
+def conv2d_stem_wgrad_split_bnpool(x: torch.Tensor, dpool: torch.Tensor, idx: torch.Tensor, y: torch.Tensor, mean, invstd, gamma, beta,
+                                   dgamma, dbeta, dw_hwio: torch.Tensor, ws: torch.Tensor, stream: Optional[int] = None) -> torch.Tensor:
+    N, H, W, Cin = x.shape
+    KH, KW, _, Cout = dw_hwio.shape
+    t0 = _begin()
+    _call("mla_conv2d_stem_wgrad_split_bnpool", _p(x), _p(dpool), _p(idx, torch.uint8), _p(y), _p(mean), _p(invstd), _p(gamma), _p(beta),
+          _p(dgamma), _p(dbeta), _p(dw_hwio), N, H, W, Cin, Cout, KH, KW, 2, 3, _p(ws), ws.numel() * ws.element_size(), stream or cur_stream())
+    _end(t0, "stem_wgrad", 2.0 * y.numel() * KH * KW * Cin)
+    return dw_hwio
+
+
 def conv2d_wgrad_tr(on: int = -1) -> int:
     return int(_lib.load().mla_conv2d_wgrad_tr(int(on)))
 
@@ -418,7 +429,10 @@
     t0 = _begin()
     _call("mla_bn_bwd_pooled", _p(dpool), _p(idx, torch.uint8), _p(y), _p(mean), _p(invstd), _p(gamma), _p(beta), _p(dy), _p(dgamma), _p(dbeta),
           _p(ws), N, H, W, C, stream or cur_stream())
-    by = 12.0 * N * H * W * C + 10.0 * dpool.numel()
+    if dy is None:
+        by = 9.0 * dpool.numel()
+    else:
+        by = 12.0 * N * H * W * C + 10.0 * dpool.numel()
     _end(t0, "bn_bwd", by, by)
 
 
```

Result: faster. 2835 samples/s, median of 6 (+1.4%).
